# srendle/libfm

Measured on AMD Instinct MI355X. Metric: SGD training examples/sec at k=64, nnz=32, 1e+08 feat, higher is better.
Workload: dtype f32

## Files before the change

libfm_amd/build.py:

```python
import os
import subprocess
import sys
from concurrent.futures import ThreadPoolExecutor

HERE = os.path.dirname(os.path.abspath(__file__))
ROOT = os.path.dirname(HERE)
CSRC = os.path.join(HERE, "csrc")
SRC = [os.path.join(CSRC, f) for f in ("fmx_core.hip", "fmx_sgd.hip", "fmx_als.hip", "fmx_io.hip", "fmx_comm.hip", "fmx_pair.hip", "fmx_topk.hip", "fmx_pairneg.hip", "fmx_eval.hip", "fmx_post.hip", "fmx_evalq.hip", "fmx_compact.hip", "fmx_rankq.hip", "fmx_mem.hip")]
DEPS = SRC + sorted(os.path.join(CSRC, f) for f in os.listdir(CSRC) if f.endswith(".h")) + [os.path.join(ROOT, "include", "fmx.h")]
EXTRA = os.environ.get("FMX_DEFS", "").split()
OUT = os.path.join(HERE, os.environ.get("FMX_OUT", "libfmx.so"))
OBJ_DIR = os.path.join(HERE, "build" + ("_" + os.environ["FMX_OUT"].replace(".", "_") if "FMX_OUT" in os.environ else ""))
HIPCC = os.environ.get("HIPCC", "/opt/rocm/bin/hipcc")
FLAGS = ["--offload-arch=gfx950", "-O3", "-std=c++17", "-munsafe-fp-atomics", "-fPIC", "-fvisibility=hidden",
         "-Wno-unused-result", "-Wno-unused-value"]


def needs_build():
    if not os.path.exists(OUT):
        return True
    t = os.path.getmtime(OUT)
    return any(os.path.getmtime(d) > t for d in DEPS)


def build(force=False, verbose=False):
    if not force and not needs_build():
        return OUT
    os.makedirs(OBJ_DIR, exist_ok=True)
    objs = [os.path.join(OBJ_DIR, os.path.basename(s)[:-4] + ".o") for s in SRC]

    def cc(pair):
        cmd = [HIPCC] + FLAGS + EXTRA + ["-c", pair[0], "-o", pair[1]]
        if verbose:
            print(" ".join(cmd))
        subprocess.check_call(cmd)
    with ThreadPoolExecutor(len(SRC)) as ex:
        list(ex.map(cc, zip(SRC, objs)))
    cmd = [HIPCC, "--offload-arch=gfx950", "-shared", "-fPIC"] + objs + ["-ldl", "-o", OUT]
    if verbose:
        print(" ".join(cmd))
    subprocess.check_call(cmd)
    return OUT


if __name__ == "__main__":
    print(build(force="--force" in sys.argv, verbose=True))
```

libfm_amd/csrc/fmx_core.hip:

```cpp
#include "fmx_internal.h"

static thread_local std::string g_create_error = "";

int fail(fmx_handle h, int code, const char* fmt, ...) {
  char buf[512];
  va_list ap;
  va_start(ap, fmt);
  vsnprintf(buf, sizeof(buf), fmt, ap);
  va_end(ap);
  if (h) h->err = buf; else g_create_error = buf;
  return code;
}

static int next_pow2(int k) { int p = 1; while (p < k) p <<= 1; return p; }

Hyper make_hyper(const fmx_config& c) {
  Hyper h;
  h.lr = (float)c.learn_rate; h.reg0 = (float)c.reg0; h.regw = (float)c.regw; h.regv = (float)c.regv;
  h.min_target = (float)c.min_target; h.max_target = (float)c.max_target;
  h.task = c.task; h.k0 = c.k0; h.k1 = c.k1;
  h.lr_d = c.learn_rate; h.reg0_d = c.reg0; h.regw_d = c.regw; h.regv_d = c.regv;
  h.min_d = c.min_target; h.max_d = c.max_target;
  h.sgda = 0;
  return h;
}

Shard make_shard(const fmx_config& c) {
  Shard sh;
  sh.n = c.num_attribute; sh.rank = (uint32_t)c.shard_rank; sh.world = (uint32_t)c.shard_world;
  sh.hashed = (c.shard_hash != 0 && c.shard_world > 1) ? 1u : 0u;
  uint32_t bits = 1; while (bits < 32 && (1ull << bits) < c.num_attribute) bits++;
  sh.half_bits = std::max<uint32_t>(1u, (bits + 1) / 2);
  return sh;
}

uint32_t resident_grid(fmx_handle h, const void* kernel, uint64_t n_waves_wanted, int over_default) {
  auto& cache = h->occ_cache;
  auto it = cache.find(kernel);
  int occ;
  if (it == cache.end()) {
    occ = 0;
    if (hipOccupancyMaxActiveBlocksPerMultiprocessor(&occ, kernel, 256, 0) != hipSuccess || occ < 1) occ = 4;
    if (occ > 8) occ = 8;
    cache[kernel] = occ;
  } else {
    occ = it->second;
  }
  uint64_t blocks = (n_waves_wanted + 3) / 4;
  const int over = over_default;
  const uint64_t cap = (uint64_t)occ * (uint64_t)h->num_cu * (uint64_t)over;
  if (blocks < 1) blocks = 1;
  if (blocks > cap) blocks = cap;
  return (uint32_t)blocks;
}
int ensure_scratch(fmx_handle h, size_t batch_cap, size_t rest_cap) {
  if (batch_cap > h->cap) {
    if (h->partial) fmx_dev_free(h->partial);
    if (h->mult) fmx_dev_free(h->mult);
    h->partial = nullptr; h->mult = nullptr; h->cap = 0;
    HIPCHK(h, fmx_dev_alloc(&h->partial, batch_cap * (size_t)(h->KP + 1) * sizeof(float)));
    HIPCHK(h, fmx_dev_alloc(&h->mult, batch_cap * sizeof(float)));
    h->cap = batch_cap;
  }
  if (rest_cap > h->cap_rest) {
    if (h->rest) fmx_dev_free(h->rest);
    h->rest = nullptr; h->cap_rest = 0;
    HIPCHK(h, fmx_dev_alloc(&h->rest, rest_cap * sizeof(float)));
    h->cap_rest = rest_cap;
  }
  return FMX_OK;
}

int check_slot(fmx_handle h, int slot, bool need_target) {
  if (!h) return FMX_E_ARG;
  if (slot < 0 || slot >= FMX_MAX_SLOTS) return fail(h, FMX_E_ARG, "slot %d out of range", slot);
  if (!h->slots[slot].used) return fail(h, FMX_E_STATE, "slot %d holds no rows (call fmx_upload_rows first)", slot);
  if (need_target && !h->slots[slot].target) return fail(h, FMX_E_STATE, "slot %d was uploaded without targets", slot);
  return FMX_OK;
}

int slot_in_session(fmx_handle h, int slot, const char* what) {
  if (h->als.slot >= 0 && h->als.slot == slot)
    return fail(h, FMX_E_STATE, "%s: slot %d is the train slot of an open ALS / MCMC session (call fmx_als_end first)", what, slot);
  return FMX_OK;
}

void free_segments(Slot& s) {
  if (s.t_ent) fmx_dev_free(s.t_ent);
  if (s.seg_feat) fmx_dev_free(s.seg_feat);
  if (s.seg_rel) fmx_dev_free(s.seg_rel);
  if (s.cmask) fmx_dev_free(s.cmask);
  if (s.cseg) fmx_dev_free(s.cseg);
  if (s.cdesc) fmx_dev_free(s.cdesc);
  if (s.d_batch_seg) fmx_dev_free(s.d_batch_seg);
  if (s.d_cbatch) fmx_dev_free(s.d_cbatch);
  if (s.d_batch_base) fmx_dev_free(s.d_batch_base);
  s.cdesc = nullptr; s.d_batch_seg = nullptr; s.d_cbatch = nullptr; s.d_batch_base = nullptr;
  s.t_ent = nullptr; s.seg_feat = nullptr; s.seg_rel = nullptr; s.seg_B = 0; s.nseg = 0;
  s.cmask = nullptr; s.cseg = nullptr; s.ncseg = 0; s.fused_cap = 0;
  s.batch_seg.clear(); s.batch_base.clear(); s.cbatch.clear();
}

void free_block(BlockRows* b) {
  if (!b) return;
  free_slot(b->rows);
  if (b->map) fmx_dev_free(b->map);
  if (b->brow_ptr) fmx_dev_free(b->brow_ptr);
  if (b->brow_list) fmx_dev_free(b->brow_list);
  if (b->pbuf) fmx_dev_free(b->pbuf);
  delete b;
}

void free_slot(Slot& s) {
  for (BlockRows* b : s.blocks) free_block(b);
  s.blocks.clear();
  free_segments(s);
  free_pairs(s);
  free_interactions(s);
  free_post(s);
  if (s.ent) fmx_dev_free(s.ent);
  if (s.row_ptr) fmx_dev_free(s.row_ptr);
  if (s.target) fmx_dev_free(s.target);
  if (s.wside) fmx_dev_free(s.wside);
  if (s.lmask) fmx_dev_free(s.lmask);
  if (s.qid) fmx_dev_free(s.qid);
  s = Slot();
}

int ensure_wside(fmx_handle h, Slot& s) {
  if (s.wside) return FMX_OK;
  if (s.nnz == 0 || s.nnz >= (1ull << 32) - 1) return FMX_OK;
  struct Acc { fmx_handle h; std::chrono::steady_clock::time_point t0;
               ~Acc() { h->setup_acc += std::chrono::duration<double>(std::chrono::steady_clock::now() - t0).count(); } } acc_{h, std::chrono::steady_clock::now()};
  const uint32_t M = (uint32_t)std::min<uint64_t>(std::max<uint64_t>(h->n_local, 1), 1ull << 27);
  uint32_t* last = nullptr;
  hipError_t er = fmx_dev_alloc(&last, (size_t)M * 4);
  if (er == hipSuccess) er = fmx_dev_alloc(&s.wside, (size_t)s.nnz * 4);
  if (er == hipSuccess) er = fmx_dev_alloc(&s.lmask, (size_t)s.n_rows * 8);
  if (er == hipSuccess) er = hipMemsetAsync(last, 0, (size_t)M * 4, h->stream);
  if (er == hipSuccess) {
    hipLaunchKernelGGL(k_wside_last, dim3((unsigned)std::min<uint64_t>((s.nnz + 255) / 256, 8192)), dim3(256), 0, h->stream, s.ent, s.nnz, M, last);
    hipLaunchKernelGGL(k_wside_mask, dim3((unsigned)std::min<uint32_t>((s.n_rows + 3) / 4, 16384)), dim3(256), 0, h->stream, s.ent, s.row_ptr, s.n_rows, M,
                       (const uint32_t*)last, s.lmask, s.wside);
    er = hipGetLastError();
  }
  if (er == hipSuccess) er = hipStreamSynchronize(h->stream);
  if (last) fmx_dev_free(last);
  if (er != hipSuccess) {
    if (s.wside) fmx_dev_free(s.wside);
    if (s.lmask) fmx_dev_free(s.lmask);
    s.wside = nullptr; s.lmask = nullptr;
    return fail(h, FMX_E_HIP, "weight side stream of the slot: %s", hipGetErrorString(er));
  }
  s.wside_version = 0;
  if (getenv("FMX_TRACE_SETUP")) fprintf(stderr, "[fmx setup] weight side stream %8.3f ms\n", 1e3 * std::chrono::duration<double>(std::chrono::steady_clock::now() - acc_.t0).count());
  return FMX_OK;
}

int launch_rest(fmx_handle h, const Slot& s, uint64_t row0, uint32_t n, float* rest, hipStream_t st, const CompactState* snap) {
  if (!s.blocks.empty()) {
    if (row0 != 0 || n != s.n_rows) return fail(h, FMX_E_ARG, "rows with kept blocks are predicted as a whole");
    int rc = ensure_scratch(h, n, 0);
    if (rc) return rc;
    float* S = h->partial;
    float* c = S + (size_t)n * h->KP;
    KP_SWITCH(h->KP, FMX_LAUNCH_WAVES((k_rowsums<KP, true, false>), n, st, s.ent, s.row_ptr, (uint64_t)0, n, RowsF32{h->tb}, h->cfg.k1, S, c));
    for (BlockRows* br : s.blocks) {
      const uint32_t B = br->rows.n_rows;
      if (!B) continue;
      Tab tb = h->tb;
      tb.V += (size_t)br->attr_offset * tb.rs; tb.w += (size_t)br->attr_offset * tb.ws;
      float* Sb = br->pbuf;
      KP_SWITCH(h->KP, FMX_LAUNCH_WAVES((k_rowsums<KP, true, false>), B, st, br->rows.ent, br->rows.row_ptr, (uint64_t)0, B, RowsF32{tb}, h->cfg.k1,
                                         Sb, Sb + (size_t)B * h->KP));
      KP_SWITCH(h->KP, hipLaunchKernelGGL((k_rel_add_partial<KP>), dim3(std::min<uint32_t>((uint32_t)(((uint64_t)n * (h->KP + 1) + 255) / 256), 4096)),
                                            dim3(256), 0, st, br->map, (uint64_t)0, n, B, (const float*)Sb, S));
    }
    KP_SWITCH(h->KP, hipLaunchKernelGGL((k_rest_from_partial<KP>), dim3(wave_grid((n + Map<KP>::EPI - 1) / Map<KP>::EPI)), dim3(256), 0, st,
                                          (const float*)S, (const float*)c, n, rest));
    HIPCHK(h, hipGetLastError());
    return FMX_OK;
  }
  const float* ws = (s.wside && s.wside_version == h->w_version && h->cfg.shard_world == 1) ? s.wside : nullptr;
  if (snap) { KP_SWITCH(h->KP, FMX_LAUNCH_WAVES((k_rowsums<KP, false, true, RowsBf16>), n, st,
                                                 s.ent, s.row_ptr, row0, n, compact_rows(h, *snap), h->cfg.k1, (float*)nullptr, rest)); }
  else { KP_SWITCH(h->KP, FMX_LAUNCH_WAVES((k_rowsums<KP, false, true>), n, st,
                                            s.ent, s.row_ptr, row0, n, RowsF32{h->tb, ws}, h->cfg.k1, (float*)nullptr, rest)); }
  HIPCHK(h, hipGetLastError());
  return FMX_OK;
}

int slot_scores(fmx_handle h, const Slot& s, const CompactState* snap, bool want_yhat, const float** score) {
  int rc = ensure_scratch(h, 0, (size_t)s.n_rows * 2); if (rc) return rc;
  HIPCHK(h, hipEventRecord(h->ev0, h->stream));
  rc = launch_rest(h, s, 0, s.n_rows, h->rest, h->stream, snap); if (rc) return rc;
  *score = h->rest;
  if (!want_yhat) return FMX_OK;
  float* yhat = h->rest + s.n_rows;
  const int k0 = (h->cfg.shard_world > 1 && h->cfg.shard_rank != 0) ? 0 : h->cfg.k0;
  hipLaunchKernelGGL(k_yhat, dim3(std::min<uint32_t>((s.n_rows + 255) / 256, 2048)), dim3(256), 0, h->stream,
                     h->rest, s.n_rows, k0, snap ? snap->w0 : h->w0, yhat);
  HIPCHK(h, hipGetLastError());
  *score = yhat;
  return FMX_OK;
}

int predict_out(fmx_handle h, const Slot& s, const CompactState* snap, double* out) {
  if (s.n_rows == 0) return FMX_OK;
  const float* yhat;
  const int rc = slot_scores(h, s, snap, true, &yhat); if (rc) return rc;
  std::vector<float> tmp(s.n_rows);
  HIPCHK(h, hipMemcpyAsync(tmp.data(), yhat, (size_t)s.n_rows * sizeof(float), hipMemcpyDeviceToHost, h->stream));
  HIPCHK(h, hipStreamSynchronize(h->stream));
  for (uint32_t r = 0; r < s.n_rows; r++) out[r] = (double)tmp[r];
  return FMX_OK;
}

int evaluate_out(fmx_handle h, const Slot& s, const CompactState* snap, fmx_eval* out) {
  const float* rest;
  const int rc = slot_scores(h, s, snap, false, &rest); if (rc) return rc;
  HIPCHK(h, hipMemsetAsync(h->acc, 0, 4 * sizeof(double), h->stream));
  hipLaunchKernelGGL(k_eval, dim3(std::min<uint32_t>((s.n_rows + 255) / 256, 2048)), dim3(256), 0, h->stream,
                     rest, s.target, s.n_rows, make_hyper(h->cfg), snap ? snap->w0 : h->w0, h->acc);
  HIPCHK(h, hipGetLastError());
  HIPCHK(h, hipEventRecord(h->ev1, h->stream));
  double acc[4];
  HIPCHK(h, hipMemcpyAsync(acc, h->acc, sizeof(acc), hipMemcpyDeviceToHost, h->stream));
  HIPCHK(h, hipStreamSynchronize(h->stream));
  float ms = 0;
  HIPCHK(h, hipEventElapsedTime(&ms, h->ev0, h->ev1));
  out->device_seconds = ms * 1e-3;
  out->rmse = std::sqrt(acc[0] / s.n_rows);
  out->mae = acc[1] / s.n_rows;
  out->accuracy = acc[2] / s.n_rows;
  return FMX_OK;
}

int ensure_coll_mass(fmx_handle h, Slot& s) {
  if (s.coll_mass >= 0.0) return FMX_OK;
  if (s.nnz == 0 || s.n_rows == 0) { s.coll_mass = 0.0; return FMX_OK; }
  struct Acc { fmx_handle h; std::chrono::steady_clock::time_point t0;
               ~Acc() { h->setup_acc += std::chrono::duration<double>(std::chrono::steady_clock::now() - t0).count(); } } acc_{h, std::chrono::steady_clock::now()};
  HIPCHK(h, hipSetDevice(h->device));
  const uint32_t M = (uint32_t)std::min<uint64_t>(std::max<uint64_t>(h->n_local, 1), 1ull << 27);
  double* hist = nullptr;
  HIPCHK(h, fmx_dev_alloc(&hist, (size_t)M * sizeof(double)));
  hipError_t er = hipMemsetAsync(hist, 0, (size_t)M * sizeof(double), h->stream);
  if (er == hipSuccess) er = hipMemsetAsync(h->acc, 0, 2 * sizeof(double), h->stream);
  if (er == hipSuccess) {
    hipLaunchKernelGGL(k_coll_hist, dim3((unsigned)std::min<uint64_t>((s.nnz + 255) / 256, 8192)), dim3(256), 0, h->stream, s.ent, s.nnz, M, hist, h->acc + 1);
    hipLaunchKernelGGL(k_coll_sumsq, dim3((unsigned)std::min<uint64_t>(((uint64_t)M + 255) / 256, 4096)), dim3(256), 0, h->stream,
                       (const double*)hist, M, h->acc);
    er = hipGetLastError();
  }
  double c[2] = {0.0, 0.0};
  if (er == hipSuccess) er = hipMemcpyAsync(c, h->acc, 2 * sizeof(double), hipMemcpyDeviceToHost, h->stream);
  if (er == hipSuccess) er = hipStreamSynchronize(h->stream);
  fmx_dev_free(hist);
  if (er != hipSuccess) return fail(h, FMX_E_HIP, "collision mass of the rows: %s", hipGetErrorString(er));
  const double N = (double)s.n_rows;
  s.coll_mass = (s.n_rows > 1) ? std::max(0.0, c[0] - c[1]) / (N * (N - 1.0)) : 0.0;
  if (getenv("FMX_TRACE_SETUP")) fprintf(stderr, "[fmx setup] collision mass     %8.3f ms\n", 1e3 * std::chrono::duration<double>(std::chrono::steady_clock::now() - acc_.t0).count());
  return FMX_OK;
}

void resolve_batch(const fmx_config& cfg, double coll_mass, uint32_t requested, uint32_t dflt, double curv_scale, fmx_batch_info* out) {
  const double curv = ((cfg.task == FMX_TASK_REGRESSION) ? 1.0 : 0.25) * curv_scale;
  const double per_row = cfg.learn_rate * curv * coll_mass;
  uint32_t B = requested ? requested : dflt;
  uint32_t status = 0;
  if (!requested && per_row > 0.0 && (double)B * per_row > 1.0) {
    uint32_t cut = 1;
    while ((double)(cut * 2) * per_row <= 1.0 && cut * 2 <= dflt) cut *= 2;
    B = std::max(cut, 32u);
    status |= FMX_STAT_BATCH_CUT;
  }
  out->collision_mass = coll_mass;
  out->batch = B;
  out->batch_gain = (double)B * per_row;
  if (out->batch_gain > 2.0) status |= FMX_STAT_UNSTABLE;
  out->status = status;
}

extern "C" {

int fmx_abi_version(void) { return FMX_ABI_VERSION; }

int fmx_device_count(void) {
  int n = 0;
  if (hipGetDeviceCount(&n) != hipSuccess) return 0;
  return n;
}

const char* fmx_last_error(fmx_handle h) { return h ? h->err.c_str() : g_create_error.c_str(); }

int fmx_create(const fmx_config* cfg, fmx_handle* out) {
  if (!cfg || !out) return fail(nullptr, FMX_E_ARG, "fmx_create: null argument");
  *out = nullptr;
  if (cfg->num_attribute == 0) return fail(nullptr, FMX_E_ARG, "num_attribute must be > 0");
  if (cfg->num_attribute > 0xFFFFFFFFull) return fail(nullptr, FMX_E_ARG, "num_attribute must fit uint32 (fm_model.h:51)");
  if (cfg->num_factor < 0) return fail(nullptr, FMX_E_ARG, "num_factor must be >= 0");
  if (cfg->num_factor > 1024) return fail(nullptr, FMX_E_UNSUPPORTED, "num_factor > 1024 is not supported");
  if (cfg->task != FMX_TASK_REGRESSION && cfg->task != FMX_TASK_CLASSIFICATION)
    return fail(nullptr, FMX_E_ARG, "unknown task");
  if (cfg->shard_world < 1 || cfg->shard_rank < 0 || cfg->shard_rank >= cfg->shard_world)
    return fail(nullptr, FMX_E_ARG, "bad shard_rank/shard_world");
  if (cfg->shard_hash != 0 && cfg->shard_hash != 1) return fail(nullptr, FMX_E_ARG, "shard_hash must be 0 or 1");
  if (cfg->place_candidates < 0 || cfg->place_candidates > 6) return fail(nullptr, FMX_E_ARG, "place_candidates must be 0 (default) .. 6");
  if (cfg->exchange_algo != FMX_EXCHANGE_ALLREDUCE && cfg->exchange_algo != FMX_EXCHANGE_RS_AG)
    return fail(nullptr, FMX_E_ARG, "exchange_algo %u: FMX_EXCHANGE_ALLREDUCE (0) or FMX_EXCHANGE_RS_AG (1)", cfg->exchange_algo);
  if ((uint64_t)cfg->shard_world > cfg->num_attribute) return fail(nullptr, FMX_E_ARG, "more feature shards than features");
  int ndev = 0;
  hipError_t e = hipGetDeviceCount(&ndev);
  if (e != hipSuccess || ndev == 0)
    return fail(nullptr, FMX_E_HIP, "no HIP device available (%s); libfmx has no CPU fallback",
                e == hipSuccess ? "device count 0" : hipGetErrorString(e));
  int dev = cfg->device;
  if (dev < 0) { if (hipGetDevice(&dev) != hipSuccess) dev = 0; }
  if (dev >= ndev) return fail(nullptr, FMX_E_ARG, "device %d out of range (%d devices)", dev, ndev);

  fmx_handle h = new fmx_context_s();
  h->cfg = *cfg;
  h->device = dev;
  h->KP = next_pow2(std::max(cfg->num_factor, 1));
  const uint64_t n = cfg->num_attribute, W = (uint64_t)cfg->shard_world, R = (uint64_t)cfg->shard_rank;
  h->n_local = (n > R) ? (n - R + W - 1) / W : 0;
  if (h->n_local == 0) h->n_local = 1;
#define CREATE_CHK(expr)                                                                     \
  do { hipError_t _e = (expr); if (_e != hipSuccess) {                                       \
      fail(nullptr, FMX_E_HIP, "%s failed: %s", #expr, hipGetErrorString(_e));               \
      fmx_destroy(h); return FMX_E_HIP; } } while (0)
  CREATE_CHK(hipSetDevice(dev));
  mark_device_used(dev);
  CREATE_CHK(hipGetDeviceProperties(&h->prop, dev));
  CREATE_CHK(hipStreamCreateWithFlags(&h->stream, hipStreamNonBlocking));
  CREATE_CHK(hipEventCreate(&h->ev0));
  CREATE_CHK(hipEventCreate(&h->ev1));
  {
    h->tb.rs = (uint32_t)h->KP;
    { const char* rk = getenv("FMX_ROW_STRIDE_KP");
      if (h->KP >= 32 && !(rk && rk[0] == '1')) h->tb.rs = std::min<uint32_t>((uint32_t)h->KP, ((uint32_t)cfg->num_factor + 15u) / 16u * 16u); }
    if (place_tables(h) != FMX_OK) { fmx_destroy(h); return FMX_E_HIP; }
    h->tb.w = h->w_sep; h->tb.ws = 1;
  }
  CREATE_CHK(fmx_dev_alloc(&h->w0, sizeof(double)));
  CREATE_CHK(fmx_dev_alloc(&h->w0_pp, 8 * sizeof(double)));
  {
    CREATE_CHK(fmx_dev_alloc(&h->handoff_ctr, 2 * sizeof(unsigned long long)));
    h->handoff_err = reinterpret_cast<uint32_t*>(h->handoff_ctr + 1);
    CREATE_CHK(hipMemsetAsync(h->handoff_ctr, 0, 2 * sizeof(unsigned long long), h->stream));
    const char* e = getenv("FMX_HANDOFF");
    h->handoff = !(e && e[0] == '0');
    CREATE_CHK(fmx_dev_alloc(&h->pit_ctr, (PIT_MAX_IT + 1) * sizeof(unsigned long long)));
    CREATE_CHK(fmx_dev_alloc(&h->pit_slots, (size_t)2 * PIT_MAX_WG * 4 * sizeof(double)));
    CREATE_CHK(hipMemsetAsync(h->pit_slots, 0, (size_t)2 * PIT_MAX_WG * 4 * sizeof(double), h->stream));
    const char* sc = getenv("FMX_SCAN");
    h->scan_pit = !(sc && strcmp(sc, "serial") == 0);
    const char* so = getenv("FMX_SMALL_ONE");
    h->small_one = !(so && so[0] == '0');
    auto env_on = [](const char* name) { const char* e = getenv(name); return !(e && e[0] == '0'); };
    h->seq_rows = env_on("FMX_SEQ_ROWS");
    h->seq_wg = env_on("FMX_SEQ_WG");
    h->seq_runs_fused = env_on("FMX_SEQ_RUNS_FUSED");
    h->seq_runs_one = env_on("FMX_SEQ_RUNS_ONE");
    const char* ts = getenv("FMX_TOPK_SPLITS");
    if (ts) h->topk_splits = (uint32_t)std::min<unsigned long>(strtoul(ts, nullptr, 10), 1024ul);
    const char* sp = getenv("FMX_DEBUG_PIT_SPINS");
    h->pit_spins = sp ? (uint32_t)strtoul(sp, nullptr, 10) : HANDOFF_SPINS;
  }
  {
    int lo = 0, hi = 0;
    CREATE_CHK(hipDeviceGetStreamPriorityRange(&lo, &hi));
    CREATE_CHK(hipStreamCreateWithPriority(&h->stream2, hipStreamNonBlocking, hi));
  }
  h->num_cu = h->prop.multiProcessorCount > 0 ? h->prop.multiProcessorCount : 256;
  CREATE_CHK(fmx_dev_alloc(&h->acc, 4 * sizeof(double)));
  CREATE_CHK(hipMemsetAsync(h->w0, 0, sizeof(double), h->stream));
  CREATE_CHK(hipStreamSynchronize(h->stream));
#undef CREATE_CHK
  *out = h;
  return FMX_OK;
}

int fmx_batch_rule(int32_t task, double learn_rate, double collision_mass, uint32_t requested, fmx_batch_info* out) {
  if (!out || (task != FMX_TASK_REGRESSION && task != FMX_TASK_CLASSIFICATION) || !(learn_rate >= 0.0) || !(collision_mass >= 0.0)) return FMX_E_ARG;
  fmx_config c = {};
  c.task = task; c.learn_rate = learn_rate;
  resolve_batch(c, collision_mass, requested, FMX_DEFAULT_BATCH, 1.0, out);
  return FMX_OK;
}

int fmx_destroy(fmx_handle h) {
  if (!h) return FMX_OK;
  hipSetDevice(h->device);
  if (h->stream) hipStreamSynchronize(h->stream);
  comm_free(h);
  als_free(h);
  sgda_free(h);
  adapt_free(h);
  ftrl_free(h);
  compact_free(h);
  for (auto& s : h->slots) free_slot(s);
  if (h->grp) fmx_dev_free(h->grp);
  free_tables(h);
  if (h->w0) fmx_dev_free(h->w0);
  if (h->w0_pp) fmx_dev_free(h->w0_pp);
  if (h->handoff_ctr) fmx_dev_free(h->handoff_ctr);
  if (h->pit_ctr) fmx_dev_free(h->pit_ctr);
  if (h->probe_flags) fmx_dev_free(h->probe_flags);
  if (h->pit_tmp) fmx_dev_free(h->pit_tmp);
  if (h->run_slots) fmx_dev_free(h->run_slots);
  if (h->small_slots) fmx_dev_free(h->small_slots);
  if (h->pit_slots) fmx_dev_free(h->pit_slots);
  if (h->w0_slots) fmx_dev_free(h->w0_slots);
  if (h->stream2) hipStreamDestroy(h->stream2);
  if (h->acc) fmx_dev_free(h->acc);
  if (h->partial) fmx_dev_free(h->partial);
  if (h->mult) fmx_dev_free(h->mult);
  if (h->rest) fmx_dev_free(h->rest);
  for (auto ev : h->ev_pool) hipEventDestroy(ev);
  for (auto ev : h->ev_sync) hipEventDestroy(ev);
  if (h->lag.ev_rest) hipEventDestroy(h->lag.ev_rest);
  for (auto e : h->lag.ev_scan) if (e) hipEventDestroy(e);
  if (h->ev0) hipEventDestroy(h->ev0);
  if (h->ev1) hipEventDestroy(h->ev1);
  if (h->stream) hipStreamDestroy(h->stream);
  delete h;
  return FMX_OK;
}

int fmx_get_info(fmx_handle h, fmx_info* out) {
  if (!h || !out) return FMX_E_ARG;
  memset(out, 0, sizeof(*out));
  out->n_local = h->n_local;
  out->k_padded = h->KP;
  out->device = h->device;
  out->bytes_params = h->n_local * (size_t)(h->tb.rs + (h->w_sep ? 1 : 0)) * sizeof(float);
  snprintf(out->device_name, sizeof(out->device_name), "%s", h->prop.name);
  snprintf(out->arch, sizeof(out->arch), "%s", h->prop.gcnArchName);
  return FMX_OK;
}

int fmx_synchronize(fmx_handle h) {
  if (!h) return FMX_E_ARG;
  { int _rc = lag_flush(h); if (_rc) return _rc; }
  HIPCHK(h, hipSetDevice(h->device));
  HIPCHK(h, hipStreamSynchronize(h->stream));
  return scan_error_check(h);
}

static int stage_params(fmx_handle h, bool to_device, double* w0, double* w, double* v) {
  if (to_device) touch_w(h);
  HIPCHK(h, hipSetDevice(h->device));
  const uint64_t n = h->cfg.num_attribute;
  const int k = h->cfg.num_factor, KP = h->KP;
  const int W = h->cfg.shard_world;
  const Shard sh = make_shard(h->cfg);
  if (to_device) {
    HIPCHK(h, hipMemcpyAsync(h->w0, w0, sizeof(double), hipMemcpyHostToDevice, h->stream));
  } else {
    HIPCHK(h, hipMemcpyAsync(w0, h->w0, sizeof(double), hipMemcpyDeviceToHost, h->stream));
  }
  const uint32_t chunk = (uint32_t)std::min<uint64_t>(n, 1u << 18);
  double* stage = nullptr;
  HIPCHK(h, fmx_dev_alloc(&stage, (size_t)chunk * (size_t)std::max(k, 1) * sizeof(double)));
  int rc = FMX_OK;
#define STAGE_CHK(expr) do { hipError_t _e = (expr); if (_e != hipSuccess) { \
    rc = fail(h, FMX_E_HIP, "%s failed: %s", #expr, hipGetErrorString(_e)); goto done; } } while (0)
  for (uint64_t j0 = 0; j0 < n; j0 += chunk) {
    const uint32_t cnt = (uint32_t)std::min<uint64_t>(chunk, n - j0);
    if (w) {
      if (to_device) {
        STAGE_CHK(hipMemcpyAsync(stage, w + j0, cnt * sizeof(double), hipMemcpyHostToDevice, h->stream));
        hipLaunchKernelGGL(k_w_in, dim3((cnt + 255) / 256), dim3(256), 0, h->stream, stage, j0, cnt, sh, h->tb);
      } else {
        if (W > 1) STAGE_CHK(hipMemcpyAsync(stage, w + j0, cnt * sizeof(double), hipMemcpyHostToDevice, h->stream));
        hipLaunchKernelGGL(k_w_out, dim3((cnt + 255) / 256), dim3(256), 0, h->stream, stage, j0, cnt, sh, h->tb);
        STAGE_CHK(hipMemcpyAsync(w + j0, stage, cnt * sizeof(double), hipMemcpyDeviceToHost, h->stream));
      }
      STAGE_CHK(hipStreamSynchronize(h->stream));
    }
    if (v && k > 0) {
      if (to_device) {
        for (int f = 0; f < k; f++)
          STAGE_CHK(hipMemcpyAsync(stage + (size_t)f * cnt, v + (size_t)f * n + j0, cnt * sizeof(double),
                                   hipMemcpyHostToDevice, h->stream));
        const uint64_t total = (uint64_t)cnt * KP;
        hipLaunchKernelGGL(k_stage_in, dim3((uint32_t)((total + 255) / 256)), dim3(256), 0, h->stream,
                           stage, j0, cnt, k, KP, sh, h->tb);
      } else {
        if (W > 1)
          for (int f = 0; f < k; f++)
            STAGE_CHK(hipMemcpyAsync(stage + (size_t)f * cnt, v + (size_t)f * n + j0, cnt * sizeof(double),
                                     hipMemcpyHostToDevice, h->stream));
        const uint64_t total = (uint64_t)cnt * k;
        hipLaunchKernelGGL(k_stage_out, dim3((uint32_t)((total + 255) / 256)), dim3(256), 0, h->stream,
                           stage, j0, cnt, k, KP, sh, h->tb);
        for (int f = 0; f < k; f++)
          STAGE_CHK(hipMemcpyAsync(v + (size_t)f * n + j0, stage + (size_t)f * cnt, cnt * sizeof(double),
                                   hipMemcpyDeviceToHost, h->stream));
      }
      STAGE_CHK(hipStreamSynchronize(h->stream));
    }
  }
  STAGE_CHK(hipGetLastError());
  STAGE_CHK(hipStreamSynchronize(h->stream));
done:
#undef STAGE_CHK
  fmx_dev_free(stage);
  return rc;
}

int fmx_set_params(fmx_handle h, double w0, const double* w, const double* v) {
  if (!h) return FMX_E_ARG;
  { int _rc = lag_flush(h); if (_rc) return _rc; }
  if (h->cfg.num_factor > 0 && !v) return fail(h, FMX_E_ARG, "fmx_set_params: v is NULL but num_factor > 0");
  double w0c = w0;
  return stage_params(h, true, &w0c, const_cast<double*>(w), const_cast<double*>(v));
}

int fmx_get_params(fmx_handle h, double* w0, double* w, double* v) {
  if (!h || !w0) return FMX_E_ARG;
  { int _rc = lag_flush(h); if (_rc) return _rc; }
  return stage_params(h, false, w0, w, v);
}

int fmx_get_param_rows(fmx_handle h, const uint32_t* ids, uint32_t count, double* w_out, double* v_out) {
  if (!h || !ids || !w_out) return FMX_E_ARG;
  { int _rc = lag_flush(h); if (_rc) return _rc; }
  const int k = h->cfg.num_factor;
  const Shard sh = make_shard(h->cfg);
  if (k > 0 && !v_out) return fail(h, FMX_E_ARG, "fmx_get_param_rows: v_out is NULL");
  if (count == 0) return FMX_OK;
  for (uint32_t i = 0; i < count; i++) {
    if (ids[i] >= h->cfg.num_attribute) return fail(h, FMX_E_ARG, "feature id %u >= num_attribute", ids[i]);
    if (!sh.owns(ids[i])) return fail(h, FMX_E_ARG, "feature id %u is not on this shard", ids[i]);
  }
  double* const outs[1][2] = {{w_out, v_out}};
  return gather_rows(h, "fmx_get_param_rows", ids, count, 1, outs, [&](int, dim3 grid, const uint32_t* d_ids, double* d_w, double* d_v) {
    hipLaunchKernelGGL(k_fetch_rows<RowsF32>, grid, dim3(256), 0, h->stream, d_ids, count, k, sh, RowsF32{h->tb}, d_w, d_v);
  });
}

int fmx_save_model(fmx_handle h, const char* path) {
  if (!h || !path) return FMX_E_ARG;
  if (h->cfg.shard_world > 1) return fail(h, FMX_E_UNSUPPORTED, "fmx_save_model on a feature shard: collect the parameters with fmx_get_params");
  { int _rc = lag_flush(h); if (_rc) return _rc; }
  HIPCHK(h, hipSetDevice(h->device));
  HIPCHK(h, hipStreamSynchronize(h->stream));
  FILE* f = fopen(path, "w");
  if (!f) return fail(h, FMX_E_ARG, "fmx_save_model: cannot open %s", path);
  const uint64_t n = h->cfg.num_attribute;
  const int k = h->cfg.num_factor;
  const size_t chunk = 1u << 16;
  std::vector<float> buf(chunk * (size_t)std::max<uint32_t>(h->tb.rs, 1));
  int rc = FMX_OK;
  if (h->cfg.k0) {
    double w0 = 0;
    if (hipMemcpy(&w0, h->w0, sizeof(double), hipMemcpyDeviceToHost) != hipSuccess) rc = FMX_E_HIP;
    fprintf(f, "#global bias W0\n%g\n", w0);
  }
// ... 535 lines not shown
```

libfm_amd/csrc/fmx_internal.h:

```cpp
#pragma once
#pragma GCC visibility push(default)
#include "../../include/fmx.h"
#pragma GCC visibility pop
#include "fmx_kernels.h"
#include "fmx_als_kernels.h"
#include "fmx_compact_kernels.h"
#include "fmx_place_plan.h"

#include <hipcub/hipcub.hpp>

#include <algorithm>
#include <chrono>
#include <cmath>
#include <cstdarg>
#include <cstdio>
#include <cstring>
#include <mutex>
#include <random>
#include <string>
#include <unordered_map>
#include <unordered_set>
#include <vector>

using namespace fmx;

struct Slot {
  Entry*    ent = nullptr;
  uint64_t* row_ptr = nullptr;
  float*    target = nullptr;
  uint32_t  n_rows = 0;
  uint64_t  nnz = 0;
  uint32_t  max_row = 0;
  uint32_t  fixed_nnz = 0;
  bool      used = false;
  double    coll_mass = -1.0;
  double    coll_mass_world = -1.0;
  uint32_t  seg_B = 0;
  TEntry*   t_ent = nullptr;
  uint32_t* seg_feat = nullptr;
  uint32_t* seg_rel = nullptr;
  uint32_t  nseg = 0;
  bool      all_ones = false;
  uint32_t  max_seg_count = 0;
  std::vector<uint32_t> batch_seg;
  std::vector<uint64_t> batch_base;
  uint64_t* cmask = nullptr;
  uint32_t* cseg = nullptr;
  uint32_t  ncseg = 0;
  CDesc*    cdesc = nullptr;
  uint32_t  fused_cap = 0;
  std::vector<uint32_t> cbatch;
  uint32_t* d_batch_seg = nullptr;
  uint32_t* d_cbatch = nullptr;
  uint64_t* d_batch_base = nullptr;
  float*    wside = nullptr;
  uint64_t* lmask = nullptr;
  uint64_t  wside_version = 0;
  std::vector<uint32_t> run_start;
  std::vector<uint8_t>  run_single;
  std::vector<struct BlockRows*> blocks;
  bool      pairs_set = false;
  uint64_t  n_pairs = 0;
  uint32_t* pair_a = nullptr;
  uint32_t* pair_b = nullptr;
  uint64_t* pair_off = nullptr;
  uint64_t  pair_nnz = 0;
  uint32_t  pair_max_len = 0;
  uint32_t  pair_seg_B = 0;
  TEntry*   pair_t_ent = nullptr;
  uint32_t* pair_seg_head = nullptr;
  uint32_t* pair_seg_feat = nullptr;
  uint32_t  pair_nseg = 0, pair_max_seg = 0;
  std::vector<uint32_t> pair_batch_seg;
  struct PairNeg* pneg = nullptr;
  struct PostAcc* post = nullptr;
  uint32_t* qid = nullptr;
  uint32_t  n_queries = 0;
};
void free_pairs(Slot& s);
void free_interactions(Slot& s);
void drop_interactions(fmx_handle h, int slot);

struct BlockRows {
  Slot      rows;
  uint32_t* map = nullptr;
  uint32_t  attr_offset = 0;
  uint32_t* brow_ptr = nullptr;
  uint32_t* brow_list = nullptr;
  float*    pbuf = nullptr;
};
void free_block(BlockRows* b);
int check_block_rows(fmx_handle h, const void* entries, const uint64_t* row_ptr, uint32_t n_rows, uint64_t nnz,
                     const fmx_relation* relations, uint32_t n_relations);
int attach_kept_blocks(fmx_handle h, int slot, uint32_t n_rows, const fmx_relation* relations, uint32_t n_relations);

struct AlsBlock {
  uint32_t* level_list = nullptr;
  std::vector<uint32_t> level_ptr;
  double*   cache = nullptr;
  double*   qb_all = nullptr;
  double*   cpart = nullptr;
  double*   delta = nullptr;
  int       lanes = 8;
};

struct AlsState {
  int       slot = -1;
  EQ*       e = nullptr;
  double*   q = nullptr;
  uint8_t*  seen = nullptr;
  uint32_t* level_list = nullptr;
  uint4*    ldesc = nullptr;
  std::vector<uint32_t> level_ptr;
  uint64_t  iter = 0;
  std::vector<AlsBlock> blk;
  EQ*       delta = nullptr;
  double*   epart = nullptr;
  float*    vt = nullptr;
  size_t    vt_stride = 0;
  uint32_t* r_row = nullptr; uint32_t* r_pos = nullptr; float* r_x = nullptr;
  float2*   dth = nullptr;
  std::vector<uint32_t> lev_ent;
  std::vector<uint8_t> lev_dense;
  uint32_t* t_row = nullptr;
  uint32_t  split_min = 0;
  double*   prior = nullptr;
  std::vector<double> prior_host;
};

struct LagState {
  static constexpr uint32_t RING = 8;
  bool       active = false;
  uint64_t   step = 0;
  uint32_t   depth = 1;
  hipEvent_t ev_rest = nullptr, ev_scan[RING] = {};
  hipStream_t in_stream = nullptr;
};

struct SgdaState { float* gw = nullptr; float* gv = nullptr; double* reg = nullptr; double* dreg = nullptr;
                   size_t dreg_cap = 0; };
struct AdaptState { float* nw = nullptr; float* nv = nullptr; float eta = 0.f; };
struct FtrlState { float* zw = nullptr; float* zv = nullptr; float* nw = nullptr; float* nv = nullptr;
                   float inv_alpha = 0.f, beta = 0.f, l1_w = 0.f, l1_v = 0.f, l2_w = 0.f, l2_v = 0.f; };
struct CompactState { uint16_t* V = nullptr; float* w = nullptr; double* w0 = nullptr; };

struct fmx_context_s {
  fmx_config cfg;
  AlsState   als;
  SgdaState  sgda;
  AdaptState adapt;
  FtrlState  ftrl;
  CompactState compact;
  LagState   lag;
  int        KP = 1;
  double     setup_acc = 0.0;
  uint32_t*  grp = nullptr;
  uint32_t   num_groups = 1;
  uint64_t   n_local = 0;
  int        device = 0;
  hipStream_t stream = nullptr;
  Tab        tb = {nullptr, nullptr, 0, 0};
  float*     w_sep = nullptr;
  Placed     placed;
  double*    w0 = nullptr;
  double*    w0_pp = nullptr;
  hipStream_t stream2 = nullptr;
  bool        handoff = true;
  double*     w0_slots = nullptr;
  uint64_t    w0_slots_cap = 0;
  unsigned long long* handoff_ctr = nullptr;
  unsigned long long  handoff_seq = 0;
  uint32_t*   handoff_err = nullptr;
  uint32_t    handoff_err_host = 0;
  bool        scan_pit = true;
  unsigned long long* pit_ctr = nullptr;
  double*     pit_slots = nullptr;
  bool        pit_used = false;
  uint32_t    run_status = 0;
  int         concurrent = -1;
  unsigned*   probe_flags = nullptr;
  uint32_t    pit_spins = 0;
  int         pit_occ = -1;
  double*     pit_tmp = nullptr;
  uint64_t    w_version = 1;
  int        num_cu = 256;
  double*    acc = nullptr;
  Slot       slots[FMX_MAX_SLOTS];
  float*     partial = nullptr;
  float*     mult = nullptr;
  float*     rest = nullptr;
  size_t     cap = 0, cap_rest = 0;
  hipEvent_t ev0 = nullptr, ev1 = nullptr;
  std::vector<hipEvent_t> ev_pool;
  std::vector<hipEvent_t> ev_sync;
  std::string err;
  hipDeviceProp_t prop;
  void*       comm = nullptr;
  struct fmx_group_s* group = nullptr;
  bool        owns_group = false;
  float*      xbuf[2] = {nullptr, nullptr};
  size_t      xcap = 0;
  hipStream_t stream_comm = nullptr;
  hipEvent_t  ev_x[4] = {};
  std::unordered_map<const void*, int> occ_cache;
  std::unordered_set<const void*> lds_raised;
  std::unordered_map<const void*, int> run_one_occ;
  bool run_one = true, run_one_used = false;
  bool seq_rows = true, seq_wg = true, seq_runs_fused = true, seq_runs_one = true;
  uint32_t topk_splits = 0;
  unsigned long long* run_slots = nullptr;
  unsigned long long* small_slots = nullptr;
  bool small_one = true, small_one_used = false;
};

int fail(fmx_handle h, int code, const char* fmt, ...);
Hyper make_hyper(const fmx_config& c);
Shard make_shard(const fmx_config& c);
constexpr int FMX_GRID_OVER_SGD = 1 << 16;
constexpr int FMX_GRID_OVER_ALS = 2;
#ifndef FMX_GRID_OVER_DEFAULT
#define FMX_GRID_OVER_DEFAULT FMX_GRID_OVER_SGD
#endif
uint32_t resident_grid(fmx_handle h, const void* kernel, uint64_t n_waves_wanted, int over_default = FMX_GRID_OVER_DEFAULT);
int ensure_scratch(fmx_handle h, size_t batch_cap, size_t rest_cap);
int check_slot(fmx_handle h, int slot, bool need_target);
int slot_in_session(fmx_handle h, int slot, const char* what);
void free_segments(Slot& s);
void free_slot(Slot& s);
int launch_rest(fmx_handle h, const Slot& s, uint64_t row0, uint32_t n, float* rest, hipStream_t st, const CompactState* snap = nullptr);
int slot_scores(fmx_handle h, const Slot& s, const CompactState* snap, bool want_yhat, const float** score);
int predict_out(fmx_handle h, const Slot& s, const CompactState* snap, double* out);
int evaluate_out(fmx_handle h, const Slot& s, const CompactState* snap, fmx_eval* out);
inline RowsBf16 compact_rows(fmx_handle h, const CompactState& c) { return RowsBf16{CTab{c.V, c.w, h->tb.rs}}; }
int ensure_segments(fmx_handle h, Slot& s, uint32_t B);
int ensure_coll_mass(fmx_handle h, Slot& s);
int ensure_wside(fmx_handle h, Slot& s);
inline void touch_w(fmx_handle h) { if (h) h->w_version++; }
void resolve_batch(const fmx_config& cfg, double coll_mass, uint32_t requested, uint32_t dflt, double curv_scale, fmx_batch_info* out);
constexpr uint32_t FMX_DEFAULT_BATCH = 262144u;
constexpr uint32_t FMX_SIDE_STREAM_BATCH = 32768u;
inline bool sgd_in_stream_batch(uint32_t batch, uint32_t flags) { return batch != 0 && batch < FMX_SIDE_STREAM_BATCH && (flags & FMX_FLAG_BIAS_LAG); }
int sgd_resolve_batch(fmx_handle h, Slot& s, const fmx_sgd_opts* opts, fmx_batch_info* bi);
int sgd_partial_rows(fmx_handle h, const Slot& s, uint64_t row0, uint32_t n_rows, float* S, float* c, hipStream_t st,
                     const CompactState* snap = nullptr);
constexpr size_t PREP_RAW_FLOATS = size_t(1) << 24;
int prep_rows(fmx_handle h, const Slot& s, uint64_t row0, uint32_t n, int k0, float* raw, size_t raw_rows, int KM,
              float* S_out, float* scal, hipStream_t st, const CompactState* snap = nullptr);
int topk_impl(fmx_handle h, const char* who, int query_slot, int cand_slot, const fmx_topk_opts* opts, uint32_t* idx_out, double* score_out,
              fmx_topk_stats* stats, const CompactState* snap);
void compact_free(fmx_handle h);
int lag_flush(fmx_handle h);
int eval_ex_check_opts(fmx_handle h, const char* who, const fmx_eval_opts* opts, uint32_t* link);
int eval_ex_check_slot(fmx_handle h, const char* who, int slot);
void eval_ex_empty(fmx_eval_ex* out);
int eval_ex_scores(fmx_handle h, const Slot& s, const float* score, int add_w0, uint32_t link, fmx_eval_ex* out);
struct EvalScratch;
int rank_sort_scan(fmx_handle h, EvalScratch& sc, unsigned long long* keys, uint32_t n, int key_bits, size_t b_more,
                   const unsigned long long** sorted);
int eval_ex_rank(fmx_handle h, unsigned long long* keys, uint32_t n, int key_bits, unsigned long long* d_num2, uint64_t* num2,
                 double* rank_seconds);
int eval_ex_finish(fmx_handle h, uint32_t n, const double* d, uint64_t pos, uint64_t nan_rows, uint64_t correct,
                   unsigned long long* keys, int key_bits, unsigned long long* d_num2, fmx_eval_ex* out);
int set_row_queries_impl(fmx_handle h, const char* who, int slot, const uint32_t* qid, uint32_t n_queries);
int evalq_check_slot(fmx_handle h, const char* who, int slot);
void evalq_empty(fmx_eval_query* out, uint32_t n_queries);
void evalq_zero_per_query(uint32_t n_queries, uint64_t* num2_q, uint32_t* pos_q, uint32_t* neg_q);
int evalq_scores(fmx_handle h, const Slot& s, const float* score, int add_w0, uint32_t link, fmx_eval_query* out,
                 uint64_t* num2_q, uint32_t* pos_q, uint32_t* neg_q);
int evalq_scores_keep(fmx_handle h, const Slot& s, const float* score, int add_w0, uint32_t link, fmx_eval_query* out,
                      uint64_t* num2_q, uint32_t* pos_q, uint32_t* neg_q, EvalScratch& sc, const unsigned long long** sorted);
int rankq_check_opts(fmx_handle h, const char* who, const fmx_rank_opts* opts, uint32_t* link);
void rankq_empty(fmx_eval_rank* out, const fmx_rank_opts* opts, uint32_t n_queries, double* dcg_q, double* hits_q);
int rankq_scores(fmx_handle h, const Slot& s, const float* score, int add_w0, uint32_t link, const fmx_rank_opts* opts,
                 fmx_eval_rank* out, double* dcg_q, double* hits_q);
struct PostAcc {
  double*  sum_all = nullptr;
  double*  sum_late = nullptr;
  float*   last = nullptr;
  uint32_t burn_in = 5, eval_rows = 0;
  uint64_t draws = 0, late_draws = 0;
};
void free_post(Slot& s);
int post_check(fmx_handle h, const char* who, int slot, bool need_begin);
int post_begin_impl(fmx_handle h, const char* who, int slot, const fmx_post_opts* opts);
int post_accum_scores(fmx_handle h, Slot& s, const float* score, int add_w0, fmx_post_stats* out);
int post_evaluate_impl(fmx_handle h, const char* who, int slot, uint32_t which, fmx_eval_ex* out);
int post_get_impl(fmx_handle h, const char* who, int slot, uint32_t which, double* out, uint64_t* draws);
int post_end_impl(fmx_handle h, const char* who, int slot);
int scan_error_check(fmx_handle h);
uint32_t multi_group_size(const Slot& s, int KP);
bool streams_concurrent(fmx_handle h);
void sgda_free(fmx_handle h);
void adapt_free(fmx_handle h);
void ftrl_free(fmx_handle h);
void als_free(fmx_handle h);
enum { GROUP_SINGLE = 0, GROUP_LOOPBACK = 1, GROUP_RCCL = 2 };
struct fmx_group_s {
  std::vector<fmx_handle> hs;
  int kind = GROUP_SINGLE;
  std::vector<void*> comms;
  bool owns_comms = false;
  std::vector<hipEvent_t> ev_part;
  hipEvent_t ev_sum = nullptr;
  std::string err;
};
int group_allreduce_f64(fmx_group_s* g, const std::vector<double*>& bufs, size_t count);
void comm_free(fmx_handle h);
int comm_sgd_epoch(fmx_handle h, int slot, const fmx_sgd_opts* opts, fmx_epoch_stats* stats);
int comm_sum_double(fmx_handle h, double* v);

void arena_cache_drop(int device);
hipError_t fmx_dev_alloc_bytes(void** p, size_t bytes);
hipError_t fmx_dev_free(void* p);
void mark_device_used(int dev);
int place_tables(fmx_handle h);
void free_tables(fmx_handle h);
template <class T> inline hipError_t fmx_dev_alloc(T** p, size_t bytes) { return fmx_dev_alloc_bytes(reinterpret_cast<void**>(p), bytes); }

struct EvalScratch {
  void* part = nullptr;
  unsigned long long* keys0 = nullptr; unsigned long long* keys1 = nullptr;
  uint32_t* negbefore = nullptr; uint32_t* runhead = nullptr; uint32_t* qhead = nullptr;
  void* tmp = nullptr; size_t tmp_bytes = 0;
  void* perq = nullptr;
  hipEvent_t ev[2] = {nullptr, nullptr};
  ~EvalScratch() {
    fmx_dev_free(part); fmx_dev_free(keys0); fmx_dev_free(keys1); fmx_dev_free(negbefore); fmx_dev_free(runhead); fmx_dev_free(qhead);
    fmx_dev_free(tmp); fmx_dev_free(perq);
    for (auto e : ev) if (e) hipEventDestroy(e);
  }
};

#define HIPCHK(h, expr)                                                                        \
  do {                                                                                          \
    hipError_t _e = (expr);                                                                     \
    if (_e != hipSuccess)                                                                       \
      return fail((h), FMX_E_HIP, "%s failed: %s (%s:%d)", #expr, hipGetErrorString(_e), __FILE__, __LINE__); \
  } while (0)

template <class Launch>
int gather_rows(fmx_handle h, const char* who, const uint32_t* ids, uint32_t count, int nt, double* const (*outs)[2], Launch launch) {
  const int k = h->cfg.num_factor;
  HIPCHK(h, hipSetDevice(h->device));
  uint32_t* d_ids = nullptr; double* d_out = nullptr;
  const size_t nout = (size_t)count * (size_t)(k + 1);
  HIPCHK(h, fmx_dev_alloc(&d_ids, (size_t)count * 4));
  hipError_t er = fmx_dev_alloc(&d_out, nout * sizeof(double));
  if (er == hipSuccess) er = hipMemcpyAsync(d_ids, ids, (size_t)count * 4, hipMemcpyHostToDevice, h->stream);
  for (int t = 0; t < nt && er == hipSuccess; t++) {
    launch(t, dim3((uint32_t)((nout + 255) / 256)), (const uint32_t*)d_ids, d_out, d_out + count);
    er = hipGetLastError();
    if (er == hipSuccess) er = hipMemcpyAsync(outs[t][0], d_out, (size_t)count * sizeof(double), hipMemcpyDeviceToHost, h->stream);
    if (er == hipSuccess && k > 0) er = hipMemcpyAsync(outs[t][1], d_out + count, (size_t)count * k * sizeof(double), hipMemcpyDeviceToHost, h->stream);
    if (er == hipSuccess) er = hipStreamSynchronize(h->stream);
  }
  fmx_dev_free(d_ids); fmx_dev_free(d_out);
  if (er != hipSuccess) return fail(h, FMX_E_HIP, "%s: %s", who, hipGetErrorString(er));
  return FMX_OK;
}

inline uint32_t wave_grid(uint64_t n_waves_wanted) {
  uint64_t blocks = (n_waves_wanted + 3) / 4;
  if (blocks < 1) blocks = 1;
  if (blocks > 256 * 8) blocks = 256 * 8;
  return (uint32_t)blocks;
}

#define FMX_LAUNCH_WAVES(kfn, waves, st, ...)                                                        \
  do { auto _k = kfn; hipLaunchKernelGGL(_k, dim3(resident_grid(h, (const void*)_k, (waves))), dim3(256), 0, st, __VA_ARGS__); } while (0)

#define KP_SWITCH(KPV, ...)                                            \
  switch (KPV) {                                                       \
    case 1:   { constexpr int KP = 1;   __VA_ARGS__; } break;          \
    case 2:   { constexpr int KP = 2;   __VA_ARGS__; } break;          \
    case 4:   { constexpr int KP = 4;   __VA_ARGS__; } break;          \
    case 8:   { constexpr int KP = 8;   __VA_ARGS__; } break;          \
    case 16:  { constexpr int KP = 16;  __VA_ARGS__; } break;          \
    case 32:  { constexpr int KP = 32;  __VA_ARGS__; } break;          \
    case 64:  { constexpr int KP = 64;  __VA_ARGS__; } break;          \
    case 128: { constexpr int KP = 128; __VA_ARGS__; } break;          \
    case 256: { constexpr int KP = 256; __VA_ARGS__; } break;          \
    case 512: { constexpr int KP = 512; __VA_ARGS__; } break;          \
    case 1024: { constexpr int KP = 1024; __VA_ARGS__; } break;        \
    default: return fail(h, FMX_E_UNSUPPORTED, "num_factor > 1024 is not supported");   \
  }
```

libfm_amd/csrc/fmx_mem.hip:

```cpp
#include "fmx_internal.h"
#include "fmx_place_kernels.h"
#include <atomic>

namespace {
std::atomic<uint64_t> g_devices_used{0};

int chk(hipError_t e) { if (e != hipSuccess) (void)hipGetLastError(); return (int)e; }
struct HipVm : Vm {
  int device = 0;
  int reserve(void** va, size_t bytes, size_t align) override { return chk(hipMemAddressReserve(va, bytes, align, nullptr, 0)); }
  int free_address(void* va, size_t bytes) override { return chk(hipMemAddressFree(va, bytes)); }
  int create(void** hnd, size_t bytes) override {
    hipMemAllocationProp prop = {};
    prop.type = hipMemAllocationTypePinned; prop.location.type = hipMemLocationTypeDevice; prop.location.id = device;
    return chk(hipMemCreate((hipMemGenericAllocationHandle_t*)hnd, bytes, &prop, 0));
  }
  int release(void* hnd) override { return chk(hipMemRelease((hipMemGenericAllocationHandle_t)hnd)); }
  int map(void* at, size_t bytes, void* hnd) override { return chk(hipMemMap(at, bytes, 0, (hipMemGenericAllocationHandle_t)hnd, 0)); }
  int unmap(void* at, size_t bytes) override { return chk(hipMemUnmap(at, bytes)); }
  int set_access(void* at, size_t bytes) override { return access_for(at, bytes, device); }
  int access_for(void* at, size_t bytes, int dev) {
    hipMemAccessDesc acc = {};
    acc.location.type = hipMemLocationTypeDevice; acc.location.id = dev; acc.flags = hipMemAccessFlagsProtReadWrite;
    return chk(hipMemSetAccess(at, bytes, &acc, 1));
  }
};
HipVm* hip_vm(int device) {
  static HipVm* const vms = []() { HipVm* v = new HipVm[64]; for (int d = 0; d < 64; d++) v[d].device = d; return v; }();
  return (device >= 0 && device < 64) ? &vms[device] : nullptr;
}
struct HipProbe : Probe {
  fmx_handle h;
  explicit HipProbe(fmx_handle h_) : h(h_) {}
  int zero(void* at, size_t bytes) override { return chk(hipMemsetAsync(at, 0, bytes, h->stream)); }
  int sync() override { return chk(hipStreamSynchronize(h->stream)); }
  int pair_ms(void* a, void* b, float* ms) override {
    const uint32_t rows_shift = 22;
    const uint32_t waves = 1u << 17;
    float best = 1e30f;
    for (int rep = 0; rep < 2; rep++) {
      hipError_t e = hipEventRecord(h->ev0, h->stream);
      hipLaunchKernelGGL(k_place_pair, dim3(waves / 4), dim3(256), 0, h->stream, (float*)a, (float*)b, rows_shift, waves, (uint64_t)rep * 7919 + 1);
      if (e == hipSuccess) e = hipGetLastError();
      if (e == hipSuccess) e = hipEventRecord(h->ev1, h->stream);
      if (e == hipSuccess) e = hipEventSynchronize(h->ev1);
      float t = 0.f;
      if (e == hipSuccess) e = hipEventElapsedTime(&t, h->ev0, h->ev1);
      if (e != hipSuccess) return (int)e;
      if (rep && t < best) best = t;
    }
    *ms = best;
    return 0;
  }
};

std::mutex g_arena_mu;
Placed* const g_arena_cache = new Placed[16];
bool arena_cache_on() { const char* e = getenv("FMX_ARENA_CACHE"); return !(e && e[0] == '0'); }
double since(std::chrono::steady_clock::time_point t0) { return std::chrono::duration<double>(std::chrono::steady_clock::now() - t0).count(); }
}

void mark_device_used(int dev) { if (dev >= 0 && dev < 64) g_devices_used.fetch_or(1ull << dev, std::memory_order_relaxed); }

void arena_cache_drop(int device) {
  std::lock_guard<std::mutex> lk(g_arena_mu);
  for (int d = 0; d < 16; d++)
    if ((device < 0 || d == device) && g_arena_cache[d].mem.va) {
      int cur = 0; (void)hipGetDevice(&cur); (void)hipSetDevice(d);
      (void)g_arena_cache[d].mem.release();
      (void)hipSetDevice(cur);
    }
}

static void arena_free(fmx_handle h) {
  Placed& A = h->placed;
  if (h->device >= 0 && h->device < 16 && arena_cache_on()) {
    (void)hipStreamSynchronize(h->stream);
    std::lock_guard<std::mutex> lk(g_arena_mu);
    Placed& c = g_arena_cache[h->device];
    if (!c.mem.va || c.mem.ch.size() < A.mem.ch.size()) {
      c = std::move(A);
      return;
    }
  }
  const int e = A.mem.release();
  if (e) h->err = std::string("arena_free: hipMemUnmap failed: ") + hipGetErrorString((hipError_t)e);
}

static bool arena_build(fmx_handle h, size_t v_bytes, size_t w_bytes, int bound_tables) {
  const auto t_start = std::chrono::steady_clock::now();
  Layout L;
  if (!place_layout(v_bytes, w_bytes, &L) || !hip_vm(h->device)) return false;
  const size_t T = L.T;
  Placed A;
  bool have = false;
  if (h->device >= 0 && h->device < 16) {
    std::lock_guard<std::mutex> lk(g_arena_mu);
    Placed& c = g_arena_cache[h->device];
    if (c.mem.va && c.mem.ch.size() >= T) {
      if (!prefix_serves(c.cls, L, v_bytes, w_bytes)) (void)c.mem.release();
      else {
        A = std::move(c);
        A.mem.shrink(T);
        prefix_recount(&A.cls, T, A.info.per_class);
        A.info.chunks = (uint32_t)T; A.info.pool = 0;
        have = hipMemsetAsync(A.mem.va, 0, T * ARENA_CHUNK, h->stream) == hipSuccess;
        if (!have) { (void)hipGetLastError(); (void)A.mem.release(); }
      }
    }
  }
  if (!have) {
    size_t free_b = 0, total_b = 0;
    if (hipMemGetInfo(&free_b, &total_b) != hipSuccess) return false;
    if (!arena_fits(T, free_b)) {
      arena_cache_drop(h->device);
      if (hipMemGetInfo(&free_b, &total_b) != hipSuccess) return false;
    }
    if (!arena_fits(T, free_b)) return false;
    HipProbe probe(h);
    A = Placed();
    if (build_arena(*hip_vm(h->device), probe, T, pool_bound(T, bound_tables, free_b), &A) != 0) return false;
  }
  h->placed = std::move(A);
  h->tb.V = (float*)h->placed.mem.va;
  h->w_sep = (float*)((char*)h->placed.mem.va + L.w_off);
  h->placed.info.seconds = since(t_start);
  return true;
}

namespace {
struct BigAlloc { int device = 0; ChunkRange mem; };
std::mutex g_big_mu;
auto& g_big = *new std::unordered_map<void*, BigAlloc>();
constexpr size_t BIG_MIN = (size_t)768 << 20, BIG_CHUNK = (size_t)1 << 30, BIG_ALIGN = (size_t)2 << 20;
bool big_alloc_on() { static const bool on = []() { const char* e = getenv("FMX_BIG_ALLOC"); return !(e && e[0] == '0'); }(); return on; }

hipError_t plain_alloc(void** p, size_t bytes) {
  hipError_t e = hipMalloc(p, bytes);
  if (e == hipErrorOutOfMemory) {
    (void)hipGetLastError();
    int d = 0;
    if (hipGetDevice(&d) == hipSuccess) { arena_cache_drop(d); e = hipMalloc(p, bytes); }
  }
  return e;
}
bool big_alloc(void** p, size_t bytes) {
  int dev = 0;
  if (hipGetDevice(&dev) != hipSuccess || !hip_vm(dev)) return false;
  HipVm& vm = *hip_vm(dev);
  BigAlloc b; b.device = dev;
  const size_t reserved = (bytes + BIG_ALIGN - 1) / BIG_ALIGN * BIG_ALIGN;
  static const bool trace = getenv("FMX_TRACE_ALLOC") != nullptr;
  const auto t0 = std::chrono::steady_clock::now();
  if (b.mem.reserve(vm, reserved, BIG_ALIGN)) return false;
  const double t_res = 1e3 * since(t0);
  bool ok = true;
  for (size_t off = 0; off < reserved && ok; off += BIG_CHUNK)
    ok = b.mem.create(std::min(BIG_CHUNK, reserved - off)) == 0 && b.mem.map(b.mem.ch.size() - 1) == 0;
  const double t_map = 1e3 * since(t0);
  if (ok) {
    int ndev = 0; (void)hipGetDeviceCount(&ndev);
    ok = vm.set_access(b.mem.va, reserved) == 0;
    const uint64_t used = g_devices_used.load(std::memory_order_relaxed);
    for (int d = 0; ok && d < ndev && d < 64; d++) {
      if (d == dev || !((used >> d) & 1ull)) continue;
      int can = 0;
      if (hipDeviceCanAccessPeer(&can, d, dev) != hipSuccess || !can) { (void)hipGetLastError(); continue; }
      (void)vm.access_for(b.mem.va, reserved, d);
    }
  }
  if (trace) fprintf(stderr, "[fmx alloc] big %zu bytes: reserve %.3f ms, create+map %.3f ms, access %.3f ms\n", bytes, t_res, t_map - t_res, 1e3 * since(t0) - t_map);
  if (!ok) return false;
  *p = b.mem.va;
  { std::lock_guard<std::mutex> lk(g_big_mu); g_big.emplace(*p, std::move(b)); }
  return true;
}
hipError_t dev_alloc_untraced(void** p, size_t bytes) {
  if (!p) return hipErrorInvalidValue;
  *p = nullptr;
  if (bytes >= BIG_MIN && big_alloc_on()) {
    if (big_alloc(p, bytes)) return hipSuccess;
    int d = 0;
    if (hipGetDevice(&d) == hipSuccess) { arena_cache_drop(d); if (big_alloc(p, bytes)) return hipSuccess; }
  }
  return plain_alloc(p, bytes);
}
}

hipError_t fmx_dev_alloc_bytes(void** p, size_t bytes) {
  static const bool trace = getenv("FMX_TRACE_ALLOC") != nullptr;
  if (!trace) return dev_alloc_untraced(p, bytes);
  const auto t0 = std::chrono::steady_clock::now();
  const hipError_t e = dev_alloc_untraced(p, bytes);
  const double ms = 1e3 * since(t0);
  if (ms > 0.5) fprintf(stderr, "[fmx alloc] %12zu bytes %9.3f ms%s\n", bytes, ms, e == hipSuccess ? "" : " FAILED");
  return e;
}
hipError_t fmx_dev_free(void* p) {
  if (!p) return hipSuccess;
  BigAlloc b; bool big = false;
  {
    std::lock_guard<std::mutex> lk(g_big_mu);
    auto it = g_big.find(p);
    if (it != g_big.end()) { b = std::move(it->second); g_big.erase(it); big = true; }
  }
  if (!big) return hipFree(p);
  int cur = 0; (void)hipGetDevice(&cur);
  if (cur != b.device) (void)hipSetDevice(b.device);
  (void)hipDeviceSynchronize();
  (void)b.mem.release();
  if (cur != b.device) (void)hipSetDevice(cur);
  return hipSuccess;
}

static hipError_t alloc_placed(fmx_handle h, float** out, size_t bytes, int max_tries, bool rows) {
  size_t free_b = 0, total_b = 0;
  const bool probe_free = bytes >= ((size_t)256 << 20) && max_tries > 1;
  const int tries = candidate_count(bytes, max_tries, probe_free && hipMemGetInfo(&free_b, &total_b) == hipSuccess, free_b);
  float* cand[PLACE_MAX_CAND] = {};
  CandidateBook book;
  hipError_t er = hipSuccess;
  for (int c = 0; c < tries && er == hipSuccess; c++) {
    if (plain_alloc((void**)&cand[c], bytes) != hipSuccess) { (void)hipGetLastError(); cand[c] = nullptr; break; }
    er = hipMemsetAsync(cand[c], 0, bytes, h->stream);
    if (tries == 1 || er != hipSuccess) break;
    float ms = 0.f;
    for (int rep = 0; rep < 2 && er == hipSuccess; rep++) {
      er = hipEventRecord(h->ev0, h->stream);
      if (rows) {
        const uint32_t waves = 1u << 19;
        hipLaunchKernelGGL(k_place_probe, dim3(waves / 4), dim3(256), 0, h->stream, cand[c], (uint64_t)h->n_local, h->tb.rs, waves, (uint64_t)rep * 7919 + 1);
      } else {
        const uint64_t total = 1ull << 24;
        hipLaunchKernelGGL(k_place_probe_w, dim3((unsigned)(total / 256)), dim3(256), 0, h->stream, cand[c], (uint64_t)(bytes / sizeof(float)), total, (uint64_t)rep * 7919 + 1);
      }
      if (er == hipSuccess) er = hipGetLastError();
      if (er == hipSuccess) er = hipEventRecord(h->ev1, h->stream);
      if (er == hipSuccess) er = hipEventSynchronize(h->ev1);
      if (er == hipSuccess) er = hipEventElapsedTime(&ms, h->ev0, h->ev1);
    }
    if (book.timed(c, ms)) break;
  }
  if (er == hipSuccess && !cand[0]) {
    arena_cache_drop(h->device);
    er = plain_alloc((void**)&cand[0], bytes);
    if (er == hipSuccess) er = hipMemsetAsync(cand[0], 0, bytes, h->stream);
  }
  for (int c = 0; c < PLACE_MAX_CAND; c++) if ((c != book.best || er != hipSuccess) && cand[c]) { fmx_dev_free(cand[c]); cand[c] = nullptr; }
  *out = cand[book.best];
  return er;
}

int place_tables(fmx_handle h) {
  const auto t_place = std::chrono::steady_clock::now();
  const int pc = h->cfg.place_candidates;
  const size_t v_bytes = h->n_local * (size_t)h->tb.rs * sizeof(float), w_bytes = h->n_local * sizeof(float);
  if (pc != 1 && v_bytes >= ((size_t)2 << 30) && arena_build(h, v_bytes, w_bytes, pc > 1 ? pc : 3)) return FMX_OK;
  const int cand = pc > 0 ? std::min(pc, PLACE_MAX_CAND) : 2;
  hipError_t er = alloc_placed(h, &h->tb.V, v_bytes, cand, true);
  if (er != hipSuccess) return fail(nullptr, FMX_E_HIP, "alloc_placed(factor table) failed: %s", hipGetErrorString(er));
  er = alloc_placed(h, &h->w_sep, w_bytes, cand, false);
  if (er != hipSuccess) return fail(nullptr, FMX_E_HIP, "alloc_placed(linear weights) failed: %s", hipGetErrorString(er));
  h->placed.info.method = (cand > 1 && v_bytes >= ((size_t)256 << 20)) ? 1 : 0;
  h->placed.info.seconds = since(t_place);
  return FMX_OK;
}

void free_tables(fmx_handle h) {
  if (h->placed.mem.va) arena_free(h);
  else { if (h->tb.V) fmx_dev_free(h->tb.V); if (h->w_sep) fmx_dev_free(h->w_sep); }
}

extern "C" {

int fmx_release_cached_memory(void) { arena_cache_drop(-1); return FMX_OK; }

int fmx_place_layout(uint64_t v_bytes, uint64_t w_bytes, uint64_t* chunk_bytes, uint32_t* chunks, uint64_t* w_offset) {
  Layout L;
  if (!chunk_bytes || !chunks || !w_offset || !place_layout(v_bytes, w_bytes, &L)) return FMX_E_ARG;
  *chunk_bytes = ARENA_CHUNK; *chunks = L.T; *w_offset = L.w_off;
  return FMX_OK;
}

int fmx_get_place_info(fmx_handle h, fmx_place_info* out) {
  if (!h || !out) return FMX_E_ARG;
  *out = h->placed.info;
  return FMX_OK;
}

}
```

libfm_amd/csrc/fmx_place_plan.h:

```cpp
#pragma once
#include <algorithm>
#include <cstddef>
#include <cstdint>
#include <vector>

#include "../../include/fmx.h"

namespace fmx {

constexpr size_t ARENA_CHUNK = (size_t)1 << 30;
constexpr int PLACE_SHORT = -1;

struct Vm {
  virtual int reserve(void** va, size_t bytes, size_t align) = 0;
  virtual int free_address(void* va, size_t bytes) = 0;
  virtual int create(void** hnd, size_t bytes) = 0;
  virtual int release(void* hnd) = 0;
  virtual int map(void* at, size_t bytes, void* hnd) = 0;
  virtual int unmap(void* at, size_t bytes) = 0;
  virtual int set_access(void* at, size_t bytes) = 0;
};
struct Probe {
  virtual int zero(void* at, size_t bytes) = 0;
  virtual int pair_ms(void* a, void* b, float* ms) = 0;
  virtual int sync() = 0;
};

struct ChunkRange {
  struct Chunk { size_t off = 0, size = 0; void* hnd = nullptr; bool held = false, mapped = false; };
  Vm* vm = nullptr;
  void* va = nullptr;
  size_t reserved = 0;
  std::vector<Chunk> ch;

  ChunkRange() = default;
  ChunkRange(const ChunkRange&) = delete;
  ChunkRange& operator=(const ChunkRange&) = delete;
  ChunkRange(ChunkRange&& o) noexcept { *this = std::move(o); }
  ChunkRange& operator=(ChunkRange&& o) noexcept {
    if (this != &o) { release(); vm = o.vm; va = o.va; reserved = o.reserved; ch = std::move(o.ch); o.va = nullptr; o.reserved = 0; o.ch.clear(); }
    return *this;
  }
  ~ChunkRange() { release(); }

  void* at(size_t i) const { return (char*)va + ch[i].off; }
  size_t end() const { return ch.empty() ? 0 : ch.back().off + ch.back().size; }

  int reserve(Vm& v, size_t bytes, size_t align) {
    vm = &v;
    const int e = v.reserve(&va, bytes, align);
    if (e) va = nullptr; else reserved = bytes;
    return e;
  }
  int create(size_t size) {
    void* hd = nullptr;
    const int e = vm->create(&hd, size);
    if (!e) ch.push_back(Chunk{end(), size, hd, true, false});
    return e;
  }
  int map(size_t i) {
    const int e = vm->map(at(i), ch[i].size, ch[i].hnd);
    if (!e) ch[i].mapped = true;
    return e;
  }
  int take_from(ChunkRange& src, size_t i) {
    Chunk& s = src.ch[i];
    int e = vm->unmap(src.at(i), s.size);
    if (e) return e;
    s.mapped = false;
    e = vm->map((char*)va + end(), s.size, s.hnd);
    if (!e) ch.push_back(Chunk{end(), s.size, nullptr, false, true});
    return e;
  }
  void shrink(size_t n) {
    for (size_t i = n; i < ch.size(); i++) drop(ch[i]);
    if (n < ch.size()) ch.resize(n);
  }
  int release() {
    int first = 0;
    for (Chunk& c : ch) { const int e = drop(c); if (e && !first) first = e; }
    if (va) (void)vm->free_address(va, reserved);
    ch.clear(); va = nullptr; reserved = 0;
    return first;
  }

 private:
  int drop(Chunk& c) {
    const int e = c.mapped ? vm->unmap((char*)va + c.off, c.size) : 0;
    if (c.held) (void)vm->release(c.hnd);
    c.mapped = c.held = false;
    return e;
  }
};

struct Placed {
  ChunkRange mem;
  fmx_place_info info = {};
  std::vector<uint8_t> cls;
};

struct Layout { uint64_t w_off = 0; uint32_t T = 0; };
inline bool place_layout(uint64_t v_bytes, uint64_t w_bytes, Layout* L) {
  if (v_bytes == 0) return false;
  const uint64_t CH = ARENA_CHUNK;
  const uint64_t w_half = ((w_bytes / 2) + 255) & ~(uint64_t)255;
  const uint64_t boundary = (v_bytes + w_half + CH - 1) / CH;
  L->w_off = boundary * CH - w_half;
  const uint64_t T = (L->w_off + w_bytes + CH - 1) / CH;
  if (T > 0xFFFFFFFFull) return false;
  L->T = (uint32_t)T;
  return true;
}

inline bool arena_fits(size_t T, size_t free_b) { return T * ARENA_CHUNK + ((size_t)2 << 30) <= free_b; }
inline size_t pool_bound(size_t T, int bound_tables, size_t free_b) {
  const size_t b = std::min<size_t>((size_t)bound_tables * T + 64, T + (free_b - T * ARENA_CHUNK) / ARENA_CHUNK / 2);
  return std::max<size_t>(b, T);
}

inline bool prefix_serves(const std::vector<uint8_t>& cls, const Layout& L, uint64_t v_bytes, uint64_t w_bytes) {
  const size_t T = L.T, CH = ARENA_CHUNK;
  if (cls.size() < T) return false;
  auto both = [&](size_t c0, size_t c1) {
    if (c1 <= c0) return true;
    bool s0 = false, s1 = false;
    for (size_t k = c0; k <= c1 && k < T; k++) { s0 |= cls[k] == 0; s1 |= cls[k] == 1; }
    return s0 && s1;
  };
  const size_t v_last = v_bytes ? (v_bytes - 1) / CH : 0;
  const size_t w_first = L.w_off / CH, w_last = w_bytes ? (L.w_off + w_bytes - 1) / CH : w_first;
  return both(0, v_last) && both(w_first, w_last);
}
inline void prefix_recount(std::vector<uint8_t>* cls, size_t T, uint32_t per_class[2]) {
  cls->resize(T);
  per_class[0] = per_class[1] = 0;
  for (uint8_t c : *cls) if (c < 2) per_class[c]++;
}

struct ClassBook {
  std::vector<size_t> refs;
  std::vector<std::vector<size_t>> of;
  std::vector<size_t> mixed;
  std::vector<float> alone;
  std::vector<int> cls;
  float slow_ms = 0.f;
  int last_cls = -1;

  void push() { alone.push_back(0.f); cls.push_back(-1); }
  void pop() { alone.pop_back(); cls.pop_back(); }
  void set_slow() { std::vector<float> s(alone); std::sort(s.begin(), s.end()); slow_ms = s[s.size() / 2]; }
  template <class Pair>
  int classify(size_t i, Pair&& pair) {
    if (alone[i] > 0.f && alone[i] < 0.95f * slow_ms) { cls[i] = -2; mixed.push_back(i); return 0; }
    for (size_t t = 0; t < refs.size() && cls[i] < 0; t++) {
      const size_t k = (last_cls >= 0) ? (t == 0 ? (size_t)last_cls : (t <= (size_t)last_cls ? t - 1 : t)) : t;
      float ms = 0.f;
      const int e = pair(refs[k], i, &ms);
      if (e) return e;
      if (ms > slow_ms / 1.08f) { cls[i] = (int)k; of[k].push_back(i); last_cls = (int)k; }
    }
    if (cls[i] < 0) { refs.push_back(i); of.push_back({i}); cls[i] = (int)refs.size() - 1; last_cls = cls[i]; }
    return 0;
  }
  bool enough(size_t T, size_t* x, size_t* y) const {
    size_t a = SIZE_MAX, b = SIZE_MAX;
    for (size_t k = 0; k < of.size(); k++) {
      if (a == SIZE_MAX || of[k].size() > of[a].size()) { b = a; a = k; }
      else if (b == SIZE_MAX || of[k].size() > of[b].size()) b = k;
    }
    *x = a; *y = b;
    return a != SIZE_MAX && b != SIZE_MAX && of[a].size() >= (T + 1) / 2 && of[b].size() >= T / 2;
  }
};

inline bool mapping_order(const std::vector<size_t>& X, const std::vector<size_t>& Y, const std::vector<size_t>& rest, size_t T,
                          std::vector<size_t>* pick, std::vector<uint8_t>* cls, uint32_t per_class[2]) {
  const size_t ny = std::min<size_t>(Y.size(), T / 2), nx = std::min<size_t>(X.size(), T - ny);
  size_t ix = 0, iy = 0, ir = 0, acc = 0;
  pick->clear(); cls->clear();
  for (size_t c = 0; c < T; c++) {
    acc += ny;
    if (iy < ny && acc >= T) { acc -= T; pick->push_back(Y[iy++]); cls->push_back(1); }
    else if (ix < nx) { pick->push_back(X[ix++]); cls->push_back(0); }
    else if (iy < Y.size()) { pick->push_back(Y[iy++]); cls->push_back(1); }
    else if (ir < rest.size()) { pick->push_back(rest[ir++]); cls->push_back(2); }
  }
  per_class[0] = (uint32_t)ix; per_class[1] = (uint32_t)iy;
  return pick->size() == T;
}
inline bool mapping_order(const ClassBook& B, size_t T, std::vector<size_t>* pick, std::vector<uint8_t>* cls, uint32_t per_class[2]) {
  size_t cx, cy;
  (void)B.enough(T, &cx, &cy);
  const std::vector<size_t> none;
  std::vector<size_t> rest;
  for (size_t k = 0; k < B.of.size(); k++) if (k != cx && k != cy) rest.insert(rest.end(), B.of[k].begin(), B.of[k].end());
  rest.insert(rest.end(), B.mixed.begin(), B.mixed.end());
  return mapping_order(cx != SIZE_MAX ? B.of[cx] : none, cy != SIZE_MAX ? B.of[cy] : none, rest, T, pick, cls, per_class);
}

inline int build_arena(Vm& vm, Probe& dev, size_t T, size_t max_pool, Placed* out) {
  const size_t CH = ARENA_CHUNK;
  ChunkRange P, A;
  ClassBook B;
  int er = P.reserve(vm, max_pool * CH, CH);
  if (er) return er;
  auto pair = [&](size_t i, size_t j, float* ms) { return dev.pair_ms(P.at(i), P.at(j), ms); };
  auto take = [&]() -> int {
    const size_t i = P.ch.size();
    int e = P.create(CH);
    if (e) return e;
    B.push();
    e = P.map(i);
    if (e) return e;
    e = vm.set_access(P.at(i), CH);
    if (!e) e = dev.zero(P.at(i), CH);
    if (!e && i < 8) e = pair(i, i, &B.alone[i]);
    return e;
  };
  size_t cx, cy;
  const size_t first = std::min<size_t>(8, max_pool);
  while (!er && P.ch.size() < first) er = take();
  if (!er) {
    B.set_slow();
    for (size_t i = 0; i < first && !er; i++) er = B.classify(i, pair);
  }
  while (!er && P.ch.size() < max_pool && !B.enough(T, &cx, &cy)) {
    er = take();
    if (er) {
      if (P.ch.size() > T) { er = 0; if (!P.ch.back().mapped) { P.shrink(P.ch.size() - 1); B.pop(); } }
      break;
    }
    er = B.classify(P.ch.size() - 1, pair);
  }
  if (er || P.ch.size() < T) return er ? er : PLACE_SHORT;
  std::vector<size_t> pick;
  fmx_place_info info = {};
  if (!mapping_order(B, T, &pick, &out->cls, info.per_class)) return PLACE_SHORT;
  er = A.reserve(vm, T * CH, CH);
  if (er) return er;
  er = dev.sync();
  for (size_t c = 0; c < T && !er; c++) er = A.take_from(P, pick[c]);
  if (!er) er = vm.set_access(A.va, T * CH);
  if (er) return er;
  info.method = 2; info.chunks = (uint32_t)T; info.pool = (uint32_t)P.ch.size(); info.classes_seen = (uint32_t)B.refs.size();
  (void)P.release();
  er = dev.zero(A.va, T * CH);
  if (er) return er;
  out->mem = std::move(A);
  out->info = info;
  return 0;
}

constexpr int PLACE_MAX_CAND = 6;
inline int candidate_count(size_t bytes, int max_tries, bool free_known, size_t free_b) {
  if (bytes < ((size_t)256 << 20) || max_tries <= 1 || !free_known) return 1;
  return (int)std::min<size_t>((size_t)std::min(max_tries, PLACE_MAX_CAND), std::max<size_t>(1, free_b / (bytes + ((size_t)4 << 30))));
}
struct CandidateBook {
  float ms[PLACE_MAX_CAND] = {};
  int best = 0;
  bool timed(int c, float t) {
    ms[c] = t;
    if (ms[c] < ms[best]) best = c;
    float worst = 0.f;
    for (int i = 0; i <= c; i++) worst = std::max(worst, ms[i]);
    return c >= 1 && ms[best] < 0.95f * worst;
  }
};

}
```

libfm_amd/csrc/fmx_sgd.hip:

```cpp
#include "fmx_internal.h"
#include "fmx_online_kernels.h"
#include "fmx_seq_kernels.h"
#include "fmx_small_kernels.h"
#include "fmx_adapt_kernels.h"
#include "fmx_ftrl_kernels.h"

namespace {
uint32_t default_w0_chunk(const fmx_config& c) { return fmx_default_w0_chunk(c.learn_rate, c.task); }

template <int KP> constexpr bool fused_zr_ok(int zr) { return Map<KP>::VEC * zr <= 128; }
template <int KP> int fused_zr_select(uint32_t max_row) {
  constexpr int EPI = Map<KP>::EPI;
  const uint32_t need = (max_row + EPI - 1) / EPI;
  for (int zr : {8, 16, 32, 40, 64})
    if (fused_zr_ok<KP>(zr) && need <= (uint32_t)zr) return zr;
  return 8;
}
template <int KP> uint32_t fused_row_cap_kp(uint32_t max_row) {
  return std::min<uint32_t>(64u, (uint32_t)fused_zr_select<KP>(max_row) * (uint32_t)Map<KP>::EPI);
}

template <int KP, int VAR>
int launch_fused_zr(fmx_handle h, const Slot& s, const Hyper& hy, uint64_t row0, uint32_t n_rows, hipStream_t st,
                    const double* w0_in, float* rest_out, const uint64_t* cmask = nullptr, float* S_out = nullptr,
                    float* mult_out = nullptr, uint32_t* handoff_err = nullptr, bool keep_wside = false) {
#define FMX_LAUNCH_ZR(ZRV)                                                                                  \
  if constexpr (fused_zr_ok<KP>(ZRV)) {                                                                     \
    FMX_LAUNCH_WAVES((k_fused<KP, ZRV, VAR>), n_rows, st, s.ent, s.row_ptr, s.target, row0,                 \
                     n_rows, h->tb, hy, w0_in, rest_out, cmask, S_out, mult_out, s.fixed_nnz, handoff_err,                  \
                     (const uint64_t*)(keep_wside ? s.lmask : nullptr), keep_wside ? s.wside : (float*)nullptr); }
  switch (fused_zr_select<KP>(s.max_row)) {
    case 8:  FMX_LAUNCH_ZR(8);  break;
    case 16: FMX_LAUNCH_ZR(16); break;
    case 32: FMX_LAUNCH_ZR(32); break;
    case 40: FMX_LAUNCH_ZR(40); break;
    case 64: FMX_LAUNCH_ZR(64); break;
  }
#undef FMX_LAUNCH_ZR
  return FMX_OK;
}

}

extern "C++" uint32_t multi_group_size(const Slot& s, int KP) {
  if (KP < 64 || KP > 256 || s.n_rows == 0) return 0;
  const double avg = (double)s.nnz / (double)s.n_rows;
  if (avg > 12.0) return 0;
  static const double fill = []() { const char* e = getenv("FMX_MULTI_FILL"); const double f = e ? atof(e) : 0.0; return (f >= 8.0 && f <= 32.0) ? f : 24.0; }();
  const double g = avg > 0.0 ? fill / avg : (double)MULTI_GMAX;
  return (uint32_t)std::max(2.0, std::min((double)MULTI_GMAX, std::floor(g)));
}

extern "C" {

uint32_t fmx_default_w0_chunk(double learn_rate, int task) {
  const double curv = (task == FMX_TASK_REGRESSION) ? 1.0 : 0.25;
  const double lim = (learn_rate > 0) ? 1.0 / (learn_rate * curv) : (double)FMX_W0_CHUNK_CAP;
  uint32_t chunk = 1;
  while (chunk < (uint32_t)FMX_W0_CHUNK_CAP && (double)(chunk * 2) <= lim) chunk *= 2;
  return chunk;
}
int fmx_partial_floats(fmx_handle h, uint32_t batch, uint64_t* n_floats) {
  if (!h || !n_floats) return FMX_E_ARG;
  *n_floats = (uint64_t)batch * (uint64_t)(h->KP + 1);
  return FMX_OK;
}

int fmx_sgd_partial(fmx_handle h, int slot, uint64_t row0, uint32_t n_rows, float* d_partial, void* stream) {
  int rc = check_slot(h, slot, false);
  if (rc) return rc;
  const Slot& s = h->slots[slot];
  if (row0 + n_rows > s.n_rows) return fail(h, FMX_E_ARG, "fmx_sgd_partial: rows [%llu,+%u) outside slot (%u rows)",
                                            (unsigned long long)row0, n_rows, s.n_rows);
  if (!s.blocks.empty()) return fail(h, FMX_E_UNSUPPORTED, "relations are not supported with SGD");
  if (!d_partial) return fail(h, FMX_E_ARG, "fmx_sgd_partial: d_partial is NULL");
  if (n_rows == 0) return FMX_OK;
  HIPCHK(h, hipSetDevice(h->device));
  hipStream_t st = stream ? (hipStream_t)stream : h->stream;
  float* S = d_partial;
  float* c = d_partial + (size_t)n_rows * h->KP;
  return sgd_partial_rows(h, s, row0, n_rows, S, c, st);
}

extern "C++" int sgd_partial_rows(fmx_handle h, const Slot& s, uint64_t row0, uint32_t n_rows, float* S, float* c, hipStream_t st,
                                  const CompactState* snap) {
  if (n_rows == 0) return FMX_OK;
  if (snap) {
    KP_SWITCH(h->KP, FMX_LAUNCH_WAVES((k_rowsums<KP, true, false, RowsBf16>), n_rows, st, s.ent, s.row_ptr, row0, n_rows, compact_rows(h, *snap), h->cfg.k1, S, c));
    HIPCHK(h, hipGetLastError());
    return FMX_OK;
  }
  if (const uint32_t G = multi_group_size(s, h->KP)) {
    KP_SWITCH(h->KP, { if constexpr (KP >= 64 && KP <= 256) { FMX_LAUNCH_WAVES((k_rowsums_multi<KP, true, false>), ((uint64_t)n_rows + G - 1) / G, st,
                                                                  s.ent, s.row_ptr, row0, n_rows, h->tb, h->cfg.k1, S, c, G); } });
    HIPCHK(h, hipGetLastError());
    return FMX_OK;
  }
  KP_SWITCH(h->KP, FMX_LAUNCH_WAVES((k_rowsums<KP, true, false>), n_rows, st, s.ent, s.row_ptr, row0, n_rows, RowsF32{h->tb}, h->cfg.k1, S, c));
  HIPCHK(h, hipGetLastError());
  return FMX_OK;
}

extern "C++" int sgd_resolve_batch(fmx_handle h, Slot& s, const fmx_sgd_opts* opts, fmx_batch_info* bi) {
  const int slot = (int)(&s - h->slots);
  double C = 0.0;
  if (h->group && !h->owns_group && h->group->hs.size() > 1) {
    for (fmx_handle m : h->group->hs) {
      if (!m) return fail(h, FMX_E_STATE, "a member of the group was destroyed");
      int rc = ensure_coll_mass(m, m->slots[slot]);
      if (rc) { h->err = m->err; return rc; }
      C += m->slots[slot].coll_mass;
    }
  } else {
    int rc = ensure_coll_mass(h, s);
    if (rc) return rc;
    C = s.coll_mass;
    if (h->comm && h->cfg.shard_world > 1) {
      rc = comm_sum_double(h, &C);
      if (rc) return rc;
      s.coll_mass_world = C;
    }
  }
  resolve_batch(h->cfg, C, opts ? opts->batch : 0u, FMX_DEFAULT_BATCH, 1.0, bi);
  return FMX_OK;
}

int fmx_sgd_batch_info(fmx_handle h, int slot, const fmx_sgd_opts* opts, fmx_batch_info* out) {
  int rc = check_slot(h, slot, false);
  if (rc) return rc;
  if (!out) return fail(h, FMX_E_ARG, "fmx_sgd_batch_info: out is NULL");
  HIPCHK(h, hipSetDevice(h->device));
  return sgd_resolve_batch(h, h->slots[slot], opts, out);
}

extern "C++" int ensure_segments(fmx_handle h, Slot& s, uint32_t B) {
  if (s.seg_B == B && s.t_ent) return FMX_OK;
  if (&s >= h->slots && &s < h->slots + FMX_MAX_SLOTS) {
    int _rc = slot_in_session(h, (int)(&s - h->slots), "re-bucketing the rows for another batch size"); if (_rc) return _rc;
  }
  free_segments(s);
  const auto t_setup0 = std::chrono::steady_clock::now();
  static const bool trace = getenv("FMX_TRACE_SETUP") != nullptr;
  auto tp = [&](const char* what) { if (trace) { (void)hipStreamSynchronize(h->stream); fprintf(stderr, "[fmx setup] segments %-22s %8.3f ms\n", what,
                                     1e3 * std::chrono::duration<double>(std::chrono::steady_clock::now() - t_setup0).count()); } };
  struct Acc { fmx_handle h; std::chrono::steady_clock::time_point t0;
               ~Acc() { h->setup_acc += std::chrono::duration<double>(std::chrono::steady_clock::now() - t0).count(); } } acc_{h, t_setup0};
  const uint64_t nnz = s.nnz;
  const uint32_t n_batches = (s.n_rows + B - 1) / B;
  if (nnz >= (1ull << 31)) return fail(h, FMX_E_UNSUPPORTED, "segmented apply: nnz >= 2^31 in one slot (split the data set)");
  hipStream_t st = h->stream;
  uint32_t cap = 64;
  KP_SWITCH(h->KP, cap = fused_row_cap_kp<KP>(s.max_row));
  uint32_t fbits = 1; while (fbits < 32 && (1ull << fbits) < std::max<uint64_t>(h->n_local, 2)) fbits++;
  int bits_batch = 1; while ((1ull << bits_batch) < n_batches) bits_batch++;
  char* scratch = nullptr;
  int rc = FMX_OK;
  const size_t cnt = (size_t)std::max<uint64_t>(nnz, 1);
  const size_t nb1 = (size_t)n_batches + 1;
#define SEG_CHK(expr) do { hipError_t _e = (expr); if (_e != hipSuccess) { \
    rc = fail(h, FMX_E_HIP, "%s failed: %s", #expr, hipGetErrorString(_e)); goto done; } } while (0)
  {
    size_t tmp_sort = 0, tmp_scan = 0, tmp_xscan = 0;
    SEG_CHK(hipcub::DeviceRadixSort::SortPairs(nullptr, tmp_sort, (uint64_t*)nullptr, (uint64_t*)nullptr, (uint64_t*)nullptr, (uint64_t*)nullptr,
                                               (int)cnt, 0, (int)fbits + bits_batch, st));
    SEG_CHK(hipcub::DeviceScan::InclusiveSum(nullptr, tmp_scan, (uint32_t*)nullptr, (uint32_t*)nullptr, (int)cnt, st));
    SEG_CHK(hipcub::DeviceScan::ExclusiveSum(nullptr, tmp_xscan, (uint32_t*)nullptr, (uint32_t*)nullptr, (int)cnt, st));
    const size_t tmp_bytes = std::max<size_t>(std::max(tmp_sort, std::max(tmp_scan, tmp_xscan)), 256);
    auto al = [](size_t x) { return (x + 255) / 256 * 256; };
    size_t off = 0;
    const size_t o_ka = off; off += al(cnt * 8);
    const size_t o_kb = off; off += al(cnt * 8);
    const size_t o_va = off; off += al(cnt * 8);
    const size_t o_fl = off; off += al(cnt * 4);
    const size_t o_po = off; off += al(cnt * 4);
    const size_t o_cf = off; off += al(cnt * 4);
    const size_t o_cp = off; off += al(cnt * 4);
    const size_t o_ct = off; off += 256;
    const size_t o_tmp = off; off += al(tmp_bytes);
    SEG_CHK(fmx_dev_alloc(&scratch, off));
    uint64_t* keys_a = (uint64_t*)(scratch + o_ka); uint64_t* keys_b = (uint64_t*)(scratch + o_kb); uint64_t* vals_a = (uint64_t*)(scratch + o_va);
    uint32_t* flags = (uint32_t*)(scratch + o_fl); uint32_t* pos = (uint32_t*)(scratch + o_po);
    uint32_t* cflag = (uint32_t*)(scratch + o_cf); uint32_t* cpos = (uint32_t*)(scratch + o_cp);
    uint32_t* d_counts = (uint32_t*)(scratch + o_ct);
    void* tmp = scratch + o_tmp;
    uint64_t* vals_b = nullptr;
    SEG_CHK(fmx_dev_alloc(&vals_b, cnt * 8));
    s.t_ent = reinterpret_cast<TEntry*>(vals_b);
    SEG_CHK(fmx_dev_alloc(&s.cmask, (size_t)std::max<uint32_t>(s.n_rows, 1) * 8));
    SEG_CHK(fmx_dev_alloc(&s.d_batch_seg, nb1 * 4));
    SEG_CHK(fmx_dev_alloc(&s.d_cbatch, nb1 * 4));
    SEG_CHK(fmx_dev_alloc(&s.d_batch_base, nb1 * 8));
    tp("allocations");
    hipLaunchKernelGGL(k_seg_slow_rows, dim3(std::min<uint32_t>((s.n_rows + 255) / 256, 2048)), dim3(256), 0, st, s.row_ptr, s.n_rows, cap, s.cmask);
    s.fused_cap = cap;
    SEG_CHK(hipMemsetAsync(d_counts, 0, 16, st));
    if (nnz) {
      hipLaunchKernelGGL(k_seg_keys, dim3(wave_grid(s.n_rows)), dim3(256), 0, st, s.ent, s.row_ptr, s.n_rows, B, fbits, keys_a, vals_a, d_counts + 3);
      size_t tb_ = tmp_bytes;
      SEG_CHK(hipcub::DeviceRadixSort::SortPairs(tmp, tb_, keys_a, keys_b, vals_a, vals_b, (int)nnz, 0, (int)fbits + bits_batch, st));
      hipLaunchKernelGGL(k_seg_heads, dim3(2048), dim3(256), 0, st, keys_b, nnz, flags);
      tp("keys + sort + heads");
      tb_ = tmp_bytes;
      SEG_CHK(hipcub::DeviceScan::InclusiveSum(tmp, tb_, flags, pos, (int)nnz, st));
      hipLaunchKernelGGL(k_seg_batches, dim3((n_batches + 256) / 256), dim3(256), 0, st, pos, nnz, s.row_ptr, s.n_rows, B, n_batches, s.d_batch_seg, s.d_batch_base);
      uint32_t* head = reinterpret_cast<uint32_t*>(keys_a);
      hipLaunchKernelGGL(k_seg_head_pos, dim3(2048), dim3(256), 0, st, flags, pos, nnz, head);
      hipLaunchKernelGGL(k_seg_max_count, dim3(2048), dim3(256), 0, st, head, pos, nnz, d_counts + 2);
      hipLaunchKernelGGL(k_seg_mark, dim3(2048), dim3(256), 0, st, keys_b, reinterpret_cast<const TEntry*>(vals_b), head, pos, nnz,
                         s.ent, s.row_ptr, B, fbits, cap, (uint32_t)(s.max_row > cap ? 1u : 0u), s.cmask, cflag);
      SEG_CHK(hipGetLastError());
      tb_ = tmp_bytes;
      SEG_CHK(hipcub::DeviceScan::ExclusiveSum(tmp, tb_, cflag, cpos, (int)nnz, st));
      hipLaunchKernelGGL(k_seg_counts, dim3(1), dim3(64), 0, st, pos, nnz, cpos, cflag, d_counts + 2, d_counts);
      uint32_t counts[4] = {0, 0, 0, 0};
      SEG_CHK(hipMemcpyAsync(counts, d_counts, 16, hipMemcpyDeviceToHost, st));
      SEG_CHK(hipStreamSynchronize(st));
      tp("scan + mark + counts");
      const uint32_t nseg = counts[0];
      s.nseg = nseg; s.ncseg = counts[1]; s.max_seg_count = counts[2]; s.all_ones = counts[3] == 0u;
      SEG_CHK(fmx_dev_alloc(&s.seg_feat, (size_t)std::max<uint32_t>(nseg, 1) * 4));
      SEG_CHK(fmx_dev_alloc(&s.seg_rel, (size_t)std::max<uint32_t>(nseg, 1) * 4));
      SEG_CHK(fmx_dev_alloc(&s.cseg, (size_t)std::max<uint32_t>(s.ncseg, 1) * 4));
      SEG_CHK(fmx_dev_alloc(&s.cdesc, (size_t)std::max<uint32_t>(s.ncseg, 1) * sizeof(CDesc)));
      hipLaunchKernelGGL(k_seg_fill, dim3(2048), dim3(256), 0, st, keys_b, flags, pos, nnz, s.row_ptr, B, fbits, s.seg_feat, s.seg_rel);
      hipLaunchKernelGGL(k_seg_compact, dim3(2048), dim3(256), 0, st, keys_b, head, cflag, cpos, nseg, s.d_batch_seg, s.cseg,
                         s.seg_feat, s.seg_rel, s.row_ptr, s.n_rows, B, fbits, s.cdesc, reinterpret_cast<const TEntry*>(vals_b));
      hipLaunchKernelGGL(k_seg_cbatch, dim3((n_batches + 256) / 256), dim3(256), 0, st, cpos, cflag, nseg, s.d_batch_seg, n_batches, s.d_cbatch);
      SEG_CHK(hipGetLastError());
    } else {
      s.nseg = 0; s.ncseg = 0; s.max_seg_count = 0; s.all_ones = false;
      SEG_CHK(hipMemsetAsync(s.d_batch_seg, 0, nb1 * 4, st));
      SEG_CHK(hipMemsetAsync(s.d_cbatch, 0, nb1 * 4, st));
      SEG_CHK(hipMemsetAsync(s.d_batch_base, 0, nb1 * 8, st));
      SEG_CHK(fmx_dev_alloc(&s.seg_feat, 4)); SEG_CHK(fmx_dev_alloc(&s.seg_rel, 4));
      SEG_CHK(fmx_dev_alloc(&s.cseg, 4));
      SEG_CHK(fmx_dev_alloc(&s.cdesc, sizeof(CDesc)));
    }
    s.batch_seg.resize(nb1); s.cbatch.resize(nb1); s.batch_base.resize(nb1);
    SEG_CHK(hipMemcpyAsync(s.batch_seg.data(), s.d_batch_seg, nb1 * 4, hipMemcpyDeviceToHost, st));
    SEG_CHK(hipMemcpyAsync(s.cbatch.data(), s.d_cbatch, nb1 * 4, hipMemcpyDeviceToHost, st));
    SEG_CHK(hipMemcpyAsync(s.batch_base.data(), s.d_batch_base, nb1 * 8, hipMemcpyDeviceToHost, st));
    SEG_CHK(hipStreamSynchronize(st));
    tp("fill + compact + tables");
    s.seg_B = B;
  }
done:
#undef SEG_CHK
  if (scratch) fmx_dev_free(scratch);
  tp("frees");
  if (rc) free_segments(s);
  return rc;
}

static int take_error_bits(fmx_handle h, uint32_t mask, uint32_t* bits) {
  uint32_t e = 0;
  HIPCHK(h, hipMemcpy(&e, h->handoff_err, sizeof(uint32_t), hipMemcpyDeviceToHost));
  if (e & mask) {
    const uint32_t rest_bits = e & ~mask;
    (void)hipMemcpy(h->handoff_err, &rest_bits, sizeof(uint32_t), hipMemcpyHostToDevice);
  }
  *bits = e & mask;
  return FMX_OK;
}
extern "C++" int scan_error_check(fmx_handle h) {
  if (!h->pit_used) return FMX_OK;
  h->pit_used = false;
  uint32_t bits = 0;
  int rc = take_error_bits(h, 4u, &bits);
  if (rc) return rc;
  if (bits) {
    h->scan_pit = false;
    h->run_status |= FMX_STAT_SCAN_FALLBACK;
  }
  return FMX_OK;
}

extern "C++" bool streams_concurrent(fmx_handle h) {
  if (h->concurrent >= 0) return h->concurrent != 0;
  h->concurrent = 0;
  if (!h->probe_flags && fmx_dev_alloc(&h->probe_flags, 4 * sizeof(unsigned)) != hipSuccess) { (void)hipGetLastError(); return false; }
  unsigned res[4] = {0, 0, 0, 0};
  hipError_t e = hipMemsetAsync(h->probe_flags, 0, 4 * sizeof(unsigned), h->stream);
  if (e == hipSuccess) e = hipStreamSynchronize(h->stream);
  if (e == hipSuccess) e = hipStreamSynchronize(h->stream2);
  if (e == hipSuccess) {
    hipLaunchKernelGGL(k_concurrency_probe, dim3(1), dim3(64), 0, h->stream2, h->probe_flags, 1u);
    hipLaunchKernelGGL(k_concurrency_probe, dim3(1), dim3(64), 0, h->stream, h->probe_flags, 0u);
    e = hipGetLastError();
  }
  if (e == hipSuccess) e = hipStreamSynchronize(h->stream2);
  if (e == hipSuccess) e = hipStreamSynchronize(h->stream);
  if (e == hipSuccess) e = hipMemcpy(res, h->probe_flags, sizeof(res), hipMemcpyDeviceToHost);
  if (e != hipSuccess) { (void)hipGetLastError(); return false; }
  h->concurrent = (res[2] == 1u && res[3] == 1u) ? 1 : 0;
  return h->concurrent != 0;
}

static int raise_lds(fmx_handle h, const void* kf, size_t bytes) {
  if (h->lds_raised.count(kf)) return FMX_OK;
  HIPCHK(h, hipFuncSetAttribute((const void*)kf, hipFuncAttributeMaxDynamicSharedMemorySize, (int)bytes));
  h->lds_raised.insert(kf);
  return FMX_OK;
}
#define FMX_RAISE_LDS(kf, bytes) do { int _rc = raise_lds(h, (const void*)(kf), (bytes)); if (_rc) return _rc; } while (0)

static uint32_t pit_concurrent_kernels(fmx_handle h) {
  uint32_t n = 1;
  if (h->group && h->group->hs.size() > 1) {
    n = 0;
    for (fmx_handle m : h->group->hs) if (m && m->device == h->device) n++;
    if (n == 0) n = 1;
  }
  return n;
}

static int launch_scan(fmx_handle h, const float* rest, const float* target, uint32_t n_rows, uint32_t chunk,
                       const Hyper& hy, float* mult, hipStream_t st, const double* w0_in = nullptr, double* w0_out = nullptr,
                       const Handoff hw = Handoff{nullptr, 0ull, nullptr}, bool short_pit = false) {
  if (hy.k0) {
    const double* wi = w0_in ? w0_in : h->w0;
    double* wo = w0_out ? w0_out : h->w0;
    if (h->scan_pit && (n_rows > 4096u || (short_pit && n_rows >= 256u)) && chunk <= PIT_MAX_CHUNK && (chunk & (chunk - 1u)) == 0u) {
      if (h->pit_occ < 0) {
        int per_cu = 0;
        auto kf = k_scan_pit<false, 1>;
        (void)hipFuncSetAttribute((const void*)kf, hipFuncAttributeMaxDynamicSharedMemorySize, (int)PIT_LDS_BYTES);
        if (hipOccupancyMaxActiveBlocksPerMultiprocessor(&per_cu, (const void*)kf, 256, PIT_LDS_BYTES) != hipSuccess) { (void)hipGetLastError(); per_cu = 0; }
        h->pit_occ = per_cu * h->num_cu;
      }
      const uint32_t piece_rows = PIT_MAX_ROWS;
      const uint32_t nwg_max = (std::min(n_rows, piece_rows) + pit_seg(chunk) - 1) / pit_seg(chunk);
      static const bool trace_pit = getenv("FMX_TRACE_PIT") != nullptr;
      if (trace_pit) fprintf(stderr, "[fmx pit] rows %u chunk %u: %u workgroups x %u kernels, device holds %d\n", n_rows, chunk, nwg_max, pit_concurrent_kernels(h), h->pit_occ);
      if ((uint64_t)nwg_max * pit_concurrent_kernels(h) <= (uint64_t)std::max(h->pit_occ, 0)) {
        const uint32_t n_pieces = (n_rows + piece_rows - 1) / piece_rows;
        if (n_pieces > 1 && !h->pit_tmp) HIPCHK(h, fmx_dev_alloc(&h->pit_tmp, 64 * sizeof(double)));
        if (n_pieces <= 64) {
          const PitSync ps{h->pit_ctr, h->pit_slots, h->handoff_err, h->pit_spins};
          for (uint32_t pc = 0; pc < n_pieces; pc++) {
            const uint32_t r0 = pc * piece_rows, rn = std::min(piece_rows, n_rows - r0);
            const uint32_t nwg = (rn + pit_seg(chunk) - 1) / pit_seg(chunk);
            const double* pin = pc == 0 ? wi : h->pit_tmp + (pc - 1);
            double* pout = pc + 1 == n_pieces ? wo : h->pit_tmp + pc;
            Handoff ph{nullptr, 0ull, nullptr};
            if (hw.ctr) {
              if (pc == 0) ph = hw;
              else if (pc + 1 == n_pieces) ph = Handoff{hw.ctr, 0ull, hw.err};
            }
            HIPCHK(h, hipMemsetAsync(h->pit_ctr, 0, (PIT_MAX_IT + 1) * sizeof(unsigned long long), st));
            float* mp = mult ? mult + r0 : nullptr;
#define FMX_PIT(WM, TK) do { auto kf = k_scan_pit<WM, TK>;                                                                       \
            FMX_RAISE_LDS(kf, PIT_LDS_BYTES);                                                                                      \
            hipLaunchKernelGGL(kf, dim3(nwg), dim3(256), PIT_LDS_BYTES, st, rest + r0, target + r0, rn, chunk, hy, pin, pout, mp, ph, ps); } while (0)
            if (hy.task == 0) { if (mult) FMX_PIT(true, 0); else FMX_PIT(false, 0); }
            else              { if (mult) FMX_PIT(true, 1); else FMX_PIT(false, 1); }
#undef FMX_PIT
          }
          h->pit_used = true;
          h->run_status |= FMX_STAT_SCAN_PIT;
          HIPCHK(h, hipGetLastError());
          return FMX_OK;
        }
      }
    }
    h->run_status |= FMX_STAT_SCAN_SERIAL;
    const bool sub = chunk == 16u || chunk == 32u || chunk == 64u || chunk == 128u;
    const bool tiled = n_rows > 8192u && ((chunk % 256u) == 0 || sub);
#define FMX_SCAN1(WM, TK, C256) do { auto kf = k_scan1<WM, TK, C256>;                                                              \
      FMX_RAISE_LDS(kf, SCAN4_LDS_BYTES);                                                                                          \
      hipLaunchKernelGGL(kf, dim3(1), dim3(256), SCAN4_LDS_BYTES, st, rest, target, n_rows, chunk, hy, wi, wo, mult, hw); } while (0)
#define FMX_SCAN(WM, TK) do { \
      if (tiled && chunk == 256u) FMX_SCAN1(WM, TK, 256); \
      else if (tiled && chunk == 128u) FMX_SCAN1(WM, TK, 128); \
      else if (tiled && chunk == 64u)  FMX_SCAN1(WM, TK, 64); \
      else if (tiled && chunk == 32u)  FMX_SCAN1(WM, TK, 32); \
      else if (tiled && chunk == 16u)  FMX_SCAN1(WM, TK, 16); \
      else if (tiled)             FMX_SCAN1(WM, TK, 0); \
      else                        hipLaunchKernelGGL((k_scan<WM, TK>), dim3(1), dim3(64), 0, st, rest, target, n_rows, chunk, hy, wi, wo, mult, hw); } while (0)
    if (hy.task == 0) { if (mult) FMX_SCAN(true, 0); else FMX_SCAN(false, 0); }
    else              { if (mult) FMX_SCAN(true, 1); else FMX_SCAN(false, 1); }
#undef FMX_SCAN
#undef FMX_SCAN1
  } else if (mult) {
    hipLaunchKernelGGL(k_mult, dim3(std::min<uint32_t>((n_rows + 255) / 256, 2048)), dim3(256), 0, st, rest, target, n_rows, hy,
                       (const double*)nullptr, mult);
  }
  HIPCHK(h, hipGetLastError());
  return FMX_OK;
}

extern "C++" int lag_flush(fmx_handle h) {
  LagState& L = h->lag;
  if (!L.active) return FMX_OK;
  if (L.in_stream) { HIPCHK(h, hipStreamSynchronize(L.in_stream)); L.in_stream = nullptr; }
  HIPCHK(h, hipStreamSynchronize(h->stream2));
  HIPCHK(h, hipMemcpyAsync(h->w0, h->w0_pp + (L.step % (L.depth + 1)), sizeof(double), hipMemcpyDeviceToDevice, h->stream));
  HIPCHK(h, hipStreamSynchronize(h->stream));
  L.active = false; L.step = 0;
  return scan_error_check(h);
}
struct StepPlan {
  bool     lag;
  bool     short_rows;
  bool     from_sums;
  bool     in_stream;
  int      apply;
  int64_t  seg_batch;
  uint32_t chunk, depth;
};
static StepPlan step_plan(fmx_handle h, const Slot& s, const fmx_sgd_opts* opts, int64_t seg_batch, bool has_rest) {
  StepPlan p;
  p.apply = opts ? opts->apply : FMX_APPLY_DEFAULT; p.seg_batch = seg_batch;
  p.chunk = (opts && opts->w0_chunk) ? opts->w0_chunk : default_w0_chunk(h->cfg);
  p.depth = (opts && opts->bias_lag) ? opts->bias_lag : 1u;
  p.lag = opts && (opts->flags & FMX_FLAG_BIAS_LAG);
  p.short_rows = (p.apply == FMX_APPLY_DEFAULT || p.apply == FMX_APPLY_FUSED) && seg_batch >= 0 && s.cmask && !s.cbatch.empty() && multi_group_size(s, h->KP) != 0;
  p.from_sums = p.lag && p.short_rows && !has_rest;
  p.in_stream = p.from_sums && sgd_in_stream_batch(opts->batch, opts->flags);
  return p;
}
static int lag_prepare(fmx_handle h, hipStream_t st, const StepPlan& plan, int* slot) {
  LagState& L = h->lag;
  const uint32_t depth = plan.depth;
  if (!L.ev_rest) {
    HIPCHK(h, hipEventCreateWithFlags(&L.ev_rest, hipEventDisableTiming));
    for (auto& e : L.ev_scan) HIPCHK(h, hipEventCreateWithFlags(&e, hipEventDisableTiming));
  }
  if (L.active && L.depth != depth) { int rc = lag_flush(h); if (rc) return rc; }
  if (!L.active) {
    L.depth = depth;
    for (uint32_t r = 0; r <= depth; r++) HIPCHK(h, hipMemcpyAsync(h->w0_pp + r, h->w0, sizeof(double), hipMemcpyDeviceToDevice, st));
    L.active = true; L.step = 0;
  } else if (L.step > depth && !plan.in_stream) {
    HIPCHK(h, hipStreamWaitEvent(st, L.ev_scan[(L.step - depth - 1) % LagState::RING], 0));
  }
  *slot = (int)(L.step % (depth + 1));
  return FMX_OK;
}
static int lag_wait_bias(fmx_handle h, const Hyper& hy, hipStream_t st) {
  LagState& L = h->lag;
  if (hy.k0 && L.step >= L.depth) HIPCHK(h, hipStreamWaitEvent(st, L.ev_scan[(L.step - L.depth) % LagState::RING], 0));
  return FMX_OK;
}
static const double* lag_bias_slot(fmx_handle h) {
  const LagState& L = h->lag;
  const uint32_t R = L.depth + 1;
  return h->w0_pp + ((L.step + R - L.depth + 1) % R);
}
static int lag_start_scan(fmx_handle h, const float* rest, const float* target, uint32_t n_rows, uint32_t chunk, const Hyper& hy, hipStream_t st) {
  LagState& L = h->lag;
  const uint64_t b = L.step;
  const uint32_t R = L.depth + 1;
  if (hy.k0) {
    HIPCHK(h, hipEventRecord(L.ev_rest, st));
    HIPCHK(h, hipStreamWaitEvent(h->stream2, L.ev_rest, 0));
    int rc = launch_scan(h, rest, target, n_rows, chunk, hy, nullptr, h->stream2, h->w0_pp + (b % R), h->w0_pp + ((b + 1) % R)); if (rc) return rc;
    HIPCHK(h, hipEventRecord(L.ev_scan[b % LagState::RING], h->stream2));
  }
  return FMX_OK;
}
static int lag_step(fmx_handle h, const float* rest, const float* target, uint32_t n_rows, uint32_t chunk,
                    const Hyper& hy, hipStream_t st) {
  int rc = lag_start_scan(h, rest, target, n_rows, chunk, hy, st); if (rc) return rc;
  rc = lag_wait_bias(h, hy, st); if (rc) return rc;
  hipLaunchKernelGGL(k_mult, dim3(std::min<uint32_t>((n_rows + 255) / 256, 2048)), dim3(256), 0, st, rest, target, n_rows, hy,
                     lag_bias_slot(h), h->mult);
  HIPCHK(h, hipGetLastError());
  h->lag.step++;
  return FMX_OK;
}

static SegWork seg_work(fmx_handle, const Slot& s, size_t b, const float* S, const float* mult) {
  const uint32_t c0 = s.cbatch[b], c1 = s.cbatch[b + 1], s0 = s.batch_seg[b], s1 = s.batch_seg[b + 1];
  const uint64_t base = s.batch_base[b];
  return SegWork{s.t_ent + base, s.seg_feat + s0, s.seg_rel + s0, s.cseg + c0, c1 - c0, s1 - s0, (uint32_t)(s.batch_base[b + 1] - base), S, mult,
                 s.cdesc + c0, nullptr, 0ull};
}
static SegWork seg_work_dense(fmx_handle, const Slot& s, size_t b, const float* S, const float* mult) {
  const uint32_t s0 = s.batch_seg[b], nseg = s.batch_seg[b + 1] - s0;
  const uint64_t base = s.batch_base[b];
  return SegWork{s.t_ent + base, s.seg_feat + s0, s.seg_rel + s0, nullptr, nseg, nseg, (uint32_t)(s.batch_base[b + 1] - base), S, mult, nullptr, nullptr, 0ull};
}
static int launch_deferred(fmx_handle h, const Slot& s, const Hyper& hy, const float* S, size_t b, hipStream_t st) {
  const SegWork sw = seg_work(h, s, b, S, h->mult);
  if (sw.nseg) { KP_SWITCH(h->KP, FMX_LAUNCH_WAVES((k_apply_seg<KP, 8, 16>), ((uint64_t)sw.nseg + 15) / 16, st, sw, h->tb, hy)); }
  return FMX_OK;
}
static int launch_apply_multi(fmx_handle h, const Slot& s, const Hyper& hy, uint64_t row0, uint32_t n_rows, bool fused, const double* bias,
                              const float* S, const float* cpart, float* rest, hipStream_t st) {
  const uint32_t G = multi_group_size(s, h->KP);
  KP_SWITCH(h->KP, { if constexpr (KP >= 64 && KP <= 256) { FMX_LAUNCH_WAVES((fused ? k_apply_multi<KP, true> : k_apply_multi<KP, false>), ((uint64_t)n_rows + G - 1) / G, st,
                                                                s.ent, s.row_ptr, s.target, row0, n_rows, h->tb, hy, bias, S, cpart, rest, h->mult, (const uint64_t*)s.cmask, G); } });
  return FMX_OK;
}
static int launch_apply(fmx_handle h, const Slot& s, const Hyper& hy, uint64_t row0, uint32_t n_rows, const float* S, const StepPlan& p,
                        hipStream_t st, hipEvent_t ev_a) {
  int apply = p.apply, rc = FMX_OK;
  const bool masked = (apply == FMX_APPLY_DEFAULT || apply == FMX_APPLY_FUSED) && s.cmask && !s.cbatch.empty() && s.nnz >= (uint64_t)24 * s.n_rows;
  if (apply == FMX_APPLY_DEFAULT || apply == FMX_APPLY_FUSED) apply = FMX_APPLY_SEGMENTED;
  if (apply == FMX_APPLY_SEGMENTED && p.seg_batch < 0) return fail(h, FMX_E_STATE, "segmented apply needs batch-aligned rows");
  if (ev_a) HIPCHK(h, hipEventRecord(ev_a, st));
  if (apply == FMX_APPLY_SEGMENTED && masked) {
    KP_SWITCH(h->KP, rc = (launch_fused_zr<KP, FUSED_APPLY>(h, s, hy, row0, n_rows, st, (const double*)h->w0, nullptr,
                                                               (const uint64_t*)s.cmask, const_cast<float*>(S), h->mult)));
    if (rc) return rc;
    return launch_deferred(h, s, hy, S, (size_t)p.seg_batch, st);
  } else if (apply == FMX_APPLY_SEGMENTED) {
    const SegWork sw = seg_work_dense(h, s, (size_t)p.seg_batch, S, h->mult);
    if (sw.nseg) { KP_SWITCH(h->KP, FMX_LAUNCH_WAVES((k_apply_seg<KP, 8, 64>), ((uint64_t)sw.nseg + 63) / 64, st, sw, h->tb, hy)); }
  } else if (apply == FMX_APPLY_ATOMIC || apply == FMX_APPLY_STORE) {
    const bool atomic = apply == FMX_APPLY_ATOMIC;
    KP_SWITCH(h->KP, FMX_LAUNCH_WAVES((atomic ? k_apply<KP, true> : k_apply<KP, false>), n_rows, st, s.ent, s.row_ptr, row0, n_rows, h->tb, hy, S, h->mult));
  } else {
    return fail(h, FMX_E_ARG, "unknown apply mode %d", apply);
  }
  return FMX_OK;
}
static int sgd_finish_impl(fmx_handle h, const Slot& s, uint64_t row0, uint32_t n_rows, const float* S, float* rest, const float* cpart,
                           const StepPlan& p, hipStream_t st, hipEvent_t ev_a, hipEvent_t ev_b) {
  const Hyper hy = make_hyper(h->cfg);
  const float* target = s.target + row0;
  int rc = FMX_OK;
  if (p.in_stream) {
    const LagState& L = h->lag;
    const uint32_t R = L.depth + 1;
    if (ev_a) HIPCHK(h, hipEventRecord(ev_a, st));
    rc = launch_apply_multi(h, s, hy, row0, n_rows, true, lag_bias_slot(h), S, cpart, rest, st); if (rc) return rc;
    const SegWork sw = seg_work(h, s, (size_t)p.seg_batch, S, h->mult);
    const ScanSmall sc{rest, target, h->w0_pp + (L.step % R), h->w0_pp + ((L.step + 1) % R), n_rows, p.chunk};
    KP_SWITCH(h->KP, hipLaunchKernelGGL((k_apply_seg_scan<KP, 8, 1>), dim3((sw.nseg + 3) / 4 + 1), dim3(256), 0, st, sw, h->tb, hy, sc));
    h->lag.step++; h->lag.in_stream = st;
    h->run_status |= FMX_STAT_SCAN_SERIAL;
  } else if (p.from_sums) {
    rc = lag_wait_bias(h, hy, st); if (rc) return rc;
    if (ev_a) HIPCHK(h, hipEventRecord(ev_a, st));
    rc = launch_apply_multi(h, s, hy, row0, n_rows, true, lag_bias_slot(h), S, cpart, rest, st); if (rc) return rc;
    HIPCHK(h, hipGetLastError());
    rc = lag_start_scan(h, rest, target, n_rows, p.chunk, hy, st); if (rc) return rc;
    h->lag.step++;
    rc = launch_deferred(h, s, hy, S, (size_t)p.seg_batch, st); if (rc) return rc;
  } else {
    rc = p.lag ? lag_step(h, rest, target, n_rows, p.chunk, hy, st) : launch_scan(h, rest, target, n_rows, p.chunk, hy, h->mult, st);
    if (rc) return rc;
    if (p.short_rows) {
      if (ev_a) HIPCHK(h, hipEventRecord(ev_a, st));
      rc = launch_apply_multi(h, s, hy, row0, n_rows, false, (const double*)h->w0, S, nullptr, nullptr, st); if (rc) return rc;
      HIPCHK(h, hipGetLastError());
      rc = launch_deferred(h, s, hy, S, (size_t)p.seg_batch, st); if (rc) return rc;
    } else {
      rc = launch_apply(h, s, hy, row0, n_rows, S, p, st, ev_a); if (rc) return rc;
    }
  }
  if (ev_b) HIPCHK(h, hipEventRecord(ev_b, st));
  HIPCHK(h, hipGetLastError());
  return FMX_OK;
}

int fmx_sgd_finish(fmx_handle h, int slot, uint64_t row0, uint32_t n_rows, const float* d_partial,
                   const fmx_sgd_opts* opts, void* stream) {
  touch_w(h);
  int rc = check_slot(h, slot, true); if (rc) return rc;
  Slot& s = h->slots[slot];
  if (row0 + n_rows > s.n_rows) return fail(h, FMX_E_ARG, "fmx_sgd_finish: rows outside slot");
  if (!s.blocks.empty()) return fail(h, FMX_E_UNSUPPORTED, "relations are not supported with SGD");
  if (!d_partial) return fail(h, FMX_E_ARG, "fmx_sgd_finish: d_partial is NULL");
  if (((uintptr_t)d_partial & 15u) != 0) return fail(h, FMX_E_ARG, "fmx_sgd_finish: d_partial must be 16-byte aligned");
  if (n_rows == 0) return FMX_OK;
  HIPCHK(h, hipSetDevice(h->device));
  hipStream_t st = stream ? (hipStream_t)stream : h->stream;
  const uint32_t Bcap = (opts && opts->batch) ? std::max(opts->batch, n_rows) : n_rows;
  const uint32_t lag_depth = (opts && opts->bias_lag) ? opts->bias_lag : 1u;
  if (lag_depth > 4) return fail(h, FMX_E_ARG, "bias_lag %u: at most 4 batches", lag_depth);
  rc = ensure_scratch(h, n_rows, (size_t)Bcap * (lag_depth + 1)); if (rc) return rc;
  const float* S = d_partial;
  const float* c = d_partial + (size_t)n_rows * h->KP;
  int64_t seg_batch = -1;
  const int apply = opts ? opts->apply : FMX_APPLY_DEFAULT;
  if (apply == FMX_APPLY_DEFAULT || apply == FMX_APPLY_SEGMENTED || apply == FMX_APPLY_FUSED) {
    const uint32_t B = (opts && opts->batch) ? opts->batch : n_rows;
    if (row0 % B != 0 || n_rows > B || n_rows != std::min<uint64_t>(B, s.n_rows - row0))
      return fail(h, FMX_E_ARG, "fmx_sgd_finish: rows [%llu,+%u) are not batch %u of the slot", (unsigned long long)row0, n_rows, B);
    rc = ensure_segments(h, h->slots[slot], B); if (rc) return rc;
    seg_batch = (int64_t)(row0 / B);
  }
  const StepPlan plan = step_plan(h, s, opts, seg_batch, false);
  int rslot = 0;
  if (plan.lag) { rc = lag_prepare(h, st, plan, &rslot); if (rc) return rc; }
  else { rc = lag_flush(h); if (rc) return rc; }
  float* rest_buf = h->rest + (size_t)rslot * Bcap;
  if (!plan.from_sums) {
    KP_SWITCH(h->KP, hipLaunchKernelGGL((k_rest_from_partial<KP>), dim3(wave_grid((n_rows + Map<KP>::EPI - 1) / Map<KP>::EPI)),
                                          dim3(256), 0, st, S, c, n_rows, rest_buf));
    HIPCHK(h, hipGetLastError());
  }
  return sgd_finish_impl(h, s, row0, n_rows, S, rest_buf, c, plan, st, nullptr, nullptr);
}

int fmx_predict_finish(fmx_handle h, uint32_t n_rows, const float* d_partial, float* d_yhat, void* stream) {
  if (!h || !d_partial || !d_yhat) return FMX_E_ARG;
  if (((uintptr_t)d_partial & 15u) != 0) return fail(h, FMX_E_ARG, "fmx_predict_finish: d_partial must be 16-byte aligned");
  { int _rc = lag_flush(h); if (_rc) return _rc; }
  if (n_rows == 0) return FMX_OK;
  HIPCHK(h, hipSetDevice(h->device));
  hipStream_t st = stream ? (hipStream_t)stream : h->stream;
  int rc = ensure_scratch(h, 0, n_rows);
  if (rc) return rc;
  const float* S = d_partial;
  const float* c = d_partial + (size_t)n_rows * h->KP;
  KP_SWITCH(h->KP, hipLaunchKernelGGL((k_rest_from_partial<KP>), dim3(wave_grid((n_rows + Map<KP>::EPI - 1) / Map<KP>::EPI)),
                                        dim3(256), 0, st, S, c, n_rows, h->rest));
  hipLaunchKernelGGL(k_yhat, dim3(std::min<uint32_t>((n_rows + 255) / 256, 2048)), dim3(256), 0, st,
                     h->rest, n_rows, h->cfg.k0, h->w0, d_yhat);
  HIPCHK(h, hipGetLastError());
  return FMX_OK;
}

struct EpochCounts { uint64_t batches = 0, launches = 0, deferred = 0; bool kept_wside = false; };

struct FusedEpoch {
  fmx_handle h; Slot* s; Hyper hy;
  uint32_t B, Bc, d, chunk; uint64_t n_batch;
  bool keep, handoff;
  double* W; unsigned long long hbase;
  int szr, small_cap;
  unsigned long long* small_trace;
};
static uint32_t rows_of_batch(const FusedEpoch& E, uint64_t b) { return (uint32_t)std::min<uint64_t>(E.B, E.s->n_rows - b * E.B); }
static const char* small_trace_file() { static const char* f = getenv("FMX_SMALL_TRACE"); return f; }
static int small_trace_arm(fmx_handle h, hipStream_t st, unsigned long long** trace) {
  if (!small_trace_file()) return FMX_OK;
  *trace = h->small_slots + (size_t)3 * SMALL_ONE_MAX;
  unsigned long long init[16];
  for (int i = 0; i < 16; i++) init[i] = (i == 0 || i == 5) ? ~0ull : 0ull;
  HIPCHK(h, hipMemcpyAsync(*trace, init, sizeof(init), hipMemcpyHostToDevice, st));
  HIPCHK(h, hipStreamSynchronize(st));
  return FMX_OK;
}
static int small_trace_dump(fmx_handle h, hipStream_t st, const unsigned long long* trace, uint64_t n_batch) {
  unsigned long long tr[16];
  HIPCHK(h, hipMemcpyAsync(tr, trace, sizeof(tr), hipMemcpyDeviceToHost, st));
  HIPCHK(h, hipStreamSynchronize(st));
  if (FILE* f = fopen(small_trace_file(), "a")) {
    const double t0 = (double)tr[0];
    fprintf(f, "batch %llu of %llu (ns after the first example started): last example started %.0f, rows gathered %.0f, multiplier published %.0f, example done %.0f | "
               "first owner started %.0f, last owner saw its tags %.0f, holds its S rows %.0f, done %.0f | recurrence done %.0f | last owner started %.0f, has its entry list %.0f\n",
            (unsigned long long)(n_batch / 2), (unsigned long long)n_batch, tr[1] - t0, tr[2] - t0, tr[3] - t0, tr[4] - t0, (double)tr[5] - t0, tr[6] - t0, tr[7] - t0, tr[8] - t0, tr[9] - t0, tr[10] - t0, tr[11] - t0);
    fclose(f);
  }
  return FMX_OK;
}
static int fused_batch_one_launch(FusedEpoch& E, uint64_t b, EpochCounts* n) {
  fmx_handle h = E.h; const Slot& s = *E.s; const Hyper& hy = E.hy;
  const uint32_t B = E.B, d = E.d, chunk = E.chunk, nb = rows_of_batch(E, b);
  const uint64_t row0 = b * B, n_batch = E.n_batch;
  float* S = h->partial;
  const SegWork sw = seg_work(h, s, (size_t)b, S, h->mult + (size_t)(b & 1) * E.Bc);
  n->deferred += sw.nseg;
  const bool defer = d >= 2u;
  const bool own = !defer || b + 1 == n_batch, prev = defer && b >= 1;
  const ScanSmall sc{nullptr, s.target + row0, h->w0_pp + (b % d), h->w0_pp + ((b + 1) % d), own ? nb : 0u, chunk};
  const ScanSmall sc_prev{nullptr, s.target + (prev ? row0 - B : 0), h->w0_pp + ((b + d - 1) % d), h->w0_pp + (b % d), prev ? B : 0u, chunk};
  unsigned long long* rs0 = h->small_slots + SMALL_ONE_MAX;
  const SmallSync sy{h->small_slots, rs0 + (size_t)(b & 1) * SMALL_ONE_MAX, rs0 + (size_t)((b + 1) & 1) * SMALL_ONE_MAX, (uint32_t)(b + 1), (uint32_t)b,
                     h->handoff_err, std::min<uint32_t>(h->pit_spins, 1u << 21), (E.small_trace && b == n_batch / 2) ? E.small_trace : nullptr};
  const uint32_t n_ex_wg = (nb + 3u) / 4u;
  bool launched = false;
#define FMX_SMALL1(KPV, ZRV) do { if (h->KP == KPV && E.szr == ZRV) {                                                                    \
    auto kf = k_small_one<KPV, ZRV>;                                                                                                       \
    if (!E.small_cap) {                                                                                                                    \
      int per_cu = 0;                                                                                                                      \
      if (hipOccupancyMaxActiveBlocksPerMultiprocessor(&per_cu, (const void*)kf, 256, 0) != hipSuccess) { (void)hipGetLastError(); per_cu = 0; } \
      E.small_cap = std::max(1, per_cu * h->num_cu);                                                                                       \
    }                                                                                                                                      \
    const uint32_t room = (uint32_t)E.small_cap > n_ex_wg + 1u ? (uint32_t)E.small_cap - n_ex_wg - 1u : 1u;                                \
    const uint32_t own_wg = sw.nseg ? std::max(1u, std::min((sw.nseg + 3u) / 4u, room)) : 0u;                                              \
    hipLaunchKernelGGL(kf, dim3(n_ex_wg + own_wg + 1u), dim3(256), 0, h->stream, s.ent, s.row_ptr, s.target, row0, nb, h->tb, hy,          \
                       (const double*)(h->w0_pp + ((b + 1) % d)), (const uint64_t*)s.cmask, S, s.fixed_nnz, sw, sc_prev, sc, sy, n_ex_wg,  \
                       (const uint64_t*)(E.keep ? s.lmask : nullptr), E.keep ? s.wside : (float*)nullptr);                                 \
    launched = true; } } while (0)
  FMX_SMALL1(8, 8);    FMX_SMALL1(16, 16);  FMX_SMALL1(32, 32);
  FMX_SMALL1(64, 16);  FMX_SMALL1(64, 40);  FMX_SMALL1(64, 64);
  FMX_SMALL1(128, 16); FMX_SMALL1(128, 40); FMX_SMALL1(128, 64);
#undef FMX_SMALL1
  if (!launched) return fail(h, FMX_E_STATE, "no one-launch instance for %d factors and %d row slots", h->KP, E.szr);
  HIPCHK(h, hipGetLastError());
  h->small_one_used = true;
  h->run_status |= FMX_STAT_SMALL_ONE;
  return FMX_OK;
}
static int fused_examples(const FusedEpoch& E, uint64_t b, const double* w0_in, float* rest, SegWork* sw, EpochCounts* n) {
  fmx_handle h = E.h; const Slot& s = *E.s;
  float* S = h->partial + (size_t)(b & 1) * E.Bc * (size_t)(h->KP + 1);
  float* mult = h->mult + (size_t)(b & 1) * E.Bc;
  int rc = FMX_OK;
  KP_SWITCH(h->KP, { rc = launch_fused_zr<KP, FUSED_EXACT>(h, s, E.hy, b * E.B, rows_of_batch(E, b), h->stream, w0_in, rest, s.cmask, S, mult,
                                                             E.handoff ? h->handoff_err : nullptr, E.keep); });
  if (rc) return rc;
  HIPCHK(h, hipGetLastError());
  *sw = seg_work(h, s, (size_t)b, S, mult);
  n->deferred += sw->nseg;
  return FMX_OK;
}
static int fused_batch_in_stream(const FusedEpoch& E, uint64_t b, EpochCounts* n) {
  fmx_handle h = E.h; const Slot& s = *E.s;
  const uint32_t d = E.d;
  float* rest = h->rest + (size_t)(b % d) * E.Bc;
  SegWork sw;
  int rc = fused_examples(E, b, h->w0_pp + ((b + 1) % d), rest, &sw, n); if (rc) return rc;
  const ScanSmall sc{rest, s.target + b * E.B, h->w0_pp + (b % d), h->w0_pp + ((b + 1) % d), rows_of_batch(E, b), E.chunk};
  KP_SWITCH(h->KP, hipLaunchKernelGGL((k_apply_seg_scan<KP, 8, 1>), dim3((sw.nseg + 3) / 4 + 1), dim3(256), 0, h->stream, sw, h->tb, E.hy, sc));
  HIPCHK(h, hipGetLastError());
  return FMX_OK;
}
static int fused_batch_side(const FusedEpoch& E, uint64_t b, EpochCounts* n) {
  fmx_handle h = E.h; const Slot& s = *E.s; const Hyper& hy = E.hy;
  hipStream_t st = h->stream;
  const uint32_t d = E.d, nb = rows_of_batch(E, b);
  const uint64_t row0 = b * E.B;
  const bool handoff = E.handoff;
  float* rest = h->rest + (size_t)(handoff ? b % (d + 1) : b % d) * E.Bc;
  if (!handoff && b >= d) HIPCHK(h, hipStreamWaitEvent(st, h->ev_sync[2 * (b - d) + 1], 0));
  const double* w0_in = handoff ? E.W + (b + 1 >= d ? b + 1 - d : 0)
                                : h->w0_pp + ((b + 1) % d);
  SegWork sw;
  int rc = fused_examples(E, b, w0_in, rest, &sw, n); if (rc) return rc;
  if (!handoff) HIPCHK(h, hipEventRecord(h->ev_sync[2 * b], st));
  if (handoff) { sw.done_ctr = h->handoff_ctr; sw.done_val = E.hbase + b + 1; }
  if (handoff && !sw.nseg) hipLaunchKernelGGL(k_handoff_signal, dim3(1), dim3(64), 0, st, h->handoff_ctr, E.hbase + b + 1);
  if (sw.nseg) {
    if (sw.nseg >= 16u * 2048u)     { KP_SWITCH(h->KP, FMX_LAUNCH_WAVES((k_apply_seg<KP, 8, 16>), ((uint64_t)sw.nseg + 15) / 16, st, sw, h->tb, hy)); }
    else if (sw.nseg >= 4u * 2048u) { KP_SWITCH(h->KP, FMX_LAUNCH_WAVES((k_apply_seg<KP, 8, 4>), ((uint64_t)sw.nseg + 3) / 4, st, sw, h->tb, hy)); }
    else                            { KP_SWITCH(h->KP, FMX_LAUNCH_WAVES((k_apply_seg<KP, 8, 1>), (uint64_t)sw.nseg, st, sw, h->tb, hy)); }
    HIPCHK(h, hipGetLastError());
  }
  if (handoff)
    return launch_scan(h, rest, s.target + row0, nb, E.chunk, hy, nullptr, h->stream2, E.W + b, E.W + b + 1,
                       Handoff{h->handoff_ctr, E.hbase + b + 1, h->handoff_err});
  HIPCHK(h, hipStreamWaitEvent(h->stream2, h->ev_sync[2 * b], 0));
  rc = launch_scan(h, rest, s.target + row0, nb, E.chunk, hy, nullptr, h->stream2, h->w0_pp + (b % d), h->w0_pp + ((b + 1) % d)); if (rc) return rc;
  HIPCHK(h, hipEventRecord(h->ev_sync[2 * b + 1], h->stream2));
  return FMX_OK;
}
static int sgd_epoch_fused(fmx_handle h, Slot& s, const fmx_sgd_opts* opts, const Hyper& hy, EpochCounts* n) {
  FusedEpoch E{h, &s, hy};
  const uint32_t B = E.B = opts->batch;
  const uint32_t d = E.d = opts->bias_lag ? opts->bias_lag : 1u;
  if (d > 4) return fail(h, FMX_E_ARG, "bias_lag %u: at most 4 batches", d);
  E.chunk = opts->w0_chunk ? opts->w0_chunk : default_w0_chunk(h->cfg);
  int rc = ensure_segments(h, s, B); if (rc) return rc;
  const bool keep_wside = (opts->flags & FMX_FLAG_KEEP_WSIDE) && hy.k1 && h->cfg.shard_world == 1 && s.blocks.empty();
  if (keep_wside) { rc = ensure_wside(h, s); if (rc) return rc; }
  n->kept_wside = E.keep = keep_wside && s.wside != nullptr;
  const uint32_t Bc = E.Bc = std::min<uint32_t>(B, s.n_rows);
  rc = ensure_scratch(h, (size_t)Bc * 2, (size_t)Bc * (d + 1)); if (rc) return rc;
  const uint64_t n_batch = E.n_batch = ((uint64_t)s.n_rows + B - 1) / B;
  const bool side = B >= FMX_SIDE_STREAM_BATCH;
  const bool handoff = E.handoff = side && h->handoff && hy.k0 && d >= 2 && !(opts->flags & FMX_FLAG_EVENT_SYNC) && streams_concurrent(h);
  if (side && hy.k0 && !handoff) h->run_status |= FMX_STAT_EVENT_SYNC;
  if (!side && hy.k0) h->run_status |= FMX_STAT_SCAN_SERIAL;
  if (handoff) {
    if (h->w0_slots_cap < n_batch + 1) {
      if (h->w0_slots) HIPCHK(h, fmx_dev_free(h->w0_slots));
      h->w0_slots = nullptr; h->w0_slots_cap = 0;
      HIPCHK(h, fmx_dev_alloc(&h->w0_slots, (size_t)(n_batch + 1) * sizeof(double)));
      h->w0_slots_cap = n_batch + 1;
    }
    E.W = h->w0_slots;
    E.hbase = h->handoff_seq; h->handoff_seq += n_batch + 1;
  }
  if (side && !handoff) while (h->ev_sync.size() < 2 * n_batch + 1) { hipEvent_t e; HIPCHK(h, hipEventCreateWithFlags(&e, hipEventDisableTiming)); h->ev_sync.push_back(e); }
  hipStream_t st = h->stream;
  HIPCHK(h, hipEventRecord(h->ev0, st));
  for (uint32_t r = 0; r < d; r++) HIPCHK(h, hipMemcpyAsync(h->w0_pp + r, h->w0, sizeof(double), hipMemcpyDeviceToDevice, st));
  if (handoff) {
    hipLaunchKernelGGL(k_handoff_arm, dim3((unsigned)std::min<uint64_t>((n_batch + 255) / 256, 64)), dim3(256), 0, st, E.W, (uint32_t)n_batch);
    HIPCHK(h, hipMemcpyAsync(E.W, h->w0, sizeof(double), hipMemcpyDeviceToDevice, st));
  }
  const bool small_one = !side && h->small_one && (h->KP == 8 || h->KP == 16 || h->KP == 32 || h->KP == 64 || h->KP == 128) && s.cdesc && Bc <= SMALL_ONE_MAX && !hy.sgda;
  if (small_one) {
    if (h->KP < 64) E.szr = h->KP;
    else {
      E.szr = (h->KP == 64) ? fused_zr_select<64>(s.max_row) : fused_zr_select<128>(s.max_row);
      if (E.szr == 8) E.szr = 16;
      if (E.szr == 32) E.szr = 40;
    }
    if (!h->small_slots) HIPCHK(h, fmx_dev_alloc(&h->small_slots, ((size_t)3 * SMALL_ONE_MAX + 16) * sizeof(unsigned long long)));
    HIPCHK(h, hipMemsetAsync(h->small_slots, 0, (size_t)3 * SMALL_ONE_MAX * sizeof(unsigned long long), st));
    HIPCHK(h, hipMemsetAsync(h->partial, 0, (size_t)Bc * (size_t)h->KP * sizeof(unsigned long long), st));
    rc = small_trace_arm(h, st, &E.small_trace); if (rc) return rc;
  }
  for (uint64_t b = 0; b < n_batch; b++) {
    rc = small_one ? fused_batch_one_launch(E, b, n) : side ? fused_batch_side(E, b, n) : fused_batch_in_stream(E, b, n); if (rc) return rc;
    n->batches++; n->launches++;
  }
  if (E.small_trace) { rc = small_trace_dump(h, st, E.small_trace, n_batch); if (rc) return rc; }
  if (handoff) {
    if (h->ev_sync.empty()) { hipEvent_t e; HIPCHK(h, hipEventCreateWithFlags(&e, hipEventDisableTiming)); h->ev_sync.push_back(e); }
    HIPCHK(h, hipEventRecord(h->ev_sync[0], h->stream2));
    HIPCHK(h, hipStreamWaitEvent(st, h->ev_sync[0], 0));
    HIPCHK(h, hipMemcpyAsync(h->w0, E.W + n_batch, sizeof(double), hipMemcpyDeviceToDevice, st));
    HIPCHK(h, hipMemcpyAsync(&h->handoff_err_host, h->handoff_err, sizeof(uint32_t), hipMemcpyDeviceToHost, st));
    return FMX_OK;
  }
  if (side) HIPCHK(h, hipStreamWaitEvent(st, h->ev_sync[2 * (n_batch - 1) + 1], 0));
  if (hy.k0) HIPCHK(h, hipMemcpyAsync(h->w0, h->w0_pp + (n_batch % d), sizeof(double), hipMemcpyDeviceToDevice, st));
  return FMX_OK;
}

static int ensure_runs(fmx_handle h, Slot& s) {
  if (!s.run_start.empty()) return FMX_OK;
  struct Acc { fmx_handle h; std::chrono::steady_clock::time_point t0;
               ~Acc() { h->setup_acc += std::chrono::duration<double>(std::chrono::steady_clock::now() - t0).count(); } } acc_{h, std::chrono::steady_clock::now()};
  const uint32_t n = s.n_rows;
  if (n == 0 || n >= 0x7FFFFFFEu || s.nnz >= (1ull << 31)) { s.run_start = {0u, n}; s.run_single = {2u}; return FMX_OK; }
  hipStream_t st = h->stream;
  std::vector<uint32_t> prev(n, 0u);
  if (s.nnz) {
    uint32_t fbits = 1; while (fbits < 32 && (1ull << fbits) < std::max<uint64_t>(h->n_local, 2)) fbits++;
    size_t tmp_bytes = 0;
    HIPCHK(h, hipcub::DeviceRadixSort::SortKeys(nullptr, tmp_bytes, (uint64_t*)nullptr, (uint64_t*)nullptr, (int)s.nnz, 0, 32 + (int)fbits, st));
    auto al = [](size_t x) { return (x + 255) / 256 * 256; };
    const size_t o_a = 0, o_b = al(s.nnz * 8), o_p = o_b + al(s.nnz * 8), o_t = o_p + al((size_t)n * 4), total = o_t + al(std::max<size_t>(tmp_bytes, 256));
    char* scratch = nullptr;
    HIPCHK(h, fmx_dev_alloc(&scratch, total));
    uint64_t* ka = (uint64_t*)(scratch + o_a); uint64_t* kb = (uint64_t*)(scratch + o_b); uint32_t* d_prev = (uint32_t*)(scratch + o_p);
    hipError_t e = hipMemsetAsync(d_prev, 0, (size_t)n * 4, st);
    if (e == hipSuccess) {
      hipLaunchKernelGGL(k_run_keys, dim3(wave_grid(n)), dim3(256), 0, st, s.ent, s.row_ptr, n, ka);
      size_t tb_ = tmp_bytes;
      e = hipcub::DeviceRadixSort::SortKeys(scratch + o_t, tb_, ka, kb, (int)s.nnz, 0, 32 + (int)fbits, st);
    }
    if (e == hipSuccess) {
      hipLaunchKernelGGL(k_run_prev, dim3(2048), dim3(256), 0, st, kb, s.nnz, d_prev);
      e = hipGetLastError();
    }
    if (e == hipSuccess) e = hipMemcpyAsync(prev.data(), d_prev, (size_t)n * 4, hipMemcpyDeviceToHost, st);
    if (e == hipSuccess) e = hipStreamSynchronize(st);
    fmx_dev_free(scratch);
    if (e != hipSuccess) return fail(h, FMX_E_HIP, "ensure_runs failed: %s", hipGetErrorString(e));
  }
  std::vector<uint32_t> starts; std::vector<uint8_t> single;
  uint32_t start = 0;
  for (uint32_t r = 0; r < n; r++) {
    const bool rep = (prev[r] & 0x80000000u) != 0;
    const uint32_t p = prev[r] & 0x7FFFFFFFu;
    if (rep) {
      if (r > start) { starts.push_back(start); single.push_back(0); }
      starts.push_back(r); single.push_back(1);
      start = r + 1;
    } else if ((p > start && r > start) || r - start >= 4096u) {
      starts.push_back(start); single.push_back(0);
      start = r;
    }
  }
  if (start < n) { starts.push_back(start); single.push_back(0); }
  starts.push_back(n);
  s.run_start.swap(starts); s.run_single.swap(single);
  return FMX_OK;
}
static int launch_run_one(fmx_handle h, const Slot& s, const Hyper& hy, uint32_t row0, uint32_t nb, int zr, const double* bias_in, double* bias_out,
                          unsigned long long* slots, uint32_t tag) {
  hipStream_t st = h->stream;
  const size_t lds = (size_t)nb * 5 * sizeof(float);
  const dim3 grid((nb + 3u) / 4u);
  const RunSync rs{slots, tag, h->handoff_err, std::min<uint32_t>(h->pit_spins, 1u << 21)};
  int launched = 0;
#define FMX_RUN1(KPV, ZRV, TK) do { if (h->KP == KPV && zr == ZRV && hy.task == TK) {                                                    \
    auto kf = k_run_fused<KPV, ZRV, TK>;                                                                                                 \
    auto it = h->run_one_occ.find((const void*)kf);                                                                                      \
    if (it == h->run_one_occ.end()) {                                                                                                    \
      int per_cu = 0;                                                                                                                    \
      if (hipOccupancyMaxActiveBlocksPerMultiprocessor(&per_cu, (const void*)kf, 256, (size_t)RUN_ONE_MAX * 5 * sizeof(float)) != hipSuccess) { (void)hipGetLastError(); per_cu = 0; } \
      it = h->run_one_occ.emplace((const void*)kf, per_cu * h->num_cu).first;                                                            \
    }                                                                                                                                    \
    if ((int)grid.x <= it->second) {                                                                                                     \
      hipLaunchKernelGGL(kf, grid, dim3(256), lds, st, s.ent, s.row_ptr, s.target, (uint64_t)row0, nb, h->tb, hy, bias_in, bias_out, rs, s.fixed_nnz); \
      launched = 1; } } } while (0)
  FMX_RUN1(8, 8, 0);    FMX_RUN1(16, 16, 0);  FMX_RUN1(32, 32, 0);  FMX_RUN1(8, 8, 1);    FMX_RUN1(16, 16, 1);  FMX_RUN1(32, 32, 1);
  FMX_RUN1(64, 16, 0);  FMX_RUN1(64, 40, 0);  FMX_RUN1(64, 64, 0);  FMX_RUN1(64, 16, 1);  FMX_RUN1(64, 40, 1);  FMX_RUN1(64, 64, 1);
  FMX_RUN1(128, 16, 0); FMX_RUN1(128, 40, 0); FMX_RUN1(128, 64, 0); FMX_RUN1(128, 16, 1); FMX_RUN1(128, 40, 1); FMX_RUN1(128, 64, 1);
#undef FMX_RUN1
  return launched;
}

static int seq_runs_epoch(fmx_handle h, Slot& s, const Hyper& hy) {
  hipStream_t st = h->stream;
  const bool fused = h->seq_runs_fused, one_env = h->seq_runs_one;
  uint32_t longest = 1;
  for (size_t i = 0; i + 1 < s.run_start.size(); i++) longest = std::max(longest, s.run_start[i + 1] - s.run_start[i]);
  int rc = ensure_scratch(h, longest, 0);
  if (rc) return rc;
  if (!h->pit_tmp) HIPCHK(h, fmx_dev_alloc(&h->pit_tmp, 64 * sizeof(double)));
  double* bias[2] = {h->w0, h->pit_tmp + 48};
  if (!h->run_slots) HIPCHK(h, fmx_dev_alloc(&h->run_slots, (size_t)RUN_ONE_MAX * sizeof(unsigned long long)));
  unsigned long long* slots = h->run_slots;
  int zr = 0;
  bool one = fused && one_env && h->run_one && (h->KP == 8 || h->KP == 16 || h->KP == 32 || h->KP == 64 || h->KP == 128) && s.max_row <= 64u;
  if (one && h->KP < 64) zr = h->KP;
  else if (one) {
    zr = (h->KP == 64) ? fused_zr_select<64>(s.max_row) : fused_zr_select<128>(s.max_row);
    if (s.max_row > (uint32_t)zr) one = false;
    if (zr == 8) zr = 16;
    if (zr == 32) zr = 40;
  }
  if (one) HIPCHK(h, hipMemsetAsync(slots, 0, (size_t)RUN_ONE_MAX * sizeof(unsigned long long), st));
  int cur = 0;
  for (size_t i = 0; i + 1 < s.run_start.size(); i++) {
    const uint32_t row0 = s.run_start[i], nb = s.run_start[i + 1] - row0;
    if (s.run_single[i]) {
      KP_SWITCH(h->KP, hipLaunchKernelGGL((k_sequential<KP>), dim3(1), dim3(64), 0, st, s.ent, s.row_ptr + row0, s.target + row0, nb, h->tb, hy, bias[cur]));
      h->run_status |= FMX_STAT_SEQ_ENTRIES;
      continue;
    }
    if (one && nb <= RUN_ONE_MAX) {
      rc = launch_run_one(h, s, hy, row0, nb, zr, bias[cur], bias[cur ^ 1], slots, (uint32_t)i + 1u);
      if (rc < 0) return rc;
      if (rc == 1) { h->run_one_used = true; h->run_status |= FMX_STAT_RUN_ONE; if (hy.k0) cur ^= 1; continue; }
    }
    float* S = h->partial;
    float* rest = S + (size_t)nb * h->KP;
    KP_SWITCH(h->KP, FMX_LAUNCH_WAVES((k_rowsums<KP, true, true>), nb, st, s.ent, s.row_ptr, (uint64_t)row0, nb, RowsF32{h->tb}, h->cfg.k1, S, rest));
    if (fused && nb <= RUN_FUSED_MAX) {
      const dim3 grid((nb + 3u) / 4u);
      const size_t lds = (size_t)nb * 5 * sizeof(float);
      if (hy.task == 0) { KP_SWITCH(h->KP, hipLaunchKernelGGL((k_run_apply<KP, 0>), grid, dim3(256), lds, st, s.ent, s.row_ptr, (uint64_t)row0, nb, h->tb, hy, S, rest, s.target, bias[cur], bias[cur ^ 1])); }
      else              { KP_SWITCH(h->KP, hipLaunchKernelGGL((k_run_apply<KP, 1>), grid, dim3(256), lds, st, s.ent, s.row_ptr, (uint64_t)row0, nb, h->tb, hy, S, rest, s.target, bias[cur], bias[cur ^ 1])); }
      h->run_status |= FMX_STAT_RUN_TWO;
      if (hy.k0) cur ^= 1;
      continue;
    }
    h->run_status |= FMX_STAT_RUN_THREE;
    rc = launch_scan(h, rest, s.target + row0, nb, 1u, hy, h->mult, st, bias[cur], bias[cur], Handoff{nullptr, 0ull, nullptr}, fused);
    if (rc) return rc;
    KP_SWITCH(h->KP, FMX_LAUNCH_WAVES((k_apply<KP, false>), nb, st, s.ent, s.row_ptr, (uint64_t)row0, nb, h->tb, hy, S, h->mult));
  }
  if (cur) HIPCHK(h, hipMemcpyAsync(h->w0, bias[1], sizeof(double), hipMemcpyDeviceToDevice, st));
  HIPCHK(h, hipGetLastError());
  return FMX_OK;
}

static int epoch_sequential(fmx_handle h, Slot& s, const Hyper& hy, EpochCounts* n) {
  const bool seq_rows = h->seq_rows, seq_wg = h->seq_wg;
  const char* sr = getenv("FMX_SEQ_RUNS");
  bool use_runs = !(sr && sr[0] == '0');
  int rc = FMX_OK;
  if (use_runs) {
    rc = ensure_runs(h, s); if (rc) return rc;
    const size_t n_runs = s.run_start.size() - 1;
    use_runs = !(s.run_single.size() == 1 && s.run_single[0] == 2) && ((sr && sr[0] == '1') || (uint64_t)s.n_rows >= 16ull * n_runs);
    HIPCHK(h, hipEventRecord(h->ev0, h->stream));
  }
  if (use_runs) {
    rc = seq_runs_epoch(h, s, hy); if (rc) return rc;
    h->run_status |= FMX_STAT_SEQ_RUNS;
  } else if (seq_rows && seq_wg && h->KP <= 128) {
    auto kf = h->KP <= 64 ? k_sequential_wg<64> : k_sequential_wg<128>;
    const size_t lds = h->KP <= 64 ? sizeof(SeqLds<64>) : sizeof(SeqLds<128>);
    FMX_RAISE_LDS(kf, lds);
    hipLaunchKernelGGL(kf, dim3(1), dim3(64 * SEQ_W), lds, h->stream, s.ent, s.row_ptr, s.target, s.n_rows, s.nnz, h->tb, hy, h->w0);
    h->run_status |= FMX_STAT_SEQ_WG;
  } else if (seq_rows && h->KP <= 128) {
    h->run_status |= FMX_STAT_SEQ_ROWS;
    const bool wide = s.max_row > 32u;
    auto kf = h->KP <= 64 ? (wide ? k_sequential_rows<64, 64> : k_sequential_rows<64, 32>) : (wide ? k_sequential_rows<128, 64> : k_sequential_rows<128, 32>);
    hipLaunchKernelGGL(kf, dim3(1), dim3(64), 0, h->stream, s.ent, s.row_ptr, s.target, s.n_rows, h->tb, hy, h->w0);
  } else {
    KP_SWITCH(h->KP, hipLaunchKernelGGL((k_sequential<KP>), dim3(1), dim3(64), 0, h->stream, s.ent, s.row_ptr,
                                          s.target, s.n_rows, h->tb, hy, h->w0));
    h->run_status |= FMX_STAT_SEQ_ENTRIES;
  }
  HIPCHK(h, hipGetLastError());
  n->batches = use_runs ? s.run_start.size() - 1 : s.n_rows;
  n->launches = 1;
  return FMX_OK;
}
static int epoch_hogwild(fmx_handle h, Slot& s, const fmx_sgd_opts* opts, const Hyper& hy, EpochCounts* n) {
  if (opts->apply == FMX_APPLY_SEGMENTED) return fail(h, FMX_E_ARG, "HOGWILD has no segmented apply");
  const uint32_t M = opts->batch ? opts->batch : 262144u;
  const uint32_t chunk = opts->w0_chunk ? opts->w0_chunk : default_w0_chunk(h->cfg);
  const uint32_t cap = std::min<uint32_t>(M, s.n_rows);
  int rc = ensure_scratch(h, 0, (size_t)cap * 3); if (rc) return rc;
  const uint64_t n_launch = ((uint64_t)s.n_rows + M - 1) / M;
  while (h->ev_sync.size() < 2 * n_launch) { hipEvent_t e; HIPCHK(h, hipEventCreateWithFlags(&e, hipEventDisableTiming)); h->ev_sync.push_back(e); }
  for (int r = 0; r < 3; r++) HIPCHK(h, hipMemcpyAsync(h->w0_pp + r, h->w0, sizeof(double), hipMemcpyDeviceToDevice, h->stream));
  for (uint64_t i = 0; i < n_launch; i++) {
    const uint64_t row0 = i * M;
    const uint32_t nb = (uint32_t)std::min<uint64_t>(M, s.n_rows - row0);
    float* rest = h->rest + (size_t)(i % 3) * cap;
    hipStream_t fs = h->stream;
    if (i >= 3) HIPCHK(h, hipStreamWaitEvent(fs, h->ev_sync[2 * (i - 3) + 1], 0));
    n->launches++;
    const double* w0_in = h->w0_pp + ((i + 1) % 3);
    if (opts->apply == FMX_APPLY_ATOMIC) {
      KP_SWITCH(h->KP, { rc = launch_fused_zr<KP, FUSED_ATOMIC>(h, s, hy, row0, nb, fs, w0_in, rest); });
    } else {
      KP_SWITCH(h->KP, { rc = launch_fused_zr<KP, FUSED_STORE>(h, s, hy, row0, nb, fs, w0_in, rest); });
    }
    if (rc) return rc;
    HIPCHK(h, hipGetLastError());
    HIPCHK(h, hipEventRecord(h->ev_sync[2 * i], fs));
    HIPCHK(h, hipStreamWaitEvent(h->stream2, h->ev_sync[2 * i], 0));
    rc = launch_scan(h, rest, s.target + row0, nb, chunk, hy, nullptr, h->stream2, h->w0_pp + (i % 3), h->w0_pp + ((i + 1) % 3)); if (rc) return rc;
    HIPCHK(h, hipEventRecord(h->ev_sync[2 * i + 1], h->stream2));
    n->batches++;
  }
  HIPCHK(h, hipStreamWaitEvent(h->stream, h->ev_sync[2 * (n_launch - 1) + 1], 0));
  if (hy.k0) HIPCHK(h, hipMemcpyAsync(h->w0, h->w0_pp + (n_launch % 3), sizeof(double), hipMemcpyDeviceToDevice, h->stream));
  return FMX_OK;
}
static int epoch_split(fmx_handle h, Slot& s, const fmx_sgd_opts* opts, EpochCounts* n) {
  const uint32_t B = opts->batch;
  const bool timed = (opts->flags & FMX_FLAG_TIME_MAIN_KERNEL) != 0;
  const bool segmented = (opts->apply == FMX_APPLY_DEFAULT || opts->apply == FMX_APPLY_SEGMENTED);
  const uint32_t lag_depth = opts->bias_lag ? opts->bias_lag : 1u;
  if (lag_depth > 4) return fail(h, FMX_E_ARG, "bias_lag %u: at most 4 batches", lag_depth);
  const uint32_t Bc = std::min<uint32_t>(B, s.n_rows);
  int rc = ensure_scratch(h, (size_t)Bc * ((opts->flags & FMX_FLAG_BIAS_LAG) ? lag_depth + 1 : 1), 0); if (rc) return rc;
  if (segmented) {
    rc = ensure_segments(h, s, B); if (rc) return rc;
    HIPCHK(h, hipEventRecord(h->ev0, h->stream));
  }
  StepPlan plan = step_plan(h, s, opts, segmented ? 0 : -1, true);
  while (timed && h->ev_pool.size() < 2 * (((size_t)s.n_rows + B - 1) / B)) { hipEvent_t e; HIPCHK(h, hipEventCreate(&e)); h->ev_pool.push_back(e); }
  for (uint64_t row0 = 0; row0 < s.n_rows; row0 += B) {
    const uint32_t nb = (uint32_t)std::min<uint64_t>(B, s.n_rows - row0);
    int pslot = 0;
    if (plan.lag) { rc = lag_prepare(h, h->stream, plan, &pslot); if (rc) return rc; }
    float* S = h->partial + (size_t)pslot * Bc * (size_t)(h->KP + 1);
    float* rest = S + (size_t)nb * h->KP;
    KP_SWITCH(h->KP, FMX_LAUNCH_WAVES((k_rowsums<KP, true, true>), nb, h->stream,
                                       s.ent, s.row_ptr, row0, nb, RowsF32{h->tb}, h->cfg.k1, S, rest));
    hipEvent_t ea = nullptr, eb = nullptr;
    if (timed) { ea = h->ev_pool[2 * n->launches]; eb = h->ev_pool[2 * n->launches + 1]; n->launches++; }
    if (segmented) plan.seg_batch = (int64_t)(row0 / B);
    rc = sgd_finish_impl(h, s, row0, nb, S, rest, nullptr, plan, h->stream, ea, eb); if (rc) return rc;
    n->batches++;
  }
  return FMX_OK;
}

static int epoch_close(fmx_handle h, Slot& s, const fmx_sgd_opts* opts, const fmx_batch_info& bi, const EpochCounts& n, fmx_epoch_stats* stats) {
  if (h->lag.active)
    HIPCHK(h, hipStreamWaitEvent(h->stream, h->lag.ev_scan[(h->lag.step - 1) % LagState::RING], 0));
  HIPCHK(h, hipEventRecord(h->ev1, h->stream));
  HIPCHK(h, hipStreamSynchronize(h->stream));
  HIPCHK(h, hipGetLastError());
  int rc = lag_flush(h); if (rc) return rc;
  rc = scan_error_check(h); if (rc) return rc;
  uint32_t bits = 0;
  const struct { bool* used; bool* enabled; const char* text; } one_launch[2] = {
    {&h->small_one_used, &h->small_one,
     "a one-launch batch never saw all of its examples (the device is shared or partitioned): the features concerned took no "
     "step (the parameters are valid numbers, the epoch is not the batch rule's) -- reload the parameters; the handle takes "
     "two launches per batch from now on"},
    {&h->run_one_used, &h->run_one,
     "a conflict-free run never saw all of its workgroups (the device is shared or partitioned): the rows concerned took no "
     "step (the parameters are valid numbers, the epoch is not the reference's) -- reload the parameters; the handle takes "
     "two launches per run from now on"}};
  for (const auto& o : one_launch) {
    if (!*o.used) continue;
    *o.used = false;
    rc = take_error_bits(h, RUN_ERR_EXCHANGE, &bits); if (rc) return rc;
    if (!bits) continue;
    *o.enabled = false;
    h->run_status |= FMX_STAT_HANDOFF_TIMEOUT;
    if (stats) stats->status = bi.status | h->run_status;
    return fail(h, FMX_E_HIP, "%s", o.text);
  }
  if (h->handoff_err_host & 3u) {
    const uint32_t e = h->handoff_err_host;
    h->handoff_err_host = 0;
    (void)take_error_bits(h, 3u, &bits);
    h->handoff = false;
    h->run_status |= FMX_STAT_HANDOFF_TIMEOUT;
    if (stats) stats->status = bi.status | h->run_status;
    return fail(h, FMX_E_HIP, "the bias hand-off between the launch stream and the recurrence timed out (flags %u): the examples concerned took no "
                              "step (the parameters are valid numbers, the epoch is not the batch rule's); the handle orders its streams with "
                              "events from now on", e);
  }
  if (n.kept_wside) s.wside_version = h->w_version;
  if (stats) {
    float ms = 0;
    HIPCHK(h, hipEventElapsedTime(&ms, h->ev0, h->ev1));
    stats->rows = s.n_rows; stats->batches = n.batches; stats->device_seconds = ms * 1e-3;
    if (opts->mode == FMX_SGD_MINIBATCH && s.seg_B) stats->max_feature_count = s.max_seg_count;
    stats->deferred_features = n.deferred;
    if (opts->mode == FMX_SGD_MINIBATCH || opts->mode == FMX_SGD_HOGWILD) {
      stats->batch_used = bi.batch; stats->collision_mass = bi.collision_mass; stats->batch_gain = bi.batch_gain; stats->status = bi.status;
    }
    stats->status |= h->run_status;
    stats->setup_seconds = h->setup_acc;
    if (opts->mode != FMX_SGD_SEQUENTIAL) stats->w0_chunk_used = opts->w0_chunk ? opts->w0_chunk : default_w0_chunk(h->cfg);
    stats->main_kernel_seconds = stats->device_seconds;
    stats->main_kernel_launches = n.launches;
    if (opts->mode == FMX_SGD_MINIBATCH && (opts->flags & FMX_FLAG_TIME_MAIN_KERNEL) && opts->apply != FMX_APPLY_FUSED) {
      double tot = 0;
      for (size_t i = 0; i < n.launches; i++) {
        float m2 = 0;
        HIPCHK(h, hipEventElapsedTime(&m2, h->ev_pool[2 * i], h->ev_pool[2 * i + 1]));
        tot += m2 * 1e-3;
      }
      stats->main_kernel_seconds = tot;
    }
  }
  return FMX_OK;
}

int fmx_sgd_epoch(fmx_handle h, int slot, const fmx_sgd_opts* opts, fmx_epoch_stats* stats) {
  int rc = check_slot(h, slot, true); if (rc) return rc;
  { int _rc = lag_flush(h); if (_rc) return _rc; }
  if (!opts) return fail(h, FMX_E_ARG, "fmx_sgd_epoch: opts is NULL");
  HIPCHK(h, hipSetDevice(h->device));
  Slot& s = h->slots[slot];
  if (stats) memset(stats, 0, sizeof(*stats));
  if (s.n_rows == 0) return FMX_OK;
  if (!s.blocks.empty()) return fail(h, FMX_E_UNSUPPORTED, "relations are not supported with SGD");
  if (!(h->group && !h->owns_group)) { h->setup_acc = 0.0; h->run_status = 0; }
  if (h->cfg.shard_world > 1 && opts->mode != FMX_SGD_MINIBATCH)
    return fail(h, FMX_E_UNSUPPORTED, "feature shards train with FMX_SGD_MINIBATCH (the split step)");
  if (h->cfg.shard_world > 1 || h->comm) return comm_sgd_epoch(h, slot, opts, stats);
  const Hyper hy = make_hyper(h->cfg);
  fmx_sgd_opts ropts = *opts;
  fmx_batch_info bi; memset(&bi, 0, sizeof(bi));
  if (opts->mode == FMX_SGD_MINIBATCH) {
    rc = sgd_resolve_batch(h, s, opts, &bi); if (rc) return rc;
    if ((opts->flags & FMX_FLAG_REJECT_UNSTABLE) && (bi.status & FMX_STAT_UNSTABLE)) {
      if (opts->batch == 0)
        return fail(h, FMX_E_ARG, "these rows are too dense for the batch rule: at the smallest batch the library takes (%u rows) learn_rate * "
                                  "curvature * batch * collision mass = %.3g > 2 (collision mass %.4g) -- lower learn_rate or train with "
                                  "FMX_SGD_SEQUENTIAL", bi.batch, bi.batch_gain, bi.collision_mass);
      return fail(h, FMX_E_ARG, "batch %u on these rows: learn_rate * curvature * batch * collision mass = %.3g > 2 -- the batch rule "
                                "diverges (collision mass %.4g; batch 0 lets the library choose)", bi.batch, bi.batch_gain, bi.collision_mass);
    }
    ropts.batch = bi.batch;
    opts = &ropts;
  } else if (opts->mode == FMX_SGD_HOGWILD) {
    rc = ensure_coll_mass(h, s); if (rc) return rc;
    const uint32_t in_flight = (uint32_t)std::min<uint64_t>(s.n_rows, (uint64_t)20 * (uint64_t)h->num_cu);
    resolve_batch(h->cfg, s.coll_mass, in_flight, in_flight, 1.0, &bi);
    if ((opts->flags & FMX_FLAG_REJECT_UNSTABLE) && (bi.status & FMX_STAT_UNSTABLE))
      return fail(h, FMX_E_ARG, "HOGWILD on these rows: learn_rate * curvature * %u rows in flight * collision mass = %.3g > 2 -- the asynchronous "
                                "step diverges (collision mass %.4g; use FMX_SGD_MINIBATCH with batch 0)", in_flight, bi.batch_gain, bi.collision_mass);
  }
  touch_w(h);
  HIPCHK(h, hipEventRecord(h->ev0, h->stream));
  EpochCounts n;
  switch (opts->mode) {
    case FMX_SGD_SEQUENTIAL: rc = epoch_sequential(h, s, hy, &n); break;
    case FMX_SGD_HOGWILD:    rc = epoch_hogwild(h, s, opts, hy, &n); break;
    case FMX_SGD_MINIBATCH:  rc = opts->apply == FMX_APPLY_FUSED ? sgd_epoch_fused(h, s, opts, hy, &n) : epoch_split(h, s, opts, &n); break;
    default: return fail(h, FMX_E_ARG, "unknown SGD mode %d", opts->mode);
  }
  if (rc) return rc;
  return epoch_close(h, s, opts, bi, n, stats);
}

extern "C++" void sgda_free(fmx_handle h) {
  if (h->sgda.gw) fmx_dev_free(h->sgda.gw);
  if (h->sgda.gv) fmx_dev_free(h->sgda.gv);
  if (h->sgda.reg) fmx_dev_free(h->sgda.reg);
  if (h->sgda.dreg) fmx_dev_free(h->sgda.dreg);
  h->sgda = SgdaState();
// ... 421 lines not shown
```

Before: 277.6 million.

## Recycle spare physical memory chunks between arena pool and big allocations

Adds a per-device pool of spare physical memory handles. Leftover pool chunks from arena construction and chunks from freed big allocations are kept in it and reused by later big allocations instead of creating new physical memory. Big reservations are also rounded up to whole chunks. The change also moves ensure_segments and ensure_runs into their own source files and adds setup tracing; it targets setup/allocation overhead rather than the training kernel, and it adds bookkeeping and lifetime risk around the shared handles.

```diff
diff --git a/libfm_amd/build.py b/libfm_amd/build.py
--- a/libfm_amd/build.py
+++ b/libfm_amd/build.py
@@ -6,7 +6,7 @@
 HERE = os.path.dirname(os.path.abspath(__file__))
 ROOT = os.path.dirname(HERE)
 CSRC = os.path.join(HERE, "csrc")
-SRC = [os.path.join(CSRC, f) for f in ("fmx_core.hip", "fmx_sgd.hip", "fmx_als.hip", "fmx_io.hip", "fmx_comm.hip", "fmx_pair.hip", "fmx_topk.hip", "fmx_pairneg.hip", "fmx_eval.hip", "fmx_post.hip", "fmx_evalq.hip", "fmx_compact.hip", "fmx_rankq.hip", "fmx_mem.hip")]
+SRC = [os.path.join(CSRC, f) for f in ("fmx_core.hip", "fmx_sgd.hip", "fmx_seg.hip", "fmx_runs.hip", "fmx_als.hip", "fmx_io.hip", "fmx_comm.hip", "fmx_pair.hip", "fmx_topk.hip", "fmx_pairneg.hip", "fmx_eval.hip", "fmx_post.hip", "fmx_evalq.hip", "fmx_compact.hip", "fmx_rankq.hip", "fmx_mem.hip")]
 DEPS = SRC + sorted(os.path.join(CSRC, f) for f in os.listdir(CSRC) if f.endswith(".h")) + [os.path.join(ROOT, "include", "fmx.h")]
 EXTRA = os.environ.get("FMX_DEFS", "").split()
 OUT = os.path.join(HERE, os.environ.get("FMX_OUT", "libfmx.so"))
diff --git a/libfm_amd/csrc/fmx_core.hip b/libfm_amd/csrc/fmx_core.hip
--- a/libfm_amd/csrc/fmx_core.hip
+++ b/libfm_amd/csrc/fmx_core.hip
@@ -242,11 +242,16 @@
   struct Acc { fmx_handle h; std::chrono::steady_clock::time_point t0;
                ~Acc() { h->setup_acc += std::chrono::duration<double>(std::chrono::steady_clock::now() - t0).count(); } } acc_{h, std::chrono::steady_clock::now()};
   HIPCHK(h, hipSetDevice(h->device));
+  static const bool trace = getenv("FMX_TRACE_SETUP") != nullptr;
+  auto tp = [&](const char* what) { if (trace) { (void)hipStreamSynchronize(h->stream); fprintf(stderr, "[fmx setup] collision mass %-16s %8.3f ms\n", what,
+                                     1e3 * std::chrono::duration<double>(std::chrono::steady_clock::now() - acc_.t0).count()); } };
   const uint32_t M = (uint32_t)std::min<uint64_t>(std::max<uint64_t>(h->n_local, 1), 1ull << 27);
   double* hist = nullptr;
   HIPCHK(h, fmx_dev_alloc(&hist, (size_t)M * sizeof(double)));
+  tp("allocation");
   hipError_t er = hipMemsetAsync(hist, 0, (size_t)M * sizeof(double), h->stream);
   if (er == hipSuccess) er = hipMemsetAsync(h->acc, 0, 2 * sizeof(double), h->stream);
+  tp("zero fill");
   if (er == hipSuccess) {
     hipLaunchKernelGGL(k_coll_hist, dim3((unsigned)std::min<uint64_t>((s.nnz + 255) / 256, 8192)), dim3(256), 0, h->stream, s.ent, s.nnz, M, hist, h->acc + 1);
     hipLaunchKernelGGL(k_coll_sumsq, dim3((unsigned)std::min<uint64_t>(((uint64_t)M + 255) / 256, 4096)), dim3(256), 0, h->stream,
@@ -256,7 +261,9 @@
   double c[2] = {0.0, 0.0};
   if (er == hipSuccess) er = hipMemcpyAsync(c, h->acc, 2 * sizeof(double), hipMemcpyDeviceToHost, h->stream);
   if (er == hipSuccess) er = hipStreamSynchronize(h->stream);
+  tp("histogram + sum");
   fmx_dev_free(hist);
+  tp("free");
   if (er != hipSuccess) return fail(h, FMX_E_HIP, "collision mass of the rows: %s", hipGetErrorString(er));
   const double N = (double)s.n_rows;
   s.coll_mass = (s.n_rows > 1) ? std::max(0.0, c[0] - c[1]) / (N * (N - 1.0)) : 0.0;
diff --git a/libfm_amd/csrc/fmx_internal.h b/libfm_amd/csrc/fmx_internal.h
--- a/libfm_amd/csrc/fmx_internal.h
+++ b/libfm_amd/csrc/fmx_internal.h
@@ -233,6 +233,7 @@
 int evaluate_out(fmx_handle h, const Slot& s, const CompactState* snap, fmx_eval* out);
 inline RowsBf16 compact_rows(fmx_handle h, const CompactState& c) { return RowsBf16{CTab{c.V, c.w, h->tb.rs}}; }
 int ensure_segments(fmx_handle h, Slot& s, uint32_t B);
+int ensure_runs(fmx_handle h, Slot& s);
 int ensure_coll_mass(fmx_handle h, Slot& s);
 int ensure_wside(fmx_handle h, Slot& s);
 inline void touch_w(fmx_handle h) { if (h) h->w_version++; }
@@ -384,3 +385,15 @@
     case 1024: { constexpr int KP = 1024; __VA_ARGS__; } break;        \
     default: return fail(h, FMX_E_UNSUPPORTED, "num_factor > 1024 is not supported");   \
   }
+
+template <int KP> constexpr bool fused_zr_ok(int zr) { return Map<KP>::VEC * zr <= 128; }
+template <int KP> inline int fused_zr_select(uint32_t max_row) {
+  constexpr int EPI = Map<KP>::EPI;
+  const uint32_t need = (max_row + EPI - 1) / EPI;
+  for (int zr : {8, 16, 32, 40, 64})
+    if (fused_zr_ok<KP>(zr) && need <= (uint32_t)zr) return zr;
+  return 8;
+}
+template <int KP> inline uint32_t fused_row_cap_kp(uint32_t max_row) {
+  return std::min<uint32_t>(64u, (uint32_t)fused_zr_select<KP>(max_row) * (uint32_t)Map<KP>::EPI);
+}
diff --git a/libfm_amd/csrc/fmx_mem.hip b/libfm_amd/csrc/fmx_mem.hip
--- a/libfm_amd/csrc/fmx_mem.hip
+++ b/libfm_amd/csrc/fmx_mem.hip
@@ -57,6 +57,51 @@
 std::mutex g_arena_mu;
 Placed* const g_arena_cache = new Placed[16];
 bool arena_cache_on() { const char* e = getenv("FMX_ARENA_CACHE"); return !(e && e[0] == '0'); }
+std::mutex g_spare_mu;
+std::vector<void*>* const g_spare = new std::vector<void*>[16];
+int g_spare_owners[16] = {};
+void* spare_take(int dev) {
+  if (dev < 0 || dev >= 16) return nullptr;
+  std::lock_guard<std::mutex> lk(g_spare_mu);
+  if (g_spare[dev].empty()) return nullptr;
+  void* hd = g_spare[dev].back();
+  g_spare[dev].pop_back();
+  return hd;
+}
+bool spare_give(int dev, void* hd) {
+  if (dev < 0 || dev >= 16) return false;
+  std::lock_guard<std::mutex> lk(g_spare_mu);
+  if (!g_spare_owners[dev] || g_spare[dev].size() >= SPARE_MAX) return false;
+  g_spare[dev].push_back(hd);
+  return true;
+}
+size_t spare_room(int dev) {
+  if (dev < 0 || dev >= 16 || !arena_cache_on()) return 0;
+  std::lock_guard<std::mutex> lk(g_spare_mu);
+  return SPARE_MAX - std::min(SPARE_MAX, g_spare[dev].size());
+}
+void spare_release(int dev, std::vector<void*>& hnds) {
+  if (hnds.empty() || !hip_vm(dev)) return;
+  int cur = 0; (void)hipGetDevice(&cur);
+  if (cur != dev) (void)hipSetDevice(dev);
+  for (void* hd : hnds) (void)hip_vm(dev)->release(hd);
+  if (cur != dev) (void)hipSetDevice(cur);
+  hnds.clear();
+}
+void spare_open(int dev) {
+  if (dev < 0 || dev >= 16 || !arena_cache_on()) return;
+  std::lock_guard<std::mutex> lk(g_spare_mu);
+  g_spare_owners[dev]++;
+}
+void spare_close(int dev) {
+  if (dev < 0 || dev >= 16) return;
+  std::vector<void*> out;
+  {
+    std::lock_guard<std::mutex> lk(g_spare_mu);
+    if (g_spare_owners[dev] > 0 && --g_spare_owners[dev] == 0) out.swap(g_spare[dev]);
+  }
+  spare_release(dev, out);
+}
 double since(std::chrono::steady_clock::time_point t0) { return std::chrono::duration<double>(std::chrono::steady_clock::now() - t0).count(); }
 }
 
@@ -64,16 +109,21 @@
 
 void arena_cache_drop(int device) {
   std::lock_guard<std::mutex> lk(g_arena_mu);
-  for (int d = 0; d < 16; d++)
-    if ((device < 0 || d == device) && g_arena_cache[d].mem.va) {
-      int cur = 0; (void)hipGetDevice(&cur); (void)hipSetDevice(d);
-      (void)g_arena_cache[d].mem.release();
-      (void)hipSetDevice(cur);
-    }
+  for (int d = 0; d < 16; d++) {
+    if (device >= 0 && d != device) continue;
+    std::vector<void*> spare;
+    { std::lock_guard<std::mutex> ls(g_spare_mu); spare.swap(g_spare[d]); }
+    if (!g_arena_cache[d].mem.va && spare.empty()) continue;
+    int cur = 0; (void)hipGetDevice(&cur); (void)hipSetDevice(d);
+    if (g_arena_cache[d].mem.va) (void)g_arena_cache[d].mem.release();
+    (void)hipSetDevice(cur);
+    spare_release(d, spare);
+  }
 }
 
 static void arena_free(fmx_handle h) {
   Placed& A = h->placed;
+  spare_close(h->device);
   if (h->device >= 0 && h->device < 16 && arena_cache_on()) {
     (void)hipStreamSynchronize(h->stream);
     std::lock_guard<std::mutex> lk(g_arena_mu);
@@ -93,6 +143,7 @@
   if (!place_layout(v_bytes, w_bytes, &L) || !hip_vm(h->device)) return false;
   const size_t T = L.T;
   Placed A;
+  std::vector<void*> spare;
   bool have = false;
   if (h->device >= 0 && h->device < 16) {
     std::lock_guard<std::mutex> lk(g_arena_mu);
@@ -119,7 +170,14 @@
     if (!arena_fits(T, free_b)) return false;
     HipProbe probe(h);
     A = Placed();
-    if (build_arena(*hip_vm(h->device), probe, T, pool_bound(T, bound_tables, free_b), &A) != 0) return false;
+    const int e = build_arena(*hip_vm(h->device), probe, T, pool_bound(T, bound_tables, free_b), &A, &spare, spare_room(h->device));
+    if (e != 0) { spare_release(h->device, spare); return false; }
+  }
+  spare_open(h->device);
+  {
+    std::vector<void*> rest;
+    for (void* hd : spare) if (!spare_give(h->device, hd)) rest.push_back(hd);
+    spare_release(h->device, rest);
   }
   h->placed = std::move(A);
   h->tb.V = (float*)h->placed.mem.va;
@@ -149,27 +207,33 @@
   if (hipGetDevice(&dev) != hipSuccess || !hip_vm(dev)) return false;
   HipVm& vm = *hip_vm(dev);
   BigAlloc b; b.device = dev;
-  const size_t reserved = (bytes + BIG_ALIGN - 1) / BIG_ALIGN * BIG_ALIGN;
+  const size_t needed = (bytes + BIG_ALIGN - 1) / BIG_ALIGN * BIG_ALIGN;
+  const size_t reserved = (bytes + BIG_CHUNK - 1) / BIG_CHUNK * BIG_CHUNK;
   static const bool trace = getenv("FMX_TRACE_ALLOC") != nullptr;
   const auto t0 = std::chrono::steady_clock::now();
   if (b.mem.reserve(vm, reserved, BIG_ALIGN)) return false;
   const double t_res = 1e3 * since(t0);
   bool ok = true;
-  for (size_t off = 0; off < reserved && ok; off += BIG_CHUNK)
-    ok = b.mem.create(std::min(BIG_CHUNK, reserved - off)) == 0 && b.mem.map(b.mem.ch.size() - 1) == 0;
+  size_t from_spare = 0;
+  for (size_t off = 0; off < needed && ok; off += BIG_CHUNK) {
+    if (void* hd = spare_take(dev)) { b.mem.adopt(hd, BIG_CHUNK); from_spare++; ok = b.mem.map(b.mem.ch.size() - 1) == 0; }
+    else ok = b.mem.create(std::min(BIG_CHUNK, needed - off)) == 0 && b.mem.map(b.mem.ch.size() - 1) == 0;
+  }
+  const size_t mapped = b.mem.end();
   const double t_map = 1e3 * since(t0);
   if (ok) {
     int ndev = 0; (void)hipGetDeviceCount(&ndev);
-    ok = vm.set_access(b.mem.va, reserved) == 0;
+    ok = vm.set_access(b.mem.va, mapped) == 0;
     const uint64_t used = g_devices_used.load(std::memory_order_relaxed);
     for (int d = 0; ok && d < ndev && d < 64; d++) {
       if (d == dev || !((used >> d) & 1ull)) continue;
       int can = 0;
       if (hipDeviceCanAccessPeer(&can, d, dev) != hipSuccess || !can) { (void)hipGetLastError(); continue; }
-      (void)vm.access_for(b.mem.va, reserved, d);
-    }
-  }
-  if (trace) fprintf(stderr, "[fmx alloc] big %zu bytes: reserve %.3f ms, create+map %.3f ms, access %.3f ms\n", bytes, t_res, t_map - t_res, 1e3 * since(t0) - t_map);
+      (void)vm.access_for(b.mem.va, mapped, d);
+    }
+  }
+  if (trace) fprintf(stderr, "[fmx alloc] big %zu bytes: reserve %.3f ms, create+map %.3f ms (%zu of %zu chunks spare), access %.3f ms\n", bytes, t_res, t_map - t_res,
+                     from_spare, b.mem.ch.size(), 1e3 * since(t0) - t_map);
   if (!ok) return false;
   *p = b.mem.va;
   { std::lock_guard<std::mutex> lk(g_big_mu); g_big.emplace(*p, std::move(b)); }
@@ -208,6 +272,11 @@
   int cur = 0; (void)hipGetDevice(&cur);
   if (cur != b.device) (void)hipSetDevice(b.device);
   (void)hipDeviceSynchronize();
+  for (size_t i = 0; i < b.mem.ch.size(); i++) {
+    if (b.mem.ch[i].size != BIG_CHUNK || !spare_room(b.device)) continue;
+    void* hd = b.mem.give_up(i);
+    if (hd && !spare_give(b.device, hd)) (void)hip_vm(b.device)->release(hd);
+  }
   (void)b.mem.release();
   if (cur != b.device) (void)hipSetDevice(cur);
   return hipSuccess;
diff --git a/libfm_amd/csrc/fmx_place_plan.h b/libfm_amd/csrc/fmx_place_plan.h
--- a/libfm_amd/csrc/fmx_place_plan.h
+++ b/libfm_amd/csrc/fmx_place_plan.h
@@ -62,6 +62,15 @@
     const int e = vm->map(at(i), ch[i].size, ch[i].hnd);
     if (!e) ch[i].mapped = true;
     return e;
+  }
+  void adopt(void* hnd, size_t size) { ch.push_back(Chunk{end(), size, hnd, true, false}); }
+  void* give_up(size_t i) {
+    Chunk& c = ch[i];
+    if (!c.held || !c.mapped || vm->unmap((char*)va + c.off, c.size)) return nullptr;
+    c.mapped = c.held = false;
+    void* hd = c.hnd;
+    c.hnd = nullptr;
+    return hd;
   }
   int take_from(ChunkRange& src, size_t i) {
     Chunk& s = src.ch[i];
@@ -198,7 +207,8 @@
   return mapping_order(cx != SIZE_MAX ? B.of[cx] : none, cy != SIZE_MAX ? B.of[cy] : none, rest, T, pick, cls, per_class);
 }
 
-inline int build_arena(Vm& vm, Probe& dev, size_t T, size_t max_pool, Placed* out) {
+constexpr size_t SPARE_MAX = 16;
+inline int build_arena(Vm& vm, Probe& dev, size_t T, size_t max_pool, Placed* out, std::vector<void*>* spare = nullptr, size_t max_spare = 0) {
   const size_t CH = ARENA_CHUNK;
   ChunkRange P, A;
   ClassBook B;
@@ -243,6 +253,9 @@
   if (!er) er = vm.set_access(A.va, T * CH);
   if (er) return er;
   info.method = 2; info.chunks = (uint32_t)T; info.pool = (uint32_t)P.ch.size(); info.classes_seen = (uint32_t)B.refs.size();
+  if (spare)
+    for (size_t i = 0; i < P.ch.size() && spare->size() < max_spare; i++)
+      if (void* hd = P.give_up(i)) spare->push_back(hd);
   (void)P.release();
   er = dev.zero(A.va, T * CH);
   if (er) return er;
diff --git a/libfm_amd/csrc/fmx_runs.hip b/libfm_amd/csrc/fmx_runs.hip
--- /dev/null
+++ b/libfm_amd/csrc/fmx_runs.hip
@@ -0,0 +1,54 @@
+#include "fmx_internal.h"
+#include "fmx_seq_kernels.h"
+
+int ensure_runs(fmx_handle h, Slot& s) {
+  if (!s.run_start.empty()) return FMX_OK;
+  struct Acc { fmx_handle h; std::chrono::steady_clock::time_point t0;
+               ~Acc() { h->setup_acc += std::chrono::duration<double>(std::chrono::steady_clock::now() - t0).count(); } } acc_{h, std::chrono::steady_clock::now()};
+  const uint32_t n = s.n_rows;
+  if (n == 0 || n >= 0x7FFFFFFEu || s.nnz >= (1ull << 31)) { s.run_start = {0u, n}; s.run_single = {2u}; return FMX_OK; }
+  hipStream_t st = h->stream;
+  std::vector<uint32_t> prev(n, 0u);
+  if (s.nnz) {
+    uint32_t fbits = 1; while (fbits < 32 && (1ull << fbits) < std::max<uint64_t>(h->n_local, 2)) fbits++;
+    size_t tmp_bytes = 0;
+    HIPCHK(h, hipcub::DeviceRadixSort::SortKeys(nullptr, tmp_bytes, (uint64_t*)nullptr, (uint64_t*)nullptr, (int)s.nnz, 0, 32 + (int)fbits, st));
+    auto al = [](size_t x) { return (x + 255) / 256 * 256; };
+    const size_t o_a = 0, o_b = al(s.nnz * 8), o_p = o_b + al(s.nnz * 8), o_t = o_p + al((size_t)n * 4), total = o_t + al(std::max<size_t>(tmp_bytes, 256));
+    char* scratch = nullptr;
+    HIPCHK(h, fmx_dev_alloc(&scratch, total));
+    uint64_t* ka = (uint64_t*)(scratch + o_a); uint64_t* kb = (uint64_t*)(scratch + o_b); uint32_t* d_prev = (uint32_t*)(scratch + o_p);
+    hipError_t e = hipMemsetAsync(d_prev, 0, (size_t)n * 4, st);
+    if (e == hipSuccess) {
+      hipLaunchKernelGGL(k_run_keys, dim3(wave_grid(n)), dim3(256), 0, st, s.ent, s.row_ptr, n, ka);
+      size_t tb_ = tmp_bytes;
+      e = hipcub::DeviceRadixSort::SortKeys(scratch + o_t, tb_, ka, kb, (int)s.nnz, 0, 32 + (int)fbits, st);
+    }
+    if (e == hipSuccess) {
+      hipLaunchKernelGGL(k_run_prev, dim3(2048), dim3(256), 0, st, kb, s.nnz, d_prev);
+      e = hipGetLastError();
+    }
+    if (e == hipSuccess) e = hipMemcpyAsync(prev.data(), d_prev, (size_t)n * 4, hipMemcpyDeviceToHost, st);
+    if (e == hipSuccess) e = hipStreamSynchronize(st);
+    fmx_dev_free(scratch);
+    if (e != hipSuccess) return fail(h, FMX_E_HIP, "ensure_runs failed: %s", hipGetErrorString(e));
+  }
+  std::vector<uint32_t> starts; std::vector<uint8_t> single;
+  uint32_t start = 0;
+  for (uint32_t r = 0; r < n; r++) {
+    const bool rep = (prev[r] & 0x80000000u) != 0;
+    const uint32_t p = prev[r] & 0x7FFFFFFFu;
+    if (rep) {
+      if (r > start) { starts.push_back(start); single.push_back(0); }
+      starts.push_back(r); single.push_back(1);
+      start = r + 1;
+    } else if ((p > start && r > start) || r - start >= 4096u) {
+      starts.push_back(start); single.push_back(0);
+      start = r;
+    }
+  }
+  if (start < n) { starts.push_back(start); single.push_back(0); }
+  starts.push_back(n);
+  s.run_start.swap(starts); s.run_single.swap(single);
+  return FMX_OK;
+}
diff --git a/libfm_amd/csrc/fmx_seg.hip b/libfm_amd/csrc/fmx_seg.hip
--- /dev/null
+++ b/libfm_amd/csrc/fmx_seg.hip
@@ -0,0 +1,121 @@
+#include "fmx_internal.h"
+
+int ensure_segments(fmx_handle h, Slot& s, uint32_t B) {
+  if (s.seg_B == B && s.t_ent) return FMX_OK;
+  if (&s >= h->slots && &s < h->slots + FMX_MAX_SLOTS) {
+    int _rc = slot_in_session(h, (int)(&s - h->slots), "re-bucketing the rows for another batch size"); if (_rc) return _rc;
+  }
+  free_segments(s);
+  const auto t_setup0 = std::chrono::steady_clock::now();
+  static const bool trace = getenv("FMX_TRACE_SETUP") != nullptr;
+  auto tp = [&](const char* what) { if (trace) { (void)hipStreamSynchronize(h->stream); fprintf(stderr, "[fmx setup] segments %-22s %8.3f ms\n", what,
+                                     1e3 * std::chrono::duration<double>(std::chrono::steady_clock::now() - t_setup0).count()); } };
+  struct Acc { fmx_handle h; std::chrono::steady_clock::time_point t0;
+               ~Acc() { h->setup_acc += std::chrono::duration<double>(std::chrono::steady_clock::now() - t0).count(); } } acc_{h, t_setup0};
+  const uint64_t nnz = s.nnz;
+  const uint32_t n_batches = (s.n_rows + B - 1) / B;
+  if (nnz >= (1ull << 31)) return fail(h, FMX_E_UNSUPPORTED, "segmented apply: nnz >= 2^31 in one slot (split the data set)");
+  hipStream_t st = h->stream;
+  uint32_t cap = 64;
+  KP_SWITCH(h->KP, cap = fused_row_cap_kp<KP>(s.max_row));
+  uint32_t fbits = 1; while (fbits < 32 && (1ull << fbits) < std::max<uint64_t>(h->n_local, 2)) fbits++;
+  int bits_batch = 1; while ((1ull << bits_batch) < n_batches) bits_batch++;
+  char* scratch = nullptr;
+  int rc = FMX_OK;
+  const size_t cnt = (size_t)std::max<uint64_t>(nnz, 1);
+  const size_t nb1 = (size_t)n_batches + 1;
+#define SEG_CHK(expr) do { hipError_t _e = (expr); if (_e != hipSuccess) { \
+    rc = fail(h, FMX_E_HIP, "%s failed: %s", #expr, hipGetErrorString(_e)); goto done; } } while (0)
+  {
+    size_t tmp_sort = 0, tmp_scan = 0, tmp_xscan = 0;
+    SEG_CHK(hipcub::DeviceRadixSort::SortPairs(nullptr, tmp_sort, (uint64_t*)nullptr, (uint64_t*)nullptr, (uint64_t*)nullptr, (uint64_t*)nullptr,
+                                               (int)cnt, 0, (int)fbits + bits_batch, st));
+    SEG_CHK(hipcub::DeviceScan::InclusiveSum(nullptr, tmp_scan, (uint32_t*)nullptr, (uint32_t*)nullptr, (int)cnt, st));
+    SEG_CHK(hipcub::DeviceScan::ExclusiveSum(nullptr, tmp_xscan, (uint32_t*)nullptr, (uint32_t*)nullptr, (int)cnt, st));
+    const size_t tmp_bytes = std::max<size_t>(std::max(tmp_sort, std::max(tmp_scan, tmp_xscan)), 256);
+    auto al = [](size_t x) { return (x + 255) / 256 * 256; };
+    size_t off = 0;
+    const size_t o_ka = off; off += al(cnt * 8);
+    const size_t o_kb = off; off += al(cnt * 8);
+    const size_t o_va = off; off += al(cnt * 8);
+    const size_t o_fl = off; off += al(cnt * 4);
+    const size_t o_po = off; off += al(cnt * 4);
+    const size_t o_cf = off; off += al(cnt * 4);
+    const size_t o_cp = off; off += al(cnt * 4);
+    const size_t o_ct = off; off += 256;
+    const size_t o_tmp = off; off += al(tmp_bytes);
+    SEG_CHK(fmx_dev_alloc(&scratch, off));
+    uint64_t* keys_a = (uint64_t*)(scratch + o_ka); uint64_t* keys_b = (uint64_t*)(scratch + o_kb); uint64_t* vals_a = (uint64_t*)(scratch + o_va);
+    uint32_t* flags = (uint32_t*)(scratch + o_fl); uint32_t* pos = (uint32_t*)(scratch + o_po);
+    uint32_t* cflag = (uint32_t*)(scratch + o_cf); uint32_t* cpos = (uint32_t*)(scratch + o_cp);
+    uint32_t* d_counts = (uint32_t*)(scratch + o_ct);
+    void* tmp = scratch + o_tmp;
+    uint64_t* vals_b = nullptr;
+    SEG_CHK(fmx_dev_alloc(&vals_b, cnt * 8));
+    s.t_ent = reinterpret_cast<TEntry*>(vals_b);
+    SEG_CHK(fmx_dev_alloc(&s.cmask, (size_t)std::max<uint32_t>(s.n_rows, 1) * 8));
+    SEG_CHK(fmx_dev_alloc(&s.d_batch_seg, nb1 * 4));
+    SEG_CHK(fmx_dev_alloc(&s.d_cbatch, nb1 * 4));
+    SEG_CHK(fmx_dev_alloc(&s.d_batch_base, nb1 * 8));
+    tp("allocations");
+    hipLaunchKernelGGL(k_seg_slow_rows, dim3(std::min<uint32_t>((s.n_rows + 255) / 256, 2048)), dim3(256), 0, st, s.row_ptr, s.n_rows, cap, s.cmask);
+    s.fused_cap = cap;
+    tp("first launch");
+    SEG_CHK(hipMemsetAsync(d_counts, 0, 16, st));
+    if (nnz) {
+      hipLaunchKernelGGL(k_seg_keys, dim3(wave_grid(s.n_rows)), dim3(256), 0, st, s.ent, s.row_ptr, s.n_rows, B, fbits, keys_a, vals_a, d_counts + 3);
+      size_t tb_ = tmp_bytes;
+      SEG_CHK(hipcub::DeviceRadixSort::SortPairs(tmp, tb_, keys_a, keys_b, vals_a, vals_b, (int)nnz, 0, (int)fbits + bits_batch, st));
+      hipLaunchKernelGGL(k_seg_heads, dim3(2048), dim3(256), 0, st, keys_b, nnz, flags);
+      tp("keys + sort + heads");
+      tb_ = tmp_bytes;
+      SEG_CHK(hipcub::DeviceScan::InclusiveSum(tmp, tb_, flags, pos, (int)nnz, st));
+      hipLaunchKernelGGL(k_seg_batches, dim3((n_batches + 256) / 256), dim3(256), 0, st, pos, nnz, s.row_ptr, s.n_rows, B, n_batches, s.d_batch_seg, s.d_batch_base);
+      uint32_t* head = reinterpret_cast<uint32_t*>(keys_a);
+      hipLaunchKernelGGL(k_seg_head_pos, dim3(2048), dim3(256), 0, st, flags, pos, nnz, head);
+      hipLaunchKernelGGL(k_seg_max_count, dim3(2048), dim3(256), 0, st, head, pos, nnz, d_counts + 2);
+      hipLaunchKernelGGL(k_seg_mark, dim3(2048), dim3(256), 0, st, keys_b, reinterpret_cast<const TEntry*>(vals_b), head, pos, nnz,
+                         s.ent, s.row_ptr, B, fbits, cap, (uint32_t)(s.max_row > cap ? 1u : 0u), s.cmask, cflag);
+      SEG_CHK(hipGetLastError());
+      tb_ = tmp_bytes;
+      SEG_CHK(hipcub::DeviceScan::ExclusiveSum(tmp, tb_, cflag, cpos, (int)nnz, st));
+      hipLaunchKernelGGL(k_seg_counts, dim3(1), dim3(64), 0, st, pos, nnz, cpos, cflag, d_counts + 2, d_counts);
+      uint32_t counts[4] = {0, 0, 0, 0};
+      SEG_CHK(hipMemcpyAsync(counts, d_counts, 16, hipMemcpyDeviceToHost, st));
+      SEG_CHK(hipStreamSynchronize(st));
+      tp("scan + mark + counts");
+      const uint32_t nseg = counts[0];
+      s.nseg = nseg; s.ncseg = counts[1]; s.max_seg_count = counts[2]; s.all_ones = counts[3] == 0u;
+      SEG_CHK(fmx_dev_alloc(&s.seg_feat, (size_t)std::max<uint32_t>(nseg, 1) * 4));
+      SEG_CHK(fmx_dev_alloc(&s.seg_rel, (size_t)std::max<uint32_t>(nseg, 1) * 4));
+      SEG_CHK(fmx_dev_alloc(&s.cseg, (size_t)std::max<uint32_t>(s.ncseg, 1) * 4));
+      SEG_CHK(fmx_dev_alloc(&s.cdesc, (size_t)std::max<uint32_t>(s.ncseg, 1) * sizeof(CDesc)));
+      hipLaunchKernelGGL(k_seg_fill, dim3(2048), dim3(256), 0, st, keys_b, flags, pos, nnz, s.row_ptr, B, fbits, s.seg_feat, s.seg_rel);
+      hipLaunchKernelGGL(k_seg_compact, dim3(2048), dim3(256), 0, st, keys_b, head, cflag, cpos, nseg, s.d_batch_seg, s.cseg,
+                         s.seg_feat, s.seg_rel, s.row_ptr, s.n_rows, B, fbits, s.cdesc, reinterpret_cast<const TEntry*>(vals_b));
+      hipLaunchKernelGGL(k_seg_cbatch, dim3((n_batches + 256) / 256), dim3(256), 0, st, cpos, cflag, nseg, s.d_batch_seg, n_batches, s.d_cbatch);
+      SEG_CHK(hipGetLastError());
+    } else {
+      s.nseg = 0; s.ncseg = 0; s.max_seg_count = 0; s.all_ones = false;
+      SEG_CHK(hipMemsetAsync(s.d_batch_seg, 0, nb1 * 4, st));
+      SEG_CHK(hipMemsetAsync(s.d_cbatch, 0, nb1 * 4, st));
+      SEG_CHK(hipMemsetAsync(s.d_batch_base, 0, nb1 * 8, st));
+      SEG_CHK(fmx_dev_alloc(&s.seg_feat, 4)); SEG_CHK(fmx_dev_alloc(&s.seg_rel, 4));
+      SEG_CHK(fmx_dev_alloc(&s.cseg, 4));
+      SEG_CHK(fmx_dev_alloc(&s.cdesc, sizeof(CDesc)));
+    }
+    s.batch_seg.resize(nb1); s.cbatch.resize(nb1); s.batch_base.resize(nb1);
+    SEG_CHK(hipMemcpyAsync(s.batch_seg.data(), s.d_batch_seg, nb1 * 4, hipMemcpyDeviceToHost, st));
+    SEG_CHK(hipMemcpyAsync(s.cbatch.data(), s.d_cbatch, nb1 * 4, hipMemcpyDeviceToHost, st));
+    SEG_CHK(hipMemcpyAsync(s.batch_base.data(), s.d_batch_base, nb1 * 8, hipMemcpyDeviceToHost, st));
+    SEG_CHK(hipStreamSynchronize(st));
+    tp("fill + compact + tables");
+    s.seg_B = B;
+  }
+done:
+#undef SEG_CHK
+  if (scratch) fmx_dev_free(scratch);
+  tp("frees");
+  if (rc) free_segments(s);
+  return rc;
+}
diff --git a/libfm_amd/csrc/fmx_sgd.hip b/libfm_amd/csrc/fmx_sgd.hip
--- a/libfm_amd/csrc/fmx_sgd.hip
+++ b/libfm_amd/csrc/fmx_sgd.hip
@@ -7,18 +7,6 @@
 
 namespace {
 uint32_t default_w0_chunk(const fmx_config& c) { return fmx_default_w0_chunk(c.learn_rate, c.task); }
-
-template <int KP> constexpr bool fused_zr_ok(int zr) { return Map<KP>::VEC * zr <= 128; }
-template <int KP> int fused_zr_select(uint32_t max_row) {
-  constexpr int EPI = Map<KP>::EPI;
-  const uint32_t need = (max_row + EPI - 1) / EPI;
-  for (int zr : {8, 16, 32, 40, 64})
-    if (fused_zr_ok<KP>(zr) && need <= (uint32_t)zr) return zr;
-  return 8;
-}
-template <int KP> uint32_t fused_row_cap_kp(uint32_t max_row) {
-  return std::min<uint32_t>(64u, (uint32_t)fused_zr_select<KP>(max_row) * (uint32_t)Map<KP>::EPI);
-}
 
 template <int KP, int VAR>
 int launch_fused_zr(fmx_handle h, const Slot& s, const Hyper& hy, uint64_t row0, uint32_t n_rows, hipStream_t st,
@@ -133,124 +121,6 @@
   return sgd_resolve_batch(h, h->slots[slot], opts, out);
 }
 
-extern "C++" int ensure_segments(fmx_handle h, Slot& s, uint32_t B) {
-  if (s.seg_B == B && s.t_ent) return FMX_OK;
-  if (&s >= h->slots && &s < h->slots + FMX_MAX_SLOTS) {
-    int _rc = slot_in_session(h, (int)(&s - h->slots), "re-bucketing the rows for another batch size"); if (_rc) return _rc;
-  }
-  free_segments(s);
-  const auto t_setup0 = std::chrono::steady_clock::now();
-  static const bool trace = getenv("FMX_TRACE_SETUP") != nullptr;
-  auto tp = [&](const char* what) { if (trace) { (void)hipStreamSynchronize(h->stream); fprintf(stderr, "[fmx setup] segments %-22s %8.3f ms\n", what,
-                                     1e3 * std::chrono::duration<double>(std::chrono::steady_clock::now() - t_setup0).count()); } };
-  struct Acc { fmx_handle h; std::chrono::steady_clock::time_point t0;
-               ~Acc() { h->setup_acc += std::chrono::duration<double>(std::chrono::steady_clock::now() - t0).count(); } } acc_{h, t_setup0};
-  const uint64_t nnz = s.nnz;
-  const uint32_t n_batches = (s.n_rows + B - 1) / B;
-  if (nnz >= (1ull << 31)) return fail(h, FMX_E_UNSUPPORTED, "segmented apply: nnz >= 2^31 in one slot (split the data set)");
-  hipStream_t st = h->stream;
-  uint32_t cap = 64;
-  KP_SWITCH(h->KP, cap = fused_row_cap_kp<KP>(s.max_row));
-  uint32_t fbits = 1; while (fbits < 32 && (1ull << fbits) < std::max<uint64_t>(h->n_local, 2)) fbits++;
-  int bits_batch = 1; while ((1ull << bits_batch) < n_batches) bits_batch++;
-  char* scratch = nullptr;
-  int rc = FMX_OK;
-  const size_t cnt = (size_t)std::max<uint64_t>(nnz, 1);
-  const size_t nb1 = (size_t)n_batches + 1;
-#define SEG_CHK(expr) do { hipError_t _e = (expr); if (_e != hipSuccess) { \
-    rc = fail(h, FMX_E_HIP, "%s failed: %s", #expr, hipGetErrorString(_e)); goto done; } } while (0)
-  {
-    size_t tmp_sort = 0, tmp_scan = 0, tmp_xscan = 0;
-    SEG_CHK(hipcub::DeviceRadixSort::SortPairs(nullptr, tmp_sort, (uint64_t*)nullptr, (uint64_t*)nullptr, (uint64_t*)nullptr, (uint64_t*)nullptr,
-                                               (int)cnt, 0, (int)fbits + bits_batch, st));
-    SEG_CHK(hipcub::DeviceScan::InclusiveSum(nullptr, tmp_scan, (uint32_t*)nullptr, (uint32_t*)nullptr, (int)cnt, st));
-    SEG_CHK(hipcub::DeviceScan::ExclusiveSum(nullptr, tmp_xscan, (uint32_t*)nullptr, (uint32_t*)nullptr, (int)cnt, st));
-    const size_t tmp_bytes = std::max<size_t>(std::max(tmp_sort, std::max(tmp_scan, tmp_xscan)), 256);
-    auto al = [](size_t x) { return (x + 255) / 256 * 256; };
-    size_t off = 0;
-    const size_t o_ka = off; off += al(cnt * 8);
-    const size_t o_kb = off; off += al(cnt * 8);
-    const size_t o_va = off; off += al(cnt * 8);
-    const size_t o_fl = off; off += al(cnt * 4);
-    const size_t o_po = off; off += al(cnt * 4);
-    const size_t o_cf = off; off += al(cnt * 4);
-    const size_t o_cp = off; off += al(cnt * 4);
-    const size_t o_ct = off; off += 256;
-    const size_t o_tmp = off; off += al(tmp_bytes);
-    SEG_CHK(fmx_dev_alloc(&scratch, off));
-    uint64_t* keys_a = (uint64_t*)(scratch + o_ka); uint64_t* keys_b = (uint64_t*)(scratch + o_kb); uint64_t* vals_a = (uint64_t*)(scratch + o_va);
-    uint32_t* flags = (uint32_t*)(scratch + o_fl); uint32_t* pos = (uint32_t*)(scratch + o_po);
-    uint32_t* cflag = (uint32_t*)(scratch + o_cf); uint32_t* cpos = (uint32_t*)(scratch + o_cp);
-    uint32_t* d_counts = (uint32_t*)(scratch + o_ct);
-    void* tmp = scratch + o_tmp;
-    uint64_t* vals_b = nullptr;
-    SEG_CHK(fmx_dev_alloc(&vals_b, cnt * 8));
-    s.t_ent = reinterpret_cast<TEntry*>(vals_b);
-    SEG_CHK(fmx_dev_alloc(&s.cmask, (size_t)std::max<uint32_t>(s.n_rows, 1) * 8));
-    SEG_CHK(fmx_dev_alloc(&s.d_batch_seg, nb1 * 4));
-    SEG_CHK(fmx_dev_alloc(&s.d_cbatch, nb1 * 4));
-    SEG_CHK(fmx_dev_alloc(&s.d_batch_base, nb1 * 8));
-    tp("allocations");
-    hipLaunchKernelGGL(k_seg_slow_rows, dim3(std::min<uint32_t>((s.n_rows + 255) / 256, 2048)), dim3(256), 0, st, s.row_ptr, s.n_rows, cap, s.cmask);
-    s.fused_cap = cap;
-    SEG_CHK(hipMemsetAsync(d_counts, 0, 16, st));
-    if (nnz) {
-      hipLaunchKernelGGL(k_seg_keys, dim3(wave_grid(s.n_rows)), dim3(256), 0, st, s.ent, s.row_ptr, s.n_rows, B, fbits, keys_a, vals_a, d_counts + 3);
-      size_t tb_ = tmp_bytes;
-      SEG_CHK(hipcub::DeviceRadixSort::SortPairs(tmp, tb_, keys_a, keys_b, vals_a, vals_b, (int)nnz, 0, (int)fbits + bits_batch, st));
-      hipLaunchKernelGGL(k_seg_heads, dim3(2048), dim3(256), 0, st, keys_b, nnz, flags);
-      tp("keys + sort + heads");
-      tb_ = tmp_bytes;
-      SEG_CHK(hipcub::DeviceScan::InclusiveSum(tmp, tb_, flags, pos, (int)nnz, st));
-      hipLaunchKernelGGL(k_seg_batches, dim3((n_batches + 256) / 256), dim3(256), 0, st, pos, nnz, s.row_ptr, s.n_rows, B, n_batches, s.d_batch_seg, s.d_batch_base);
-      uint32_t* head = reinterpret_cast<uint32_t*>(keys_a);
-      hipLaunchKernelGGL(k_seg_head_pos, dim3(2048), dim3(256), 0, st, flags, pos, nnz, head);
-      hipLaunchKernelGGL(k_seg_max_count, dim3(2048), dim3(256), 0, st, head, pos, nnz, d_counts + 2);
-      hipLaunchKernelGGL(k_seg_mark, dim3(2048), dim3(256), 0, st, keys_b, reinterpret_cast<const TEntry*>(vals_b), head, pos, nnz,
-                         s.ent, s.row_ptr, B, fbits, cap, (uint32_t)(s.max_row > cap ? 1u : 0u), s.cmask, cflag);
-      SEG_CHK(hipGetLastError());
-      tb_ = tmp_bytes;
-      SEG_CHK(hipcub::DeviceScan::ExclusiveSum(tmp, tb_, cflag, cpos, (int)nnz, st));
-      hipLaunchKernelGGL(k_seg_counts, dim3(1), dim3(64), 0, st, pos, nnz, cpos, cflag, d_counts + 2, d_counts);
-      uint32_t counts[4] = {0, 0, 0, 0};
-      SEG_CHK(hipMemcpyAsync(counts, d_counts, 16, hipMemcpyDeviceToHost, st));
-      SEG_CHK(hipStreamSynchronize(st));
-      tp("scan + mark + counts");
-      const uint32_t nseg = counts[0];
-      s.nseg = nseg; s.ncseg = counts[1]; s.max_seg_count = counts[2]; s.all_ones = counts[3] == 0u;
-      SEG_CHK(fmx_dev_alloc(&s.seg_feat, (size_t)std::max<uint32_t>(nseg, 1) * 4));
-      SEG_CHK(fmx_dev_alloc(&s.seg_rel, (size_t)std::max<uint32_t>(nseg, 1) * 4));
-      SEG_CHK(fmx_dev_alloc(&s.cseg, (size_t)std::max<uint32_t>(s.ncseg, 1) * 4));
-      SEG_CHK(fmx_dev_alloc(&s.cdesc, (size_t)std::max<uint32_t>(s.ncseg, 1) * sizeof(CDesc)));
-      hipLaunchKernelGGL(k_seg_fill, dim3(2048), dim3(256), 0, st, keys_b, flags, pos, nnz, s.row_ptr, B, fbits, s.seg_feat, s.seg_rel);
-      hipLaunchKernelGGL(k_seg_compact, dim3(2048), dim3(256), 0, st, keys_b, head, cflag, cpos, nseg, s.d_batch_seg, s.cseg,
-                         s.seg_feat, s.seg_rel, s.row_ptr, s.n_rows, B, fbits, s.cdesc, reinterpret_cast<const TEntry*>(vals_b));
-      hipLaunchKernelGGL(k_seg_cbatch, dim3((n_batches + 256) / 256), dim3(256), 0, st, cpos, cflag, nseg, s.d_batch_seg, n_batches, s.d_cbatch);
-      SEG_CHK(hipGetLastError());
-    } else {
-      s.nseg = 0; s.ncseg = 0; s.max_seg_count = 0; s.all_ones = false;
-      SEG_CHK(hipMemsetAsync(s.d_batch_seg, 0, nb1 * 4, st));
-      SEG_CHK(hipMemsetAsync(s.d_cbatch, 0, nb1 * 4, st));
-      SEG_CHK(hipMemsetAsync(s.d_batch_base, 0, nb1 * 8, st));
-      SEG_CHK(fmx_dev_alloc(&s.seg_feat, 4)); SEG_CHK(fmx_dev_alloc(&s.seg_rel, 4));
-      SEG_CHK(fmx_dev_alloc(&s.cseg, 4));
-      SEG_CHK(fmx_dev_alloc(&s.cdesc, sizeof(CDesc)));
-    }
-    s.batch_seg.resize(nb1); s.cbatch.resize(nb1); s.batch_base.resize(nb1);
-    SEG_CHK(hipMemcpyAsync(s.batch_seg.data(), s.d_batch_seg, nb1 * 4, hipMemcpyDeviceToHost, st));
-    SEG_CHK(hipMemcpyAsync(s.cbatch.data(), s.d_cbatch, nb1 * 4, hipMemcpyDeviceToHost, st));
-    SEG_CHK(hipMemcpyAsync(s.batch_base.data(), s.d_batch_base, nb1 * 8, hipMemcpyDeviceToHost, st));
-    SEG_CHK(hipStreamSynchronize(st));
-    tp("fill + compact + tables");
-    s.seg_B = B;
-  }
-done:
-#undef SEG_CHK
-  if (scratch) fmx_dev_free(scratch);
-  tp("frees");
-  if (rc) free_segments(s);
-  return rc;
-}
 
 static int take_error_bits(fmx_handle h, uint32_t mask, uint32_t* bits) {
   uint32_t e = 0;
@@ -807,57 +677,6 @@
   return FMX_OK;
 }
 
-static int ensure_runs(fmx_handle h, Slot& s) {
-  if (!s.run_start.empty()) return FMX_OK;
-  struct Acc { fmx_handle h; std::chrono::steady_clock::time_point t0;
-               ~Acc() { h->setup_acc += std::chrono::duration<double>(std::chrono::steady_clock::now() - t0).count(); } } acc_{h, std::chrono::steady_clock::now()};
-  const uint32_t n = s.n_rows;
-  if (n == 0 || n >= 0x7FFFFFFEu || s.nnz >= (1ull << 31)) { s.run_start = {0u, n}; s.run_single = {2u}; return FMX_OK; }
-  hipStream_t st = h->stream;
-  std::vector<uint32_t> prev(n, 0u);
-  if (s.nnz) {
-    uint32_t fbits = 1; while (fbits < 32 && (1ull << fbits) < std::max<uint64_t>(h->n_local, 2)) fbits++;
-    size_t tmp_bytes = 0;
-    HIPCHK(h, hipcub::DeviceRadixSort::SortKeys(nullptr, tmp_bytes, (uint64_t*)nullptr, (uint64_t*)nullptr, (int)s.nnz, 0, 32 + (int)fbits, st));
-    auto al = [](size_t x) { return (x + 255) / 256 * 256; };
-    const size_t o_a = 0, o_b = al(s.nnz * 8), o_p = o_b + al(s.nnz * 8), o_t = o_p + al((size_t)n * 4), total = o_t + al(std::max<size_t>(tmp_bytes, 256));
-    char* scratch = nullptr;
-    HIPCHK(h, fmx_dev_alloc(&scratch, total));
-    uint64_t* ka = (uint64_t*)(scratch + o_a); uint64_t* kb = (uint64_t*)(scratch + o_b); uint32_t* d_prev = (uint32_t*)(scratch + o_p);
-    hipError_t e = hipMemsetAsync(d_prev, 0, (size_t)n * 4, st);
-    if (e == hipSuccess) {
-      hipLaunchKernelGGL(k_run_keys, dim3(wave_grid(n)), dim3(256), 0, st, s.ent, s.row_ptr, n, ka);
-      size_t tb_ = tmp_bytes;
-      e = hipcub::DeviceRadixSort::SortKeys(scratch + o_t, tb_, ka, kb, (int)s.nnz, 0, 32 + (int)fbits, st);
-    }
-    if (e == hipSuccess) {
-      hipLaunchKernelGGL(k_run_prev, dim3(2048), dim3(256), 0, st, kb, s.nnz, d_prev);
-      e = hipGetLastError();
-    }
-    if (e == hipSuccess) e = hipMemcpyAsync(prev.data(), d_prev, (size_t)n * 4, hipMemcpyDeviceToHost, st);
-    if (e == hipSuccess) e = hipStreamSynchronize(st);
-    fmx_dev_free(scratch);
-    if (e != hipSuccess) return fail(h, FMX_E_HIP, "ensure_runs failed: %s", hipGetErrorString(e));
-  }
-  std::vector<uint32_t> starts; std::vector<uint8_t> single;
-  uint32_t start = 0;
-  for (uint32_t r = 0; r < n; r++) {
-    const bool rep = (prev[r] & 0x80000000u) != 0;
-    const uint32_t p = prev[r] & 0x7FFFFFFFu;
-    if (rep) {
-      if (r > start) { starts.push_back(start); single.push_back(0); }
-      starts.push_back(r); single.push_back(1);
-      start = r + 1;
-    } else if ((p > start && r > start) || r - start >= 4096u) {
-      starts.push_back(start); single.push_back(0);
-      start = r;
-    }
-  }
-  if (start < n) { starts.push_back(start); single.push_back(0); }
-  starts.push_back(n);
-  s.run_start.swap(starts); s.run_single.swap(single);
-  return FMX_OK;
-}
 static int launch_run_one(fmx_handle h, const Slot& s, const Hyper& hy, uint32_t row0, uint32_t nb, int zr, const double* bias_in, double* bias_out,
                           unsigned long long* slots, uint32_t tag) {
   hipStream_t st = h->stream;
```

After: 277.6 million (median of 2 runs). No clear change (-0.0%).
